# shanglianlm0525/CvPytorch

Hardware: AMD Instinct MI355X
Metric: images/sec/node train step, YOLOv5-s@640 (value: batch resident in HBM when the timed region starts; with_h2d.value: the same step fed from pinned host memory inside the region) & DeepLabv3+R50@1024x512 (config3_deeplabv3plus_r50.value) (higher is better)
Workload: dtype bf16; 1 GPU; coco_yolov5_s.yml YOLOv5-s 640x640 bf16 train step (fwd+loss+bwd+SGD-nesterov+EMA), per-GPU batch 64, synthetic COCO-shape tensors resident in HBM; global_batch=64, parallelism=dp1, launch=hipGraph replay of the whole step, world=1, transport=none (single process), grad_buckets=0, sync_bn=False, deterministic=True

## Files before the change

cvpytorch_amd/arena.py:

```python
import math
from copy import deepcopy

import torch

from . import comm as CM
from . import lib as L
from . import ops
from .train import build_param_groups

_PREP_PLAN = __import__("os").environ.get("CVHIP_PREP_PLAN", "1") != "0"
_ALIGN = 8


def _dense_view(flat, off, like):
    return flat[off:off + like.numel()].as_strided(like.shape, like.stride())


def paired_arena_order(items, follow):
    present = {id(t) for t in items}
    out, placed = [], set()
    for t in items:
        if id(t) in placed:
            continue
        out.append(t)
# ... 346 lines not shown
            if torch.cuda.is_current_stream_capturing():
                ops._OWNED_BACKWARD[0] = True
                try:
                    loss.backward()
                finally:
                    ops._OWNED_BACKWARD[0] = False
                ops.check_parked()
                return None
            seed = self._seeds[key] = torch.ones_like(loss)
        ops._OWNED_BACKWARD[0] = True
        try:
            loss.backward(gradient=seed)
        finally:
            ops._OWNED_BACKWARD[0] = False
        ops.check_parked()

    def scale_loss(self, loss):
        return loss * self.ls_state[0] if self.loss_scaling else loss

    def loss_scale(self):
        v = self.ls_state.tolist()
        return v[0], int(v[3])

    def pre_step(self):
        d = 0.0
        if self.ema_param is not None:
            self.ema_updates += 1
            d = self.ema_decay * (1 - math.exp(-self.ema_updates / 2000))
        slot = self._dyn_host[self.steps % self._dyn_host.shape[0]]
        slot[0], slot[1] = d, self.lr_scale
        self.dyn.copy_(slot, non_blocking=True)

    def step_kernels(self):
        self.finish_allreduce()
        ema_ptr = self.ema_param.data_ptr() if self.ema_param is not None else None
        st = ops._stream()
        if self.loss_scaling:
            g, b, iv = self.ls_hyper
            L.call("cvhip_loss_scale_check", self.grad.data_ptr(), self.total, self.ls_state.data_ptr(), st)
            L.call("cvhip_loss_scale_update", self.ls_state.data_ptr(), self.ls_dyn.data_ptr(), g, b, iv, st)
        if self.optimizer == "adamw":
            L.call("cvhip_adamw_ema", self.param.data_ptr(), self.grad.data_ptr(), self.mom.data_ptr(), self.mom2.data_ptr(), ema_ptr, self.total,
                   self.seg_bounds.data_ptr(), self.seg_lr.data_ptr(), self.seg_wd.data_ptr(), len(self.params), self.betas[0], self.betas[1],
                   self.adam_eps, self.adam_step.data_ptr(), 0.0, 1.0 / self.world, self.dyn.data_ptr(),
                   self.ls_dyn.data_ptr() if self.loss_scaling else None, st)
        elif self.loss_scaling:
            L.call("cvhip_sgd_nesterov_ema_scaled", self.param.data_ptr(), self.grad.data_ptr(), self.mom.data_ptr(), ema_ptr, self.total,
                   self.seg_bounds.data_ptr(), self.seg_lr.data_ptr(), self.seg_wd.data_ptr(), len(self.params), self.momentum,
                   int(self.nesterov), 0, 0.0, 1.0 / self.world, self.dyn.data_ptr(), self.ls_dyn.data_ptr(), st)
        else:
            L.call("cvhip_sgd_nesterov_ema", self.param.data_ptr(), self.grad.data_ptr(), self.mom.data_ptr(), ema_ptr, self.total,
                   self.seg_bounds.data_ptr(), self.seg_lr.data_ptr(), self.seg_wd.data_ptr(), len(self.params), self.momentum,
                   int(self.nesterov), 0, 0.0, 1.0 / self.world, self.dyn.data_ptr(), st)
        if self.ema_buf is not None and self.buf.numel():
            L.call("cvhip_ema_update", self.ema_buf.data_ptr(), self.buf.data_ptr(), self.buf.numel(), 0.0, self.dyn.data_ptr(), st)
        if self._nbt is not None and self.model.training:
            L.call("cvhip_i64_add", self._nbt.data_ptr(), self._nbt.numel(), 1, st)
        self.zero_grad()
        self.zero_stats()

    def prepare_weights(self):
        if not _PREP_PLAN:
            return
        plan = self.prep_plan
        if plan is None or not plan.valid():
            states = [s for s in ops.conv_states_of(self.model) if s.w_fprop is not None and s.rec is not None]
            if not states:
                return
            if torch.cuda.is_current_stream_capturing():
                return
            plan = self.prep_plan = ops.PrepPlan(states)
        plan.run()

    def post_step(self):
        self.steps += 1
        ops.bump_weights_epoch()
        self._reset_buckets()

    def step(self):
        self.pre_step()
        self.step_kernels()
        self.post_step()


class FlatTrainStep:

    def __init__(self, model, state, sync_buffers=False):
        self.model, self.state, self.sync_buffers = model, state, sync_buffers
        self.g1 = self.g2 = None
        self.static_losses = None
        self.eager_tail = False
        self.static_imgs = self.static_targets = None
        self.feats = self.g_feats = None

    @property
    def graph(self):
        return self.g1

    @graph.setter
    def graph(self, v):
        if v is None:
            self.g1 = self.g2 = None
            self.state.defer_allreduce = False
            self.eager_tail = False

    def _eager(self, imgs, targets):
        self.state.prepare_weights()
        losses = self.model(imgs, targets, "train")
        self.state.backward(losses["loss"])
# ... 83 lines not shown
```

cvpytorch_amd/csrc/f16_names.h:

```cpp
#pragma once
#define cvhip_adamw_ema cvhip_adamw_ema_f16
#define cvhip_add2d cvhip_add2d_f16
#define cvhip_add_act_fwd cvhip_add_act_fwd_f16
#define cvhip_bn_acc_shards cvhip_bn_acc_shards_f16
#define cvhip_bn_act_bwd_apply cvhip_bn_act_bwd_apply_f16
#define cvhip_bn_act_bwd_apply_acc cvhip_bn_act_bwd_apply_acc_f16
#define cvhip_bn_act_bwd_partial cvhip_bn_act_bwd_partial_f16
#define cvhip_bn_act_bwd_sums_acc cvhip_bn_act_bwd_sums_acc_f16
#define cvhip_bn_act_fwd cvhip_bn_act_fwd_f16
#define cvhip_bn_act_fwd_acc cvhip_bn_act_fwd_acc_f16
#define cvhip_bn_act_fwd_acc_lazyres cvhip_bn_act_fwd_acc_lazyres_f16
#define cvhip_bn_add_act_fwd cvhip_bn_add_act_fwd_f16
#define cvhip_bn_bwd_finalize cvhip_bn_bwd_finalize_f16
#define cvhip_bn_eval_scale_shift cvhip_bn_eval_scale_shift_f16
#define cvhip_bn_finalize cvhip_bn_finalize_f16
#define cvhip_bn_finalize_acc cvhip_bn_finalize_acc_f16
#define cvhip_bn_stats_partial cvhip_bn_stats_partial_f16
#define cvhip_bn_tail_bwd_sums_acc cvhip_bn_tail_bwd_sums_acc_f16
#define cvhip_box_iou cvhip_box_iou_f16
#define cvhip_channel_scale_bwd_ds cvhip_channel_scale_bwd_ds_f16
#define cvhip_colreduce_rows cvhip_colreduce_rows_f16
#define cvhip_colsum_finalize cvhip_colsum_finalize_f16
#define cvhip_colsum_partial cvhip_colsum_partial_f16
#define cvhip_conv1x1_bwd_fused cvhip_conv1x1_bwd_fused_f16
// ... 31 lines not shown
#define cvhip_dwconv2d_fprop cvhip_dwconv2d_fprop_f16
#define cvhip_dwconv2d_fprop_act cvhip_dwconv2d_fprop_act_f16
#define cvhip_dwconv2d_fprop_stats cvhip_dwconv2d_fprop_stats_f16
#define cvhip_dwconv2d_fprop_stats_rows cvhip_dwconv2d_fprop_stats_rows_f16
#define cvhip_dwconv2d_wgrad cvhip_dwconv2d_wgrad_f16
#define cvhip_ema_update cvhip_ema_update_f16
#define cvhip_f32_unpad_add cvhip_f32_unpad_add_f16
#define cvhip_focus_nchw_f32_to_nhwc_bf16 cvhip_focus_nchw_f32_to_nhwc_bf16_f16
#define cvhip_global_avgpool_bwd cvhip_global_avgpool_bwd_f16
#define cvhip_global_avgpool_fwd cvhip_global_avgpool_fwd_f16
#define cvhip_head_permute_bwd cvhip_head_permute_bwd_f16
#define cvhip_head_permute_fwd cvhip_head_permute_fwd_f16
#define cvhip_i64_add cvhip_i64_add_f16
#define cvhip_last_error cvhip_last_error_f16
#define cvhip_loss_scale_check cvhip_loss_scale_check_f16
#define cvhip_loss_scale_update cvhip_loss_scale_update_f16
#define cvhip_maxpool2d_bwd cvhip_maxpool2d_bwd_f16
#define cvhip_maxpool2d_fwd cvhip_maxpool2d_fwd_f16
#define cvhip_nchw_f32_to_nhwc_bf16 cvhip_nchw_f32_to_nhwc_bf16_f16
#define cvhip_nchw_f32_to_nhwc_bf16_ld cvhip_nchw_f32_to_nhwc_bf16_ld_f16
#define cvhip_nhwc_bf16_to_nchw_f32 cvhip_nhwc_bf16_to_nchw_f32_f16
#define cvhip_nms_sorted cvhip_nms_sorted_f16
#define cvhip_nms_workspace_bytes cvhip_nms_workspace_bytes_f16
#define cvhip_ohem_select cvhip_ohem_select_f16
#define cvhip_ohem_select_workspace_bytes cvhip_ohem_select_workspace_bytes_f16
#define cvhip_ota_assign cvhip_ota_assign_f16
#define cvhip_ota_read_overflow cvhip_ota_read_overflow_f16
#define cvhip_ota_workspace_bytes cvhip_ota_workspace_bytes_f16
#define cvhip_prep_plan_build cvhip_prep_plan_build_f16
#define cvhip_prep_plan_item_bytes cvhip_prep_plan_item_bytes_f16
#define cvhip_prep_plan_run cvhip_prep_plan_run_f16
#define cvhip_resize_bilinear_bwd cvhip_resize_bilinear_bwd_f16
#define cvhip_resize_bilinear_bwd_workspace_bytes cvhip_resize_bilinear_bwd_workspace_bytes_f16
#define cvhip_resize_bilinear_bwd_ws cvhip_resize_bilinear_bwd_ws_f16
#define cvhip_resize_bilinear_fwd cvhip_resize_bilinear_fwd_f16
#define cvhip_resize_nearest_bwd cvhip_resize_nearest_bwd_f16
#define cvhip_resize_nearest_fwd cvhip_resize_nearest_fwd_f16
#define cvhip_scale_nc cvhip_scale_nc_f16
#define cvhip_seg_ce_bilinear_bwd cvhip_seg_ce_bilinear_bwd_f16
#define cvhip_seg_ce_bilinear_bwd_ohem cvhip_seg_ce_bilinear_bwd_ohem_f16
#define cvhip_seg_ce_bilinear_bwd_px cvhip_seg_ce_bilinear_bwd_px_f16
#define cvhip_seg_ce_bilinear_fwd cvhip_seg_ce_bilinear_fwd_f16
#define cvhip_seg_ce_bilinear_fwd_px cvhip_seg_ce_bilinear_fwd_px_f16
#define cvhip_seg_ce_bilinear_ok cvhip_seg_ce_bilinear_ok_f16
#define cvhip_seg_ce_bwd cvhip_seg_ce_bwd_f16
#define cvhip_seg_ce_fwd cvhip_seg_ce_fwd_f16
#define cvhip_seg_ce_rows cvhip_seg_ce_rows_f16
#define cvhip_sgd_nesterov_ema cvhip_sgd_nesterov_ema_f16
#define cvhip_sgd_nesterov_ema_scaled cvhip_sgd_nesterov_ema_scaled_f16
#define cvhip_simota_loss_bwd cvhip_simota_loss_bwd_f16
#define cvhip_simota_loss_fwd cvhip_simota_loss_fwd_f16
#define cvhip_simota_read_assignment cvhip_simota_read_assignment_f16
#define cvhip_simota_workspace_bytes cvhip_simota_workspace_bytes_f16
#define cvhip_u8_nhwc_to_bf16_norm cvhip_u8_nhwc_to_bf16_norm_f16
#define cvhip_upsample2x_bwd cvhip_upsample2x_bwd_f16
#define cvhip_upsample2x_cat_fwd cvhip_upsample2x_cat_fwd_f16
#define cvhip_version cvhip_version_f16
#define cvhip_yolov5_decode cvhip_yolov5_decode_f16
#define cvhip_yolov5_loss_finalize cvhip_yolov5_loss_finalize_f16
#define cvhip_yolov5_loss_level_bwd cvhip_yolov5_loss_level_bwd_f16
#define cvhip_yolov5_loss_level_bwd_bias cvhip_yolov5_loss_level_bwd_bias_f16
#define cvhip_yolov5_loss_level_fwd cvhip_yolov5_loss_level_fwd_f16
#define cvhip_yolov5_loss_level_fwd_assigned cvhip_yolov5_loss_level_fwd_assigned_f16
#define cvhip_yolov5_loss_workspace_bytes cvhip_yolov5_loss_workspace_bytes_f16
#define cvhip_zero_fill cvhip_zero_fill_f16
```

cvpytorch_amd/csrc/pool_resize.hip:

```cpp
#include "common.h"
#include "bilinear_index.h"

namespace cvhip {

__device__ __forceinline__ bool aligned16(const void* p) { return (((uintptr_t)p) & 15) == 0; }

__device__ __forceinline__ f32x8 load8(const h16_t* p, int c, int C, bool vec) {
  if (vec) return unpack8(*reinterpret_cast<const uint4*>(p + c));
  f32x8 r;
#pragma unroll
  for (int j = 0; j < 8; ++j) r.v[j] = (c + j < C) ? (float)p[c + j] : 0.f;
  return r;
}
__device__ __forceinline__ void store8(h16_t* p, int c, int C, bool vec, const f32x8& v) {
  if (vec) {
    *reinterpret_cast<uint4*>(p + c) = pack8(v);
    return;
  }
#pragma unroll
  for (int j = 0; j < 8; ++j)
    if (c + j < C) p[c + j] = (h16_t)v.v[j];
}

struct PoolParams {
// ... 71 lines not shown
    int oh_lo = ih + p.pad - p.k + 1;
    oh_lo = oh_lo <= 0 ? 0 : (oh_lo + p.s - 1) / p.s;
    int oh_hi = (ih + p.pad) / p.s;
    if (oh_hi > p.OH - 1) oh_hi = p.OH - 1;
    int ow_lo = iw + p.pad - p.k + 1;
    ow_lo = ow_lo <= 0 ? 0 : (ow_lo + p.s - 1) / p.s;
    int ow_hi = (iw + p.pad) / p.s;
    if (ow_hi > p.OW - 1) ow_hi = p.OW - 1;
    for (int oh = oh_lo; oh <= oh_hi; ++oh) {
      const int kh = ih - (oh * p.s - p.pad);
      for (int ow = ow_lo; ow <= ow_hi; ++ow) {
        const int kw = iw - (ow * p.s - p.pad);
        const int off = kh * p.k + kw;
        const int64_t opix = ((int64_t)(n * p.OH + oh) * p.OW + ow);
        const f32x8 g = load8(p.dy + opix * p.ld_dy, c, p.C, vec);
        const uint8_t* ip = p.cidx + opix * p.C + c;
        if (vec) {
          const uint2 iv = *reinterpret_cast<const uint2*>(ip);
#pragma unroll
          for (int j = 0; j < 8; ++j) {
            const unsigned b = ((j < 4 ? iv.x : iv.y) >> (8 * (j & 3))) & 0xffu;
            if ((int)b == off) acc[j] += g.v[j];
          }
        } else {
#pragma unroll
          for (int j = 0; j < 8; ++j)
            if (c + j < p.C && ip[j] == off) acc[j] += g.v[j];
        }
      }
    }
    h16_t* dst = p.dx + ((int64_t)(n * p.H + ih) * p.W + iw) * p.ld_dx;
    f32x8 o;
    if (p.accumulate) {
      const f32x8 old = load8(dst, c, p.C, vec);
#pragma unroll
      for (int j = 0; j < 8; ++j) o.v[j] = old.v[j] + acc[j];
    } else {
#pragma unroll
      for (int j = 0; j < 8; ++j) o.v[j] = acc[j];
    }
    store8(dst, c, p.C, vec, o);
  }
}

constexpr int kPoolLdsCvbMax = 4;
constexpr int kPoolLdsMaxPix = 4096;
static inline int pool_lds_cvb(int HW, bool bwd) {
  for (int cvb = kPoolLdsCvbMax; cvb >= 1; cvb >>= 1)
    if (HW * cvb * (bwd ? 24 : 40) <= 160 * 1024) return cvb;
  return 0;
}

template <int K, int kPoolLdsCvb>
__global__ __launch_bounds__(256) void maxpool_s1_lds_fwd_kernel(const PoolParams p) {
  extern __shared__ __attribute__((aligned(16))) unsigned char pool_smem[];
  const int CV = p.C >> 3;
  const int groups = (CV + kPoolLdsCvb - 1) / kPoolLdsCvb;
  const int n = blockIdx.x / groups, cv0 = (blockIdx.x - n * groups) * kPoolLdsCvb;
  const int cvb = min(kPoolLdsCvb, CV - cv0);
  const int HW = p.H * p.W;
  const int items = HW * kPoolLdsCvb;
  uint4* const xs = reinterpret_cast<uint4*>(pool_smem);
  uint4* const rvs = xs + items;
  uint2* const rks = reinterpret_cast<uint2*>(rvs + items);
  const h16_t* const xn = p.x + (int64_t)n * HW * p.ld_x + cv0 * 8;
  for (int i = threadIdx.x; i < items; i += 256) {
    const int pix = i / kPoolLdsCvb, cv = i - pix * kPoolLdsCvb;
    if (cv < cvb) xs[i] = *reinterpret_cast<const uint4*>(xn + (int64_t)pix * p.ld_x + cv * 8);
  }
  __syncthreads();
  constexpr int PAD = K / 2;
  for (int i = threadIdx.x; i < items; i += 256) {
    const int pix = i / kPoolLdsCvb, cv = i - pix * kPoolLdsCvb;
    if (cv >= cvb) continue;
    const int h = pix / p.W, w = pix - h * p.W;
    f32x8 ov;
    int ok[8];
    bool first = true;
#pragma unroll
    for (int j = 0; j < 8; ++j) {
      ov.v[j] = -INFINITY;
      ok[j] = 0;
    }
#pragma unroll
    for (int kw = 0; kw < K; ++kw) {
      const int iw = w + kw - PAD;
      if ((unsigned)iw >= (unsigned)p.W) continue;
      const f32x8 v = unpack8(xs[(h * p.W + iw) * kPoolLdsCvb + cv]);
#pragma unroll
      for (int j = 0; j < 8; ++j) {
        if (first) ok[j] = kw;
        if (v.v[j] > ov.v[j] || v.v[j] != v.v[j]) {
          ov.v[j] = v.v[j];
          ok[j] = kw;
        }
      }
      first = false;
    }
    rvs[i] = pack8(ov);
    uint2 kk;
    kk.x = (unsigned)ok[0] | ((unsigned)ok[1] << 8) | ((unsigned)ok[2] << 16) | ((unsigned)ok[3] << 24);
    kk.y = (unsigned)ok[4] | ((unsigned)ok[5] << 8) | ((unsigned)ok[6] << 16) | ((unsigned)ok[7] << 24);
    rks[i] = kk;
  }
  __syncthreads();
  for (int i = threadIdx.x; i < items; i += 256) {
    const int pix = i / kPoolLdsCvb, cv = i - pix * kPoolLdsCvb;
    if (cv >= cvb) continue;
    const int h = pix / p.W, w = pix - h * p.W;
    float best[8];
    int bi[8];
    bool first = true;
#pragma unroll
    for (int j = 0; j < 8; ++j) {
      best[j] = -INFINITY;
      bi[j] = 0;
    }
#pragma unroll
    for (int kh = 0; kh < K; ++kh) {
      const int ih = h + kh - PAD;
      if ((unsigned)ih >= (unsigned)p.H) continue;
      const int o = (ih * p.W + w) * kPoolLdsCvb + cv;
      const f32x8 v = unpack8(rvs[o]);
      const uint2 kk = rks[o];
#pragma unroll
      for (int j = 0; j < 8; ++j) {
        const int off = kh * K + (int)(((j < 4 ? kk.x : kk.y) >> (8 * (j & 3))) & 0xffu);
        if (first) bi[j] = off;
        if (v.v[j] > best[j] || v.v[j] != v.v[j]) {
          best[j] = v.v[j];
          bi[j] = off;
        }
      }
      first = false;
    }
    {
      const int64_t opix = (int64_t)n * HW + h * p.W + w;
      f32x8 o;
#pragma unroll
      for (int j = 0; j < 8; ++j) o.v[j] = best[j];
      *reinterpret_cast<uint4*>(p.y + opix * p.ld_y + (cv0 + cv) * 8) = pack8(o);
      if (p.idx) {
        uint2 iv;
        iv.x = (unsigned)bi[0] | ((unsigned)bi[1] << 8) | ((unsigned)bi[2] << 16) | ((unsigned)bi[3] << 24);
        iv.y = (unsigned)bi[4] | ((unsigned)bi[5] << 8) | ((unsigned)bi[6] << 16) | ((unsigned)bi[7] << 24);
        *reinterpret_cast<uint2*>(p.idx + opix * p.C + (cv0 + cv) * 8) = iv;
      }
    }
  }
}

template <int K, int kPoolLdsCvb>
__global__ __launch_bounds__(256) void maxpool_s1_lds_bwd_kernel(const PoolParams p) {
  extern __shared__ __attribute__((aligned(16))) unsigned char pool_smem[];
  const int HW = p.H * p.W;
  uint4* const gs = reinterpret_cast<uint4*>(pool_smem);
  uint2* const is = reinterpret_cast<uint2*>(pool_smem + (size_t)HW * kPoolLdsCvb * 16);
  const int CV = p.C >> 3;
  const int groups = (CV + kPoolLdsCvb - 1) / kPoolLdsCvb;
  const int n = blockIdx.x / groups, cv0 = (blockIdx.x - n * groups) * kPoolLdsCvb;
  const int cvb = min(kPoolLdsCvb, CV - cv0);
  for (int i = threadIdx.x; i < HW * kPoolLdsCvb; i += 256) {
    const int pix = i / kPoolLdsCvb, cv = i - pix * kPoolLdsCvb;
    if (cv < cvb) {
      const int64_t opix = (int64_t)n * HW + pix;
      gs[i] = *reinterpret_cast<const uint4*>(p.dy + opix * p.ld_dy + (cv0 + cv) * 8);
      is[i] = *reinterpret_cast<const uint2*>(p.cidx + opix * p.C + (cv0 + cv) * 8);
    }
  }
  __syncthreads();
  constexpr int PAD = K / 2;
  for (int i = threadIdx.x; i < HW * kPoolLdsCvb; i += 256) {
    const int pix = i / kPoolLdsCvb, cv = i - pix * kPoolLdsCvb;
    if (cv >= cvb) continue;
    const int ih = pix / p.W, iw = pix - ih * p.W;
    float acc[8];
#pragma unroll
    for (int j = 0; j < 8; ++j) acc[j] = 0.f;
    const int oh_lo = max(0, ih - PAD), oh_hi = min(p.H - 1, ih + PAD);
    const int ow_lo = max(0, iw - PAD), ow_hi = min(p.W - 1, iw + PAD);
    for (int oh = oh_lo; oh <= oh_hi; ++oh) {
      const int kh = ih - oh + PAD;
      for (int ow = ow_lo; ow <= ow_hi; ++ow) {
        const unsigned off = (unsigned)(kh * K + (iw - ow + PAD));
        const int o = (oh * p.W + ow) * kPoolLdsCvb + cv;
        const f32x8 g = unpack8(gs[o]);
        const uint2 iv = is[o];
#pragma unroll
        for (int j = 0; j < 8; ++j) {
          const unsigned b = ((j < 4 ? iv.x : iv.y) >> (8 * (j & 3))) & 0xffu;
          if (b == off) acc[j] += g.v[j];
        }
      }
    }
    h16_t* const dst = p.dx + ((int64_t)n * HW + pix) * p.ld_dx + (cv0 + cv) * 8;
    f32x8 o;
    if (p.accumulate) {
      const f32x8 old = unpack8(*reinterpret_cast<const uint4*>(dst));
#pragma unroll
      for (int j = 0; j < 8; ++j) o.v[j] = old.v[j] + acc[j];
    } else {
#pragma unroll
      for (int j = 0; j < 8; ++j) o.v[j] = acc[j];
    }
    *reinterpret_cast<uint4*>(dst) = pack8(o);
  }
}

static bool pool_lds_ok(const PoolParams& p, bool bwd) {
  auto a16 = [](const void* q) { return (((uintptr_t)q) & 15) == 0; };
  static int on = -1;
  if (on < 0) {
    const char* e = getenv("CVHIP_POOL_LDS");
    on = (e && e[0] == '0') ? 0 : 1;
  }
  if (!on || p.s != 1 || !(p.k & 1) || p.pad != p.k / 2 || p.OH != p.H || p.OW != p.W || (p.k != 3 && p.k != 5 && p.k != 9 && p.k != 13)) return false;
  const int cvb = pool_lds_cvb(p.H * p.W, bwd);
  if ((p.C & 7) || p.H * p.W > kPoolLdsMaxPix || cvb == 0 || (int64_t)p.N * ((p.C / 8 + cvb - 1) / cvb) < 128) return false;
  if (bwd) return (p.ld_dy & 7) == 0 && (p.ld_dx & 7) == 0 && a16(p.dy) && a16(p.dx) && ((((uintptr_t)p.cidx) & 7) == 0);
  return (p.ld_x & 7) == 0 && (p.ld_y & 7) == 0 && a16(p.x) && a16(p.y) && (!p.idx || ((((uintptr_t)p.idx) & 7) == 0));
}

template <int K, int CVB>
static int launch_pool_lds(const PoolParams& p, bool bwd, hipStream_t s) {
  constexpr int kPoolLdsCvb = CVB;
  const int groups = (p.C / 8 + kPoolLdsCvb - 1) / kPoolLdsCvb;
  const int lds = p.H * p.W * kPoolLdsCvb * (bwd ? 24 : 40);
  auto kf = maxpool_s1_lds_fwd_kernel<K, CVB>;
  auto kb = maxpool_s1_lds_bwd_kernel<K, CVB>;
  static bool attr_done[2][64] = {};
  int devid = 0;
  (void)hipGetDevice(&devid);
  bool& done = attr_done[bwd ? 1 : 0][devid & 63];
  if (!done) {
    const int cap = 160 * 1024;
    hipError_t e = bwd ? hipFuncSetAttribute(reinterpret_cast<const void*>(kb), hipFuncAttributeMaxDynamicSharedMemorySize, cap)
                       : hipFuncSetAttribute(reinterpret_cast<const void*>(kf), hipFuncAttributeMaxDynamicSharedMemorySize, cap);
    if (e != hipSuccess) {
      set_last_error("hipFuncSetAttribute(maxpool_s1_lds)", e);
      return CVHIP_ERR_LAUNCH;
    }
    done = true;
  }
  if (bwd) hipLaunchKernelGGL(kb, dim3(p.N * groups), dim3(256), lds, s, p);
  else hipLaunchKernelGGL(kf, dim3(p.N * groups), dim3(256), lds, s, p);
  return check_launch(bwd ? "maxpool_s1_lds_bwd_kernel" : "maxpool_s1_lds_fwd_kernel");
}

static int try_pool_lds(const PoolParams& p, bool bwd, hipStream_t s) {
  if (!pool_lds_ok(p, bwd)) return -1;
  const int cvb = pool_lds_cvb(p.H * p.W, bwd);
#define CVHIP_POOL_K(KV)                                       \
  if (cvb == 4) return launch_pool_lds<KV, 4>(p, bwd, s);     \
  if (cvb == 2) return launch_pool_lds<KV, 2>(p, bwd, s);     \
  return launch_pool_lds<KV, 1>(p, bwd, s);
  switch (p.k) {
    case 3: CVHIP_POOL_K(3)
    case 5: CVHIP_POOL_K(5)
    case 9: CVHIP_POOL_K(9)
    default: CVHIP_POOL_K(13)
  }
#undef CVHIP_POOL_K
}

struct UpParams {
  const h16_t *a, *b;
  h16_t* out;
  int ld_a, ld_b, ld_out, Ca, Cb, N, Ha, Wa;
};

__global__ __launch_bounds__(256) void up2cat_fwd_kernel(const UpParams p) {
  const int Ct = p.Ca + p.Cb;
  const int CVa = (p.Ca + 7) >> 3, CVb = (p.Cb + 7) >> 3;
  const int CV = CVa + CVb;
  const int OH = p.Ha * 2, OW = p.Wa * 2;
  const bool vec = (p.Ca & 7) == 0 && (p.Cb & 7) == 0 && (p.ld_a & 7) == 0 && (p.ld_b & 7) == 0 &&
                   (p.ld_out & 7) == 0 && aligned16(p.a) && aligned16(p.b) && aligned16(p.out);
  (void)Ct;
  const int64_t total = (int64_t)p.N * OH * OW * CV;
  for (int64_t i = (int64_t)blockIdx.x * 256 + threadIdx.x; i < total; i += (int64_t)gridDim.x * 256) {
    int cv, ow, oh, n;
    split_index(i, CV, OW, OH, &cv, &ow, &oh, &n);
    h16_t* orow = p.out + ((int64_t)(n * OH + oh) * OW + ow) * p.ld_out;
    if (cv < CVa) {
      const f32x8 v = load8(p.a + ((int64_t)(n * p.Ha + (oh >> 1)) * p.Wa + (ow >> 1)) * p.ld_a, cv * 8, p.Ca, vec);
      store8(orow, cv * 8, p.Ca, vec, v);
    } else {
      const int cb = (cv - CVa) * 8;
      const f32x8 v = load8(p.b + ((int64_t)(n * OH + oh) * OW + ow) * p.ld_b, cb, p.Cb, vec);
      store8(orow + p.Ca, cb, p.Cb, vec, v);
    }
  }
}

__global__ __launch_bounds__(256) void up2_bwd_kernel(const UpParams p) {
  const int CV = (p.Ca + 7) >> 3;
  const int OW = p.Wa * 2, OH = p.Ha * 2;
  const bool vec = (p.Ca & 7) == 0 && (p.ld_a & 7) == 0 && (p.ld_out & 7) == 0 && aligned16(p.a) && aligned16(p.out);
  const int64_t total = (int64_t)p.N * p.Ha * p.Wa * CV;
  for (int64_t i = (int64_t)blockIdx.x * 256 + threadIdx.x; i < total; i += (int64_t)gridDim.x * 256) {
    int cv, w, h, n;
    split_index(i, CV, p.Wa, p.Ha, &cv, &w, &h, &n);
    f32x8 s;
#pragma unroll
    for (int j = 0; j < 8; ++j) s.v[j] = 0.f;
#pragma unroll
    for (int dy = 0; dy < 2; ++dy)
#pragma unroll
      for (int dx = 0; dx < 2; ++dx) {
        const f32x8 v = load8(p.out + ((int64_t)(n * OH + 2 * h + dy) * OW + 2 * w + dx) * p.ld_out, cv * 8, p.Ca, vec);
#pragma unroll
        for (int j = 0; j < 8; ++j) s.v[j] += v.v[j];
      }
    store8(const_cast<h16_t*>(p.a) + ((int64_t)(n * p.Ha + h) * p.Wa + w) * p.ld_a, cv * 8, p.Ca, vec, s);
  }
// ... 553 lines not shown
  if (k * k > 255 || pad * 2 > k) return CVHIP_ERR_UNSUPPORTED;
  PoolParams p{};
  p.x = (const h16_t*)x;
  p.y = (h16_t*)y;
  p.idx = argmax;
  p.ld_x = ld_x;
  p.ld_y = ld_y;
  p.N = N;
  p.C = C;
  p.H = H;
  p.W = W;
  p.k = k;
  p.s = stride;
  p.pad = pad;
  p.OH = (H + 2 * pad - k) / stride + 1;
  p.OW = (W + 2 * pad - k) / stride + 1;
  {
    const int rc = try_pool_lds(p, false, (hipStream_t)stream);
    if (rc >= 0 || rc < -1) return rc;
  }
  const int64_t total = (int64_t)N * p.OH * p.OW * ((C + 7) / 8);
  hipLaunchKernelGGL(maxpool_fwd_kernel, dim3(grid_for(total)), dim3(256), 0, (hipStream_t)stream, p);
  return check_launch("maxpool_fwd_kernel");
}

int cvhip_maxpool2d_bwd(const void* dy, int32_t ld_dy, const uint8_t* argmax, void* dx, int32_t ld_dx, int32_t N,
                        int32_t C, int32_t H, int32_t W, int32_t k, int32_t stride, int32_t pad, int accumulate,
                        void* stream) {
  if (!dy || !dx || !argmax || N <= 0 || C <= 0 || H <= 0 || W <= 0 || k <= 0 || stride <= 0 || pad < 0)
    return CVHIP_ERR_INVALID;
  PoolParams p{};
  p.dy = (const h16_t*)dy;
  p.cidx = argmax;
  p.dx = (h16_t*)dx;
  p.ld_dy = ld_dy;
  p.ld_dx = ld_dx;
  p.N = N;
  p.C = C;
  p.H = H;
  p.W = W;
  p.k = k;
  p.s = stride;
  p.pad = pad;
  p.OH = (H + 2 * pad - k) / stride + 1;
  p.OW = (W + 2 * pad - k) / stride + 1;
  p.accumulate = accumulate;
  {
    const int rc = try_pool_lds(p, true, (hipStream_t)stream);
    if (rc >= 0 || rc < -1) return rc;
  }
  const int64_t total = (int64_t)N * H * W * ((C + 7) / 8);
  hipLaunchKernelGGL(maxpool_bwd_kernel, dim3(grid_for(total)), dim3(256), 0, (hipStream_t)stream, p);
  return check_launch("maxpool_bwd_kernel");
}

int cvhip_upsample2x_cat_fwd(const void* a, int32_t ld_a, int32_t Ca, const void* b, int32_t ld_b, int32_t Cb,
                             void* out, int32_t ld_out, int32_t N, int32_t Ha, int32_t Wa, void* stream) {
  if (!a || !out || Ca <= 0 || Cb < 0 || (Cb > 0 && !b) || N <= 0 || Ha <= 0 || Wa <= 0) return CVHIP_ERR_INVALID;
  UpParams p{};
  p.a = (const h16_t*)a;
  p.b = (const h16_t*)b;
  p.out = (h16_t*)out;
  p.ld_a = ld_a;
  p.ld_b = ld_b;
  p.ld_out = ld_out;
  p.Ca = Ca;
  p.Cb = Cb;
  p.N = N;
  p.Ha = Ha;
  p.Wa = Wa;
  const int64_t total = (int64_t)N * Ha * 2 * Wa * 2 * ((Ca + 7) / 8 + (Cb + 7) / 8);
  hipLaunchKernelGGL(up2cat_fwd_kernel, dim3(grid_for(total)), dim3(256), 0, (hipStream_t)stream, p);
  return check_launch("up2cat_fwd_kernel");
}

int cvhip_upsample2x_bwd(const void* dout, int32_t ld_dout, void* da, int32_t ld_da, int32_t Ca, int32_t N, int32_t Ha,
                         int32_t Wa, void* stream) {
  if (!dout || !da || Ca <= 0 || N <= 0 || Ha <= 0 || Wa <= 0) return CVHIP_ERR_INVALID;
  UpParams p{};
  p.out = (h16_t*)const_cast<void*>(dout);
  p.a = (const h16_t*)da;
  p.ld_out = ld_dout;
  p.ld_a = ld_da;
  p.Ca = Ca;
  p.N = N;
  p.Ha = Ha;
  p.Wa = Wa;
  const int64_t total = (int64_t)N * Ha * Wa * ((Ca + 7) / 8);
  hipLaunchKernelGGL(up2_bwd_kernel, dim3(grid_for(total)), dim3(256), 0, (hipStream_t)stream, p);
  return check_launch("up2_bwd_kernel");
}

int cvhip_resize_nearest_fwd(const void* x, int32_t ld_x, void* y, int32_t ld_y, int32_t N, int32_t C, int32_t Hi, int32_t Wi,
                             int32_t Ho, int32_t Wo, void* stream) {
  if (!x || !y || N <= 0 || C <= 0 || Hi <= 0 || Wi <= 0 || Ho <= 0 || Wo <= 0) return CVHIP_ERR_INVALID;
  BilParams p{};
  p.src = (const h16_t*)x;
  p.dst = (h16_t*)y;
  p.ld_src = ld_x;
  p.ld_dst = ld_y;
  p.N = N;
  p.C = C;
  p.Hi = Hi;
  p.Wi = Wi;
  p.Ho = Ho;
  p.Wo = Wo;
// ... 186 lines not shown
```

cvpytorch_amd/csrc/weights_optim.hip:

```cpp
#include <string.h>

#include "common.h"
#include "conv_plan.h"

namespace cvhip {

__global__ __launch_bounds__(256) void cast_f32_bf16_kernel(const float* __restrict__ src, h16_t* __restrict__ dst, int64_t n) {
  const int64_t nv = n >> 3;
  const bool al = (((uintptr_t)src) & 15) == 0;
  for (int64_t i = (int64_t)blockIdx.x * 256 + threadIdx.x; i < nv; i += (int64_t)gridDim.x * 256) {
    float4 a, b;
    if (al) {
      a = reinterpret_cast<const float4*>(src)[2 * i];
      b = reinterpret_cast<const float4*>(src)[2 * i + 1];
    } else {
      const float* q = src + 8 * i;
      a = make_float4(q[0], q[1], q[2], q[3]);
      b = make_float4(q[4], q[5], q[6], q[7]);
    }
    uint4 u;
    u.x = pack2(a.x, a.y);
    u.y = pack2(a.z, a.w);
    u.z = pack2(b.x, b.y);
    u.w = pack2(b.z, b.w);
// ... 475 lines not shown
    it.K = d->K;
    it.R = d->R;
    it.S = d->S;
    it.C = d->C;
    it.Kv = d->k_valid > 0 ? d->k_valid : d->K;
    it.Cv = d->c_valid > 0 ? d->c_valid : d->C;
    const int64_t nel = (int64_t)d->K * d->R * d->S * d->C;
    it.blk_begin = blk;
    it.nblk_f = (int)cdiv64(nel, kPrepFpropPerBlock);
    it.nblk_d = 0;
    if (it.wd) {
      IgemmParams ip;
      const int ncls = plan_dgrad(d, &ip);
      if (ncls < 0) return ncls;
      it.ncls = ncls;
      int64_t end = 0;
      int tapn = 0;
      for (int q = 0; q < ncls; ++q) {
        const IgemmClass& c = ip.cls[q];
        PrepClass& pc = it.cls[q];
        pc.TR = c.TR; pc.TS = c.TS; pc.r0 = c.r0; pc.r_step = c.r_step; pc.s0 = c.s0; pc.s_step = c.s_step;
        pc.tap_begin = tapn;
        tapn += c.TR * c.TS;
        pc.w_off = c.w_off;
        pc.w_end = c.w_off + (int64_t)d->C * c.TR * c.TS * d->K;
        if (pc.w_off != end) return CVHIP_ERR_UNSUPPORTED;
        end = pc.w_end;
      }
      if (end != nel || tapn != d->R * d->S) return CVHIP_ERR_UNSUPPORTED;
      it.ktiles = cdiv(d->K, kPrepTile);
      it.ctiles = cdiv(d->C, kPrepTile);
      it.nblk_d = tapn * it.ktiles * it.ctiles;
    }
    it.nblk_bf = band_image_fprop(d) ? (int)cdiv64(nel / 8, 256) : 0;
    it.nblk_bd = (it.wd && band_image_dgrad(d)) ? (int)cdiv64(nel / 8, 256) : 0;
    blk += it.nblk_f + it.nblk_d + it.nblk_bf + it.nblk_bd;
  }
  *total_blocks = blk;
  return CVHIP_OK;
}

int cvhip_prep_plan_run(const void* table_device, int32_t n, int32_t total_blocks, void* stream) {
  if (!table_device || n <= 0 || total_blocks <= 0) return CVHIP_ERR_INVALID;
  hipLaunchKernelGGL(prep_all_kernel, dim3(total_blocks), dim3(256), 0, (hipStream_t)stream, (const PrepItem*)table_device, n);
  return check_launch("prep_all_kernel");
}

extern "C++" {
namespace cvhip {
__global__ void i64_add_kernel(long long* v, int64_t n, long long delta) {
  const int64_t i = (int64_t)blockIdx.x * blockDim.x + threadIdx.x;
  if (i < n) v[i] += delta;
}
}
}

int cvhip_i64_add(int64_t* v, int64_t n, int64_t delta, void* stream) {
  if (!v || n < 0) return CVHIP_ERR_INVALID;
  if (n == 0) return CVHIP_OK;
  hipLaunchKernelGGL(i64_add_kernel, dim3((unsigned)((n + 255) / 256)), dim3(256), 0, (hipStream_t)stream, (long long*)v, n, (long long)delta);
  return check_launch("i64_add_kernel");
}

int cvhip_ema_update(float* ema, const float* src, int64_t n, float decay, const float* dyn_decay, void* stream) {
  if (!ema || !src || n < 0) return CVHIP_ERR_INVALID;
  if (n == 0) return CVHIP_OK;
  hipLaunchKernelGGL(ema_kernel, dim3(grid1d(n)), dim3(256), 0, (hipStream_t)stream, ema, src, n, decay, dyn_decay);
  return check_launch("ema_kernel");
}

}
```

cvpytorch_amd/csrc/yolo_loss.hip:

```cpp
#pragma clang fp contract(off)
#include "common.h"
#include "dual4.h"

namespace cvhip {

constexpr int kLossMaxA = 8;
constexpr int kCandStride = 4;

struct YoloLossParams {
  const h16_t* raw;
  h16_t* draw;
  const float* targets;
  const int* assign;
  int ld, N, A, NO, H, W, T, nc, ncand;
  float anchor_t;
  float anchors[kLossMaxA * 2];
  int* winner;
  int* head;
  int* next;
  int* cell;
  float* cand;
  float* cgrad;
  int gstride;
  float* partial;
  float* dobj;
  float* sums;
  const float* gout;
  float k_box, k_cls, k_obj;
};

__device__ __forceinline__ D4 ciou_xywh(float x, float y, float w, float h, float tx, float ty, float tw, float th) {
  const float eps = 1e-7f;
  const D4 X = var(x, 0), Y = var(y, 1), Wd = var(w, 2), Hd = var(h, 3);
  const D4 b1x1 = X - scale(Wd, 0.5f), b1x2 = X + scale(Wd, 0.5f);
  const D4 b1y1 = Y - scale(Hd, 0.5f), b1y2 = Y + scale(Hd, 0.5f);
  const float b2x1 = tx - tw / 2, b2x2 = tx + tw / 2, b2y1 = ty - th / 2, b2y2 = ty + th / 2;
  const D4 iw = clamp0(dmin(b1x2, cst(b2x2)) - dmax(b1x1, cst(b2x1)));
  const D4 ih = clamp0(dmin(b1y2, cst(b2y2)) - dmax(b1y1, cst(b2y1)));
  const D4 inter = iw * ih;
  const D4 w1 = b1x2 - b1x1, h1 = (b1y2 - b1y1) + cst(eps);
  const float w2 = b2x2 - b2x1, h2 = b2y2 - b2y1 + eps;
  const D4 uni = (w1 * h1 + cst(w2 * h2)) - inter + cst(eps);
  const D4 iou = inter / uni;
  const D4 cw = dmax(b1x2, cst(b2x2)) - dmin(b1x1, cst(b2x1));
  const D4 ch = dmax(b1y2, cst(b2y2)) - dmin(b1y1, cst(b2y1));
  const D4 c2 = cw * cw + ch * ch + cst(eps);
  const D4 dx = cst(b2x1 + b2x2) - b1x1 - b1x2;
  const D4 dy = cst(b2y1 + b2y2) - b1y1 - b1y2;
  const D4 rho2 = scale(dx * dx + dy * dy, 0.25f);
  const D4 da = cst(atanf(w2 / h2)) - datan(w1 / h1);
  const D4 v = scale(da * da, 0.40528473456935108578f);
  const float alpha = v.v / (v.v - iou.v + (1.f + eps));
  return iou - (rho2 / c2 + scale(v, alpha));
}

__global__ __launch_bounds__(256) void yolo_cand_kernel(const YoloLossParams p) {
  const int lane = threadIdx.x & 63;
  const int c = blockIdx.x * 4 + (threadIdx.x >> 6);
  if (c >= p.ncand) return;
  const int T = p.T, A = p.A;
  const int off = c / (A * T);
  const int a = (c / T) % A;
  const int t = c % T;
  const float* tg = p.targets + (int64_t)t * 6;
  const float img = tg[0];
  const float nx = (float)p.W, ny = (float)p.H;
  const float gx = tg[2] * nx, gy = tg[3] * ny, gw = tg[4] * nx, gh = tg[5] * ny;
  const float aw = p.anchors[a * 2], ah = p.anchors[a * 2 + 1];
  const float rw = gw / aw, rh = gh / ah;
  const float rmax = fmaxf(fmaxf(rw, 1.f / rw), fmaxf(rh, 1.f / rh));
  bool sel = (img >= 0.f) && (rmax < p.anchor_t);
  const float gxi = nx - gx, gyi = ny - gy;
  const float g = 0.5f;
  if (off == 1) sel = sel && ((gx - floorf(gx)) < g) && (gx > 1.f);
  else if (off == 2) sel = sel && ((gy - floorf(gy)) < g) && (gy > 1.f);
  else if (off == 3) sel = sel && ((gxi - floorf(gxi)) < g) && (gxi > 1.f);
  else if (off == 4) sel = sel && ((gyi - floorf(gyi)) < g) && (gyi > 1.f);
  float* cs = p.cand + (int64_t)c * kCandStride;
  const float* tm = tg;
  if (p.assign) {
    const int m = p.assign[c];
    sel = m >= 0;
    if (sel) tm = p.targets + (int64_t)m * 6;
  }
  if (!sel) {
    if (lane == 0) {
      p.cell[c] = -1;
      cs[0] = 0.f;
      cs[1] = 0.f;
      cs[2] = 0.f;
    }
    return;
  }
  const float ox = (off == 1 ? 0.5f : (off == 3 ? -0.5f : 0.f)), oy = (off == 2 ? 0.5f : (off == 4 ? -0.5f : 0.f));
  int gi = (int)(gx - ox), gj = (int)(gy - oy);
  gi = min(max(gi, 0), p.W - 1);
  gj = min(max(gj, 0), p.H - 1);
  const int b = (int)img;
  const int cell = ((b * A + a) * p.H + gj) * p.W + gi;
  if (lane == 0) {
    p.cell[c] = cell;
    atomicMax(p.winner + cell, c + 1);
    p.next[c] = atomicExch(p.head + cell, c + 1);
  }
  const h16_t* px = p.raw + ((int64_t)(b * p.H + gj) * p.W + gi) * p.ld + a * p.NO;
  const float r0 = (float)px[0], r1 = (float)px[1], r2 = (float)px[2], r3 = (float)px[3];
  const float s0 = sigmoid_ref(r0), s1 = sigmoid_ref(r1), s2 = sigmoid_ref(r2), s3 = sigmoid_ref(r3);
  const float bx = s0 * 2.f - 0.5f, by = s1 * 2.f - 0.5f;
  const float bw = (s2 * 2.f) * (s2 * 2.f) * aw, bh = (s3 * 2.f) * (s3 * 2.f) * ah;
  const float mx = tm[2] * nx, my = tm[3] * ny, mw = tm[4] * nx, mh = tm[5] * ny;
  const D4 ci = ciou_xywh(bx, by, bw, bh, mx - (float)gi, my - (float)gj, mw, mh);
  float* gr = p.cgrad + (int64_t)c * p.gstride;
  if (lane == 0) {
    cs[0] = ci.v;
    cs[1] = 1.f - ci.v;
    gr[0] = -ci.d[0] * (2.f * s0 * (1.f - s0));
    gr[1] = -ci.d[1] * (2.f * s1 * (1.f - s1));
    gr[2] = -ci.d[2] * (8.f * s2 * s2 * (1.f - s2) * aw);
    gr[3] = -ci.d[3] * (8.f * s3 * s3 * (1.f - s3) * ah);
    gr[4] = 0.f;
  }
  int cls = (int)tm[1];
  cls = min(max(cls, 0), p.nc - 1);
  float lsum = 0.f;
  for (int k = lane; k < p.nc; k += 64) {
    const float x = (float)px[5 + k];
    const float tt = (k == cls) ? 1.f : 0.f;
    lsum += bce_logits(x, tt);
    gr[5 + k] = sigmoid_ref(x) - tt;
  }
#pragma unroll
  for (int o = 32; o > 0; o >>= 1) lsum += __shfl_xor(lsum, o, 64);
  if (lane == 0) cs[2] = p.nc > 1 ? lsum : 0.f;
}

__device__ __forceinline__ float block_sum_1024(float v, float* red) {
  const int t = threadIdx.x;
  red[t] = v;
  __syncthreads();
  for (int s = 512; s > 0; s >>= 1) {
    if (t < s) red[t] += red[t + s];
    __syncthreads();
  }
  const float r = red[0];
  __syncthreads();
  return r;
}

__device__ __forceinline__ void yolo_cand_reduce(const YoloLossParams& p, float* red) {
  float n = 0.f, lb = 0.f, lc = 0.f;
  for (int c0 = threadIdx.x; c0 < p.ncand; c0 += 8 * 1024) {
    int cl[8];
    float b8[8], c8[8];
#pragma unroll
    for (int u = 0; u < 8; ++u) {
      const int c = c0 + u * 1024;
      cl[u] = c < p.ncand ? p.cell[c] : -1;
    }
#pragma unroll
    for (int u = 0; u < 8; ++u) {
      const int64_t c = cl[u] >= 0 ? c0 + u * 1024 : 0;
      b8[u] = p.cand[c * kCandStride + 1];
      c8[u] = p.cand[c * kCandStride + 2];
    }
#pragma unroll
    for (int u = 0; u < 8; ++u) {
      if (cl[u] >= 0) {
        n += 1.f;
        lb += b8[u];
        lc += c8[u];
      }
    }
  }
  n = block_sum_1024(n, red);
  lb = block_sum_1024(lb, red);
  lc = block_sum_1024(lc, red);
  if (threadIdx.x == 0) {
    p.sums[0] = n;
    p.sums[1] = lb;
    p.sums[2] = lc;
  }
}

template <typename IT>
__global__ __launch_bounds__(256) void yolo_obj_bwd_fill_kernel(const YoloLossParams p) {
  const IT VP = (IT)(p.ld >> 3);
  const IT HW = (IT)p.H * (IT)p.W;
  const IT nvec = (IT)p.N * HW * VP;
  const float go = (p.gout ? p.gout[0] : 1.f) * p.k_obj;
  const IT step = (IT)gridDim.x * 256;
  const bool inv = (VP & (VP - 1)) == 0 && (step & (VP - 1)) == 0;
  const int vp_shift = inv ? __ffs((int)VP) - 1 : 0;
  auto anchors_of = [&](int c0) {
    unsigned m = 0;
    for (int a = 0; a < p.A; ++a) {
      const int oc = a * p.NO + 4;
      if (oc >= c0 && oc < c0 + 8) m |= 1u << a;
    }
    return m;
  };
  const unsigned my_mask = inv ? anchors_of((int)(((IT)blockIdx.x * 256 + threadIdx.x) & (VP - 1)) * 8) : 0u;
  for (IT i = (IT)blockIdx.x * 256 + threadIdx.x; i < nvec; i += step) {
    IT pix;
    int c0;
    unsigned mask;
    if (inv) {
      pix = i >> vp_shift;
      c0 = (int)(i & (VP - 1)) * 8;
      mask = my_mask;
    } else {
      pix = i / VP;
      c0 = (int)(i - pix * VP) * 8;
      mask = anchors_of(c0);
    }
    h16_t out[8];
#pragma unroll
    for (int j = 0; j < 8; ++j) out[j] = (h16_t)0.f;
    if (mask) {
      const IT n = pix / HW;
      const IT cell0 = pix + n * (IT)(p.A - 1) * HW;
      for (int a = 0; a < p.A; ++a) {
        if (!((mask >> a) & 1u)) continue;
        const int oc = a * p.NO + 4;
        const h16_t gq = (h16_t)(p.dobj[(int64_t)cell0 + (int64_t)a * (int64_t)HW] * go);
#pragma unroll
        for (int j = 0; j < 8; ++j)
          if (c0 + j == oc) out[j] = gq;
      }
    }
    *reinterpret_cast<uint4*>(p.draw + (int64_t)pix * p.ld + c0) = *reinterpret_cast<const uint4*>(out);
  }
}

template <bool BWD, typename IT>
__global__ __launch_bounds__(256) void yolo_obj_kernel(const YoloLossParams p) {
  __shared__ float red[256];
  const IT ncell = (IT)p.N * (IT)p.A * (IT)p.H * (IT)p.W;
  const float go = BWD ? (p.gout ? p.gout[0] : 1.f) * p.k_obj : 0.f;
  float acc = 0.f;
  for (IT i = (IT)blockIdx.x * 256 + threadIdx.x; i < ncell; i += (IT)gridDim.x * 256) {
    IT r = i / (IT)p.W;
    const int gi = (int)(i - r * (IT)p.W);
    const IT r2 = r / (IT)p.H;
    const int gj = (int)(r - r2 * (IT)p.H);
    const int n = (int)(r2 / (IT)p.A);
    const int a = (int)(r2 - (IT)n * (IT)p.A);
    const int64_t o = ((int64_t)(n * p.H + gj) * p.W + gi) * p.ld + a * p.NO + 4;
    const float x = (float)p.raw[o];
    const int w = p.winner[i];
    const float tt = w > 0 ? fmaxf(p.cand[(int64_t)(w - 1) * kCandStride], 0.f) : 0.f;
    if (BWD) p.draw[o] = (h16_t)((sigmoid_ref(x) - tt) * go);
    else {
      acc += bce_logits(x, tt);
      p.dobj[i] = sigmoid_ref(x) - tt;
    }
  }
  if (!BWD) {
    red[threadIdx.x] = acc;
    __syncthreads();
    for (int s = 128; s > 0; s >>= 1) {
      if (threadIdx.x < s) red[threadIdx.x] += red[threadIdx.x + s];
      __syncthreads();
    }
    if (threadIdx.x == 0) p.partial[blockIdx.x] = red[0];
  }
}

__global__ __launch_bounds__(1024) void yolo_obj_reduce_kernel(const YoloLossParams p, int nblocks) {
  __shared__ float red[1024];
  if (blockIdx.x == 1) {
    yolo_cand_reduce(p, red);
    return;
  }
  float v = 0.f;
  for (int i = threadIdx.x; i < nblocks; i += 1024) v += p.partial[i];
  v = block_sum_1024(v, red);
  if (threadIdx.x == 0) p.sums[3] = v;
}

__global__ __launch_bounds__(256) void yolo_cand_bwd_kernel(const YoloLossParams p) {
  const int lane = threadIdx.x & 63;
  const int c = blockIdx.x * 4 + (threadIdx.x >> 6);
  if (c >= p.ncand) return;
  const int cell = p.cell[c];
  if (cell < 0 || p.winner[cell] != c + 1) return;
  const float n = p.sums[0];
  const float g = p.gout ? p.gout[0] : 1.f;
  const float kb = g * p.k_box / n, kc = g * p.k_cls / n;
  int mine = 0x7fffffff;
  int cur = p.head[cell];
  int cnt = 0;
  float acc0 = 0.f, acc1 = 0.f;
  const int ch0 = lane, ch1 = lane + 64;
  while (cur != 0) {
    const int e = cur - 1;
    if (cnt < 64) {
      if (lane == cnt) mine = e;
    } else {
      const float* gr = p.cgrad + (int64_t)e * p.gstride;
      if (ch0 < p.NO) acc0 += gr[ch0];
      if (ch1 < p.NO) acc1 += gr[ch1];
    }
    ++cnt;
    cur = p.next[e];
  }
  const int k = cnt < 64 ? cnt : 64;
  int last = -1;
  for (int i = 0; i < k; ++i) {
    int cand_v = mine > last ? mine : 0x7fffffff;
#pragma unroll
    for (int o = 32; o > 0; o >>= 1) cand_v = min(cand_v, __shfl_xor(cand_v, o, 64));
    last = cand_v;
    const float* gr = p.cgrad + (int64_t)cand_v * p.gstride;
    if (ch0 < p.NO) acc0 += gr[ch0];
    if (ch1 < p.NO) acc1 += gr[ch1];
  }
  const int gi = cell % p.W;
  int r = cell / p.W;
  const int gj = r % p.H;
  r /= p.H;
  const int a = r % p.A;
  const int b = r / p.A;
  h16_t* dst = p.draw + ((int64_t)(b * p.H + gj) * p.W + gi) * p.ld + a * p.NO;
  if (ch0 < p.NO && ch0 != 4) dst[ch0] = (h16_t)(acc0 * (ch0 < 4 ? kb : kc));
  if (ch1 < p.NO) dst[ch1] = (h16_t)(acc1 * kc);
}

constexpr int kBiasRows = CVHIP_YOLO_BIAS_ROWS;
template <typename IT>
__global__ __launch_bounds__(256) void yolo_bias_partial_kernel(const YoloLossParams p, float* __restrict__ part) {
  __shared__ float wacc[4][kLossMaxA * 128];
  __shared__ float ored[kLossMaxA][256];
  const int K = p.A * p.NO;
  const int t = threadIdx.x, lane = t & 63, wave = t >> 6;
  for (int i = t; i < 4 * kLossMaxA * 128; i += 256) (&wacc[0][0])[i] = 0.f;
  __syncthreads();
  const int per_blk = (p.ncand + gridDim.x - 1) / gridDim.x;
  const int c_begin = blockIdx.x * per_blk, c_end = min(c_begin + per_blk, p.ncand);
  for (int g0 = c_begin + wave * 64; g0 < c_end; g0 += 256) {
    const int c = g0 + lane;
    unsigned long long m = __ballot(c < c_end && p.cell[c] >= 0);
    while (m) {
      int cc[8];
      float v0[8], v1[8];
      int nv = 0;
#pragma unroll
      for (int u = 0; u < 8; ++u) {
        cc[u] = -1;
        if (m) {
          cc[u] = g0 + __ffsll((long long)m) - 1;
          m &= m - 1;
          nv = u + 1;
        }
      }
#pragma unroll
      for (int u = 0; u < 8; ++u) {
        const float* gr = p.cgrad + (int64_t)(cc[u] >= 0 ? cc[u] : 0) * p.gstride;
        v0[u] = (cc[u] >= 0 && lane < p.NO && lane != 4) ? gr[lane] : 0.f;
        v1[u] = (cc[u] >= 0 && lane + 64 < p.NO) ? gr[lane + 64] : 0.f;
      }
#pragma unroll
      for (int u = 0; u < 8; ++u) {
        if (u < nv) {
          const int a = (cc[u] / p.T) % p.A;
          if (lane < p.NO && lane != 4) wacc[wave][a * p.NO + lane] += v0[u];
          if (lane + 64 < p.NO) wacc[wave][a * p.NO + lane + 64] += v1[u];
        }
      }
    }
  }
  float oa[kLossMaxA];
#pragma unroll
  for (int k = 0; k < kLossMaxA; ++k) oa[k] = 0.f;
  {
    const IT ncell = (IT)p.N * (IT)p.A * (IT)p.H * (IT)p.W, HW = (IT)p.H * (IT)p.W;
    const IT per = (ncell + gridDim.x - 1) / gridDim.x;
    const IT i_begin = (IT)blockIdx.x * per;
    IT i_end = i_begin + per;
    if (i_end > ncell) i_end = ncell;
    for (IT i0 = i_begin + t; i0 < i_end; i0 += 256 * 8) {
      float d[8];
      int a[8];
#pragma unroll
      for (int u = 0; u < 8; ++u) {
        const IT i = i0 + (IT)u * 256;
        const bool ok = i < i_end;
        d[u] = ok ? p.dobj[ok ? i : i_begin] : 0.f;
        a[u] = (int)(((ok ? i : i_begin) / HW) % (IT)p.A);
      }
#pragma unroll
      for (int u = 0; u < 8; ++u)
#pragma unroll
        for (int k = 0; k < kLossMaxA; ++k) oa[k] += k == a[u] ? d[u] : 0.f;
    }
  }
#pragma unroll
  for (int k = 0; k < kLossMaxA; ++k) ored[k][t] = oa[k];
  __syncthreads();
  for (int st = 128; st > 0; st >>= 1) {
    if (t < st) {
#pragma unroll
      for (int k = 0; k < kLossMaxA; ++k) ored[k][t] += ored[k][t + st];
    }
    __syncthreads();
  }
  const float n = p.sums[0];
  const float g = p.gout ? p.gout[0] : 1.f;
  const float kb = n > 0.f ? g * p.k_box / n : 0.f, kc = n > 0.f ? g * p.k_cls / n : 0.f, go = g * p.k_obj;
  float* const row = part + (int64_t)blockIdx.x * 2 * K;
  for (int ch = t; ch < K; ch += 256) {
    const int a = ch / p.NO, o = ch - a * p.NO;
    const float v = ((wacc[0][ch] + wacc[1][ch]) + wacc[2][ch]) + wacc[3][ch];
    row[ch] = o == 4 ? ored[a][0] * go : v * (o < 4 ? kb : kc);
  }
}

__global__ void yolo_finalize_kernel(const float* sums, int L, const float* ncell, const float* balance, float hyp_box,
                                     float hyp_obj, float hyp_cls, int nc, float bs, float* total, float* stats) {
  if (threadIdx.x != 0 || blockIdx.x != 0) return;
  float lbox = 0.f, lobj = 0.f, lcls = 0.f;
  for (int i = 0; i < L; ++i) {
    const float n = sums[i * 4];
    if (n > 0.f) {
      lbox += sums[i * 4 + 1] / n;
      lcls += sums[i * 4 + 2] / (n * (float)nc);
    }
    lobj += sums[i * 4 + 3] / ncell[i] * balance[i];
  }
  lbox *= hyp_box;
  lobj *= hyp_obj;
  lcls *= hyp_cls;
  total[0] = (lbox + lobj + lcls) * bs;
  stats[0] = lbox;
  stats[1] = lobj;
  stats[2] = lcls;
}

static int fill(YoloLossParams& p, const cvhip_yolo_loss_desc* d, const void* raw, const float* targets, void* ws, float* sums) {
  if (!d || !raw || !targets || !ws || !sums) return CVHIP_ERR_INVALID;
  if (d->N <= 0 || d->A <= 0 || d->A > kLossMaxA || d->NO < 6 || d->NO > 128 || d->H <= 0 || d->W <= 0 || d->T <= 0 || d->ld < d->A * d->NO)
    return CVHIP_ERR_INVALID;
  const int64_t ncell = (int64_t)d->N * d->A * d->H * d->W;
  const int64_t ncand = (int64_t)5 * d->A * d->T;
  if (ncell >= (1ll << 31) || ncand >= (1ll << 30)) return CVHIP_ERR_UNSUPPORTED;
  p.raw = (const h16_t*)raw;
  p.draw = nullptr;
  p.targets = targets;
  p.assign = nullptr;
  p.ld = d->ld;
  p.N = d->N;
  p.A = d->A;
  p.NO = d->NO;
  p.H = d->H;
  p.W = d->W;
  p.T = d->T;
  p.nc = d->NO - 5;
  p.ncand = (int)ncand;
  p.anchor_t = d->anchor_t;
  for (int i = 0; i < d->A * 2; ++i) p.anchors[i] = d->anchors[i];
  p.gstride = (d->NO + 3) / 4 * 4;
  unsigned char* w = (unsigned char*)ws;
  auto take = [&](int64_t bytes) {
    unsigned char* r = w;
    w += (bytes + 255) / 256 * 256;
    return r;
  };
  p.winner = (int*)take(ncell * 4);
  p.head = (int*)take(ncell * 4);
  p.next = (int*)take(ncand * 4);
  p.cell = (int*)take(ncand * 4);
  p.cand = (float*)take(ncand * kCandStride * 4);
  p.cgrad = (float*)take(ncand * p.gstride * 4);
  p.partial = (float*)take(1024 * 4);
  p.dobj = (float*)take(ncell * 4);
  p.sums = sums;
  p.gout = nullptr;
  p.k_box = p.k_cls = p.k_obj = 0.f;
  return CVHIP_OK;
}

}

using namespace cvhip;

extern "C" {

int64_t cvhip_yolov5_loss_workspace_bytes(const cvhip_yolo_loss_desc* d) {
  if (!d || d->N <= 0 || d->A <= 0 || d->NO <= 0 || d->H <= 0 || d->W <= 0 || d->T <= 0) return CVHIP_ERR_INVALID;
  const int64_t ncell = (int64_t)d->N * d->A * d->H * d->W;
  const int64_t ncand = (int64_t)5 * d->A * d->T;
  const int64_t gs = (d->NO + 3) / 4 * 4;
  auto r = [](int64_t b) { return (b + 255) / 256 * 256; };
  return r(ncell * 4) * 2 + r(ncand * 4) * 2 + r(ncand * kCandStride * 4) + r(ncand * gs * 4) + r(1024 * 4) + r(ncell * 4);
}

static int level_fwd(const cvhip_yolo_loss_desc* d, const void* raw, const float* targets, const int32_t* assign, void* ws, float* sums4,
                     void* stream);

int cvhip_yolov5_loss_level_fwd(const cvhip_yolo_loss_desc* d, const void* raw, const float* targets, void* ws, float* sums4,
                                void* stream) {
  return level_fwd(d, raw, targets, nullptr, ws, sums4, stream);
}

int cvhip_yolov5_loss_level_fwd_assigned(const cvhip_yolo_loss_desc* d, const void* raw, const float* targets, const int32_t* assign,
                                         void* ws, float* sums4, void* stream) {
  if (!assign) return CVHIP_ERR_INVALID;
  return level_fwd(d, raw, targets, assign, ws, sums4, stream);
}

static int level_fwd(const cvhip_yolo_loss_desc* d, const void* raw, const float* targets, const int32_t* assign, void* ws, float* sums4,
                     void* stream) {
  YoloLossParams p;
  int rc = fill(p, d, raw, targets, ws, sums4);
  if (rc != CVHIP_OK) return rc;
  p.assign = assign;
  hipStream_t st = (hipStream_t)stream;
  const int64_t ncell = (int64_t)p.N * p.A * p.H * p.W;
  rc = zero_fill(p.winner, (ncell * 4 + 255) / 256 * 256 * 2, st);
  if (rc != CVHIP_OK) return rc;
  hipLaunchKernelGGL(yolo_cand_kernel, dim3(cdiv(p.ncand, 4)), dim3(256), 0, st, p);
  const int nb = (int)(cdiv64(ncell, 256) < 1024 ? cdiv64(ncell, 256) : 1024);
// ... 9 lines not shown
  hipLaunchKernelGGL(yolo_finalize_kernel, dim3(1), dim3(64), 0, (hipStream_t)stream, sums, levels, ncell, balance, hyp_box, hyp_obj,
                     hyp_cls, nc, batch, total, stats3);
  return check_launch("yolov5_loss_finalize");
}

static int level_bwd(const cvhip_yolo_loss_desc* d, const void* raw, const float* targets, void* ws, const float* sums4, const float* gout,
                     float k_box, float k_cls, float k_obj, void* draw, float* bias_partial, void* stream);

int cvhip_yolov5_loss_level_bwd(const cvhip_yolo_loss_desc* d, const void* raw, const float* targets, void* ws, const float* sums4,
                                const float* gout, float k_box, float k_cls, float k_obj, void* draw, void* stream) {
  return level_bwd(d, raw, targets, ws, sums4, gout, k_box, k_cls, k_obj, draw, nullptr, stream);
}

int cvhip_yolov5_loss_level_bwd_bias(const cvhip_yolo_loss_desc* d, const void* raw, const float* targets, void* ws, const float* sums4,
                                     const float* gout, float k_box, float k_cls, float k_obj, void* draw, float* bias_partial,
                                     void* stream) {
  if (!bias_partial) return CVHIP_ERR_INVALID;
  return level_bwd(d, raw, targets, ws, sums4, gout, k_box, k_cls, k_obj, draw, bias_partial, stream);
}

static int level_bwd(const cvhip_yolo_loss_desc* d, const void* raw, const float* targets, void* ws, const float* sums4, const float* gout,
                     float k_box, float k_cls, float k_obj, void* draw, float* bias_partial, void* stream) {
  YoloLossParams p;
  int rc = fill(p, d, raw, targets, ws, const_cast<float*>(sums4));
  if (rc != CVHIP_OK) return rc;
  if (!draw) return CVHIP_ERR_INVALID;
  p.draw = (h16_t*)draw;
  p.gout = gout;
  p.k_box = k_box;
  p.k_cls = k_cls;
  p.k_obj = k_obj;
  hipStream_t st = (hipStream_t)stream;
  const int64_t ncell = (int64_t)p.N * p.A * p.H * p.W;
  if ((p.ld & 7) == 0 && (((uintptr_t)p.draw) & 15) == 0) {
    const int64_t nvec = (int64_t)p.N * p.H * p.W * (p.ld >> 3);
    const int nbf = (int)(cdiv64(nvec, 256 * 4) < 8192 ? cdiv64(nvec, 256 * 4) : 8192);
    if (nvec + (int64_t)nbf * 256 < (1ll << 32)) hipLaunchKernelGGL(yolo_obj_bwd_fill_kernel<unsigned>, dim3(nbf > 0 ? nbf : 1), dim3(256), 0, st, p);
    else hipLaunchKernelGGL(yolo_obj_bwd_fill_kernel<int64_t>, dim3(nbf > 0 ? nbf : 1), dim3(256), 0, st, p);
  } else {
    rc = zero_fill(p.draw, (int64_t)p.N * p.H * p.W * p.ld * 2, st);
    if (rc != CVHIP_OK) return rc;
    const int nb = (int)(cdiv64(ncell, 256) < 8192 ? cdiv64(ncell, 256) : 8192);
    if (ncell + (int64_t)nb * 256 < (1ll << 32)) hipLaunchKernelGGL((yolo_obj_kernel<true, unsigned>), dim3(nb), dim3(256), 0, st, p);
    else hipLaunchKernelGGL((yolo_obj_kernel<true, int64_t>), dim3(nb), dim3(256), 0, st, p);
  }
  hipLaunchKernelGGL(yolo_cand_bwd_kernel, dim3(cdiv(p.ncand, 4)), dim3(256), 0, st, p);
  if (bias_partial) {
    if (ncell < (1ll << 31)) hipLaunchKernelGGL(yolo_bias_partial_kernel<unsigned>, dim3(kBiasRows), dim3(256), 0, st, p, bias_partial);
    else hipLaunchKernelGGL(yolo_bias_partial_kernel<int64_t>, dim3(kBiasRows), dim3(256), 0, st, p, bias_partial);
  }
  return check_launch("yolov5_loss_level_bwd");
}

}
```

cvpytorch_amd/lib.py:

```python
import ctypes as C
import os

import torch

_HERE = os.path.dirname(os.path.abspath(__file__))
LIB_PATH = os.environ.get("CVHIP_LIB") or os.path.join(_HERE, "libcvhip.so")

OK, ERR_INVALID, ERR_UNSUPPORTED, ERR_LAUNCH = 0, -1, -2, -3
ACT_NONE, ACT_RELU, ACT_SILU, ACT_LEAKY, ACT_SIGMOID, ACT_HSWISH = 0, 1, 2, 3, 4, 5
DTYPE_F32, DTYPE_F64, DTYPE_I32, DTYPE_BF16, DTYPE_U8 = 0, 1, 2, 3, 4
RED_SUM, RED_MAX, RED_MIN = 0, 1, 2
DGRAD_CLASS_INTS = 12
REDUCE_SCRATCH_ROWS = 64
YOLO_BIAS_ROWS = 256
BN_ACC_SHARDS = 16


class CvhipError(RuntimeError):
    pass


class ConvDesc(C.Structure):
    _fields_ = [(n, C.c_int32) for n in (
        "N", "C", "H", "W", "K", "R", "S", "stride_h", "stride_w", "pad_h", "pad_w", "dil_h", "dil_w",
        "groups", "x_ld", "y_ld", "k_valid", "c_valid")]

    def key(self):
        return tuple(getattr(self, n) for n, _ in self._fields_)


class ConvFuse(C.Structure):
    _fields_ = [("bias", C.c_void_p), ("stats_partial", C.c_void_p), ("bn_acc", C.c_void_p), ("ep_scale", C.c_void_p),
                ("ep_shift", C.c_void_p), ("ep_act", C.c_int32), ("ep_act_param", C.c_float), ("pro_scale", C.c_void_p),
                ("pro_shift", C.c_void_p), ("pro_act", C.c_int32), ("pro_act_param", C.c_float), ("z_out", C.c_void_p),
                ("z_ld", C.c_int32), ("residual", C.c_void_p), ("residual_ld", C.c_int32), ("residual_pre", C.c_int32),
                ("x_image", C.c_void_p), ("x_image_planes", C.c_int32), ("pro_lo", C.c_int32), ("pro_hi", C.c_int32),
                ("y2", C.c_void_p), ("y2_ld", C.c_int32), ("y_split", C.c_int32)]


class LazyIn(C.Structure):
    _fields_ = [("scale", C.c_void_p), ("shift", C.c_void_p), ("act", C.c_int32), ("act_param", C.c_float), ("c_lo", C.c_int32),
                ("c_hi", C.c_int32)]


PATCH_CLASS_INTS = 30
BAND_PLAN_INTS = 13
WGRAD_BAND_PLAN_INTS = 8


class PrepEntry(C.Structure):
    _fields_ = [("desc", ConvDesc), ("master", C.c_void_p), ("w_fprop", C.c_void_p), ("w_dgrad", C.c_void_p)]


class YoloLossDesc(C.Structure):
    _fields_ = [(n, C.c_int32) for n in ("N", "A", "NO", "H", "W", "ld", "T")] + [("anchor_t", C.c_float), ("anchors", C.c_float * 16)]


class OtaDesc(C.Structure):
    _fields_ = [(n, C.c_int32) for n in ("L", "N", "A", "NO", "T", "G")] + [("H", C.c_int32 * 4), ("W", C.c_int32 * 4), ("ld", C.c_int32 * 4),
                                                                            ("stride", C.c_float * 4), ("anchors", (C.c_float * 16) * 4),
                                                                            ("anchor_t", C.c_float), ("img_size", C.c_float)]


class SimotaDesc(C.Structure):
    _fields_ = [(n, C.c_int32) for n in ("L", "B", "A", "G", "nc")] + [("H", C.c_int32 * 4), ("W", C.c_int32 * 4), ("ld", C.c_int32 * 4),
                                                                       ("stride", C.c_float * 4)]

# ... 22 lines not shown
    "cvhip_prep_plan_run": (_i32, [_p, _i32, _i32, _p]),
    "cvhip_conv2d_fprop": (_i32, [_dp, _p, _p, _p, _p, _p, _p]),
    "cvhip_conv2d_fprop_fused": (_i32, [_dp, _p, _p, _p, C.POINTER(ConvFuse), _p]),
    "cvhip_conv2d_wgrad_image": (_i32, [_dp, _p, _i32, _p, _p, _p]),
    "cvhip_conv2d_fprop_prologue_ok": (_i32, [_dp, _i32]),
    "cvhip_conv2d_patch_plan": (_i32, [_dp, _i32, C.POINTER(_i32), _i32]),
    "cvhip_conv2d_band_plan": (_i32, [_dp, _i32, C.POINTER(_i32)]),
    "cvhip_conv2d_wgrad_band_plan": (_i32, [_dp, C.POINTER(_i32)]),
    "cvhip_conv1x1_stream_prologue_ok": (_i32, [_dp, _i32]),
    "cvhip_conv2d_wgrad_stem_bn": (_i32, [_dp, _p, _p, _i32, _p, _p, _p, _p, _p, _p, _p, _i32, _p, _p, _i32, _i32, _f32, _p, _p]),
    "cvhip_bn_finalize_acc": (_i32, [_p, _i32, _i32, _i64, _p, _p, _p, _p, _f32, _f32, _p, _p, _p, _p, _p]),
    "cvhip_bn_act_fwd_acc_lazyres": (_i32, [_p, _i32, _p, _i32, _i64, _i32, _p, _i32, _i64, _p, _p, _p, _p, _f32, _f32, _p, _p, _p, _p, _i32, _f32,
                                     _p, _i32, _p, _p, _p]),
    "cvhip_conv1x1_bwd_fused_split": (_i32, [_dp, _p, _i32, _p, _i32, _i32, _p, _p, _i32, _p, _p, _p, _p, _p, _p, _p, _i32, _p, _p, _i32, _i32, _f32, _p,
                                      _i32, _p, _i32, _p, C.POINTER(LazyIn), _p]),
    "cvhip_conv1x1_bwd_fused_lazy": (_i32, [_dp, _p, _i32, _p, _i32, _i32, _p, _p, _p, _p, _p, _p, _p, _p, _i32, _p, _p, _i32, _i32, _f32, _p, _i32,
                                     _p, _i32, _p, C.POINTER(LazyIn), _p]),
    "cvhip_conv2d_dgrad": (_i32, [_dp, _p, _p, _p, _p]),
    "cvhip_conv2d_dgrad_add": (_i32, [_dp, _p, _p, _p, _i32, _p, _p]),
    "cvhip_conv2d_wgrad": (_i32, [_dp, _p, _p, _p, _i32, _p]),
    "cvhip_conv2d_wgrad_det_workspace_bytes": (_i64, [_dp]),
    "cvhip_conv2d_wgrad_det": (_i32, [_dp, _p, _p, _p, _i32, _p, _i64, _p]),
    "cvhip_conv1x1_bwd_fused_ok": (_i32, [_dp]),
    "cvhip_conv1x1_bwd_fused": (_i32, [_dp, _p, _i32, _p, _i32, _i32, _p, _p, _p, _p, _p, _p, _p, _p, _p, _i32, _f32, _p, _i32, _p, _i32,
                                _p, _p]),
    "cvhip_dwconv2d_fprop": (_i32, [_dp, _p, _p, _p, _p, _p]),
    "cvhip_dwconv2d_fprop_act": (_i32, [_dp, _p, _p, _p, _i32, _f32, _p, _p]),
    "cvhip_dwconv2d_fprop_stats_rows": (_i64, [_dp, _p, _p]),
    "cvhip_dwconv2d_fprop_stats": (_i32, [_dp, _p, _p, _p, _p, _p, _p]),
    "cvhip_dwconv2d_dgrad": (_i32, [_dp, _p, _p, _p, _p]),
    "cvhip_dwconv2d_wgrad": (_i32, [_dp, _p, _p, _p, _i32, _p]),
    "cvhip_colreduce_rows": (_i32, [_i64, _i32]),
    "cvhip_bn_stats_partial": (_i32, [_p, _i64, _i32, _i32, _p, _p]),
    "cvhip_bn_finalize": (_i32, [_p, _i32, _i32, _i64, _p, _p, _p, _p, _f32, _f32, _p, _p, _p, _p, _p]),
    "cvhip_bn_eval_scale_shift": (_i32, [_i32, _p, _p, _p, _p, _f32, _p, _p, _p]),
    "cvhip_bn_act_fwd": (_i32, [_p, _i32, _p, _i32, _i64, _i32, _p, _p, _i32, _f32, _p, _i32, _p]),
    "cvhip_bn_add_act_fwd": (_i32, [_p, _i32, _p, _i32, _i64, _i32, _p, _p, _i32, _f32, _p, _i32, _p]),
    "cvhip_bn_act_bwd_partial": (_i32, [_p, _i32, _p, _i32, _i64, _i32, _p, _p, _p, _p, _i32, _f32, _p, _p]),
    "cvhip_bn_bwd_finalize": (_i32, [_p, _i32, _i32, _p, _p, _p, _p, _p]),
    "cvhip_bn_act_bwd_apply": (_i32, [_p, _i32, _p, _i32, _p, _i32, _i64, _i32, _p, _p, _p, _p, _p, _p, _i32, _f32, _p]),
    "cvhip_bn_acc_shards": (_i32, []),
    "cvhip_conv2d_fprop_acc": (_i32, [_dp, _p, _p, _p, _p, _p]),
    "cvhip_bn_act_fwd_acc": (_i32, [_p, _i32, _p, _i32, _i64, _i32, _p, _i32, _i64, _p, _p, _p, _p, _f32, _f32, _p, _p, _p, _p, _i32, _f32, _p, _i32,
                             _i32, _p]),
    "cvhip_bn_act_bwd_sums_acc": (_i32, [_p, _i32, _p, _i32, _i64, _i32, _p, _p, _p, _p, _i32, _f32, _p, _i32, _p]),
    "cvhip_bn_tail_bwd_sums_acc": (_i32, [_p, _i32, _p, _i32, _p, _i32, _p, _i32, _i64, _i32, _p, _p, _i32, _f32, _p, _i32, _p]),
    "cvhip_bn_act_bwd_apply_acc": (_i32, [_p, _i32, _p, _i32, _p, _i32, _i64, _i32, _p, _p, _p, _p, _p, _i32, _p, _p, _i32, _i32, _f32, _p]),
    "cvhip_conv1x1_bwd_fused_acc": (_i32, [_dp, _p, _i32, _p, _i32, _i32, _p, _p, _p, _p, _p, _p, _p, _p, _i32, _p, _p, _i32, _i32, _f32, _p, _i32,
                                    _p, _i32, _p, _p]),
    "cvhip_colsum_partial": (_i32, [_p, _i64, _i32, _i32, _p, _p]),
    "cvhip_colsum_finalize": (_i32, [_p, _i32, _i32, _p, _i32, _p]),
    "cvhip_maxpool2d_fwd": (_i32, [_p, _i32, _p, _i32, _p, _i32, _i32, _i32, _i32, _i32, _i32, _i32, _p]),
    "cvhip_maxpool2d_bwd": (_i32, [_p, _i32, _p, _p, _i32, _i32, _i32, _i32, _i32, _i32, _i32, _i32, _i32, _p]),
    "cvhip_upsample2x_cat_fwd": (_i32, [_p, _i32, _i32, _p, _i32, _i32, _p, _i32, _i32, _i32, _i32, _p]),
    "cvhip_upsample2x_bwd": (_i32, [_p, _i32, _p, _i32, _i32, _i32, _i32, _i32, _p]),
    "cvhip_zero_fill": (_i32, [_p, _i64, _p]),
    "cvhip_f32_unpad_add": (_i32, [_p, _p, _i32, _i32, _i32, _i32, _p]),
    "cvhip_copy2d": (_i32, [_p, _i32, _p, _i32, _i64, _i32, _p]),
    "cvhip_add2d": (_i32, [_p, _i32, _p, _i32, _p, _i32, _i64, _i32, _p]),
    "cvhip_add_act_fwd": (_i32, [_p, _i32, _p, _i32, _p, _i32, _i64, _i32, _i32, _f32, _p]),
    "cvhip_channel_scale_bwd_ds": (_i32, [_p, _i32, _p, _i32, _p, _i32, _i32, _i32, _p]),
    "cvhip_scale_nc": (_i32, [_p, _i32, _p, _p, _i32, _i32, _i32, _i32, _p]),
    "cvhip_seg_ce_rows": (_i32, [_i64]),
    "cvhip_seg_ce_fwd": (_i32, [_p, _i32, _p, _i64, _i32, _i32, _p, _p, _p]),
    "cvhip_seg_ce_bwd": (_i32, [_p, _i32, _p, _i64, _i32, _i32, _p, _p, _p, _i32, _p]),
    "cvhip_seg_ce_bilinear_ok": (_i32, [_i32, _i32, _i32, _i32, _i32, _i32]),
    "cvhip_seg_ce_bilinear_fwd": (_i32, [_p, _i32, _p, _i32, _i32, _i32, _i32, _i32, _i32, _i32, _i32, _p, _p, _p]),
    "cvhip_seg_ce_bilinear_bwd": (_i32, [_p, _i32, _p, _i32, _i32, _i32, _i32, _i32, _i32, _i32, _i32, _p, _p, _p, _i32, _p]),
    "cvhip_seg_ce_bilinear_fwd_px": (_i32, [_p, _i32, _p, _i32, _i32, _i32, _i32, _i32, _i32, _i32, _i32, _p, _p]),
    "cvhip_seg_ce_bilinear_bwd_px": (_i32, [_p, _i32, _p, _i32, _i32, _i32, _i32, _i32, _i32, _i32, _i32, _p, _p, _p, _i32, _p]),
    "cvhip_detail_boundary_targets": (_i32, [_p, _i32, _i32, _i32, _f32, _p, _p]),
    "cvhip_ohem_select_workspace_bytes": (_i64, []),
    "cvhip_ohem_select": (_i32, [_p, _i64, _i32, _f32, _f32, _p, _p, _p]),
    "cvhip_seg_ce_bilinear_bwd_ohem": (_i32, [_p, _i32, _p, _i32, _i32, _i32, _i32, _i32, _i32, _i32, _i32, _p, _f32, _p, _p, _p, _i32, _p]),
    "cvhip_resize_nearest_fwd": (_i32, [_p, _i32, _p, _i32, _i32, _i32, _i32, _i32, _i32, _i32, _p]),
    "cvhip_resize_nearest_bwd": (_i32, [_p, _i32, _p, _i32, _i32, _i32, _i32, _i32, _i32, _i32, _p]),
    "cvhip_resize_bilinear_fwd": (_i32, [_p, _i32, _p, _i32, _i32, _i32, _i32, _i32, _i32, _i32, _i32, _p]),
    "cvhip_resize_bilinear_bwd": (_i32, [_p, _i32, _p, _i32, _i32, _i32, _i32, _i32, _i32, _i32, _i32, _p]),
    "cvhip_resize_bilinear_bwd_workspace_bytes": (_i64, [_i32, _i32, _i32, _i32, _i32, _i32]),
    "cvhip_resize_bilinear_bwd_ws": (_i32, [_p, _i32, _p, _i32, _i32, _i32, _i32, _i32, _i32, _i32, _i32, _p, _i64, _p]),
    "cvhip_global_avgpool_fwd": (_i32, [_p, _i32, _p, _i32, _i32, _i32, _p]),
    "cvhip_global_avgpool_bwd": (_i32, [_p, _p, _i32, _i32, _i32, _i32, _p]),
    "cvhip_nchw_f32_to_nhwc_bf16": (_i32, [_p, _p, _i32, _i32, _i32, _i32, _i32, _p]),
    "cvhip_focus_nchw_f32_to_nhwc_bf16": (_i32, [_p, _p, _i32, _i32, _i32, _i32, _i32, _p]),
    "cvhip_nhwc_bf16_to_nchw_f32": (_i32, [_p, _i32, _p, _i32, _i32, _i32, _i32, _p]),
    "cvhip_nchw_f32_to_nhwc_bf16_ld": (_i32, [_p, _p, _i32, _i32, _i32, _i32, _i32, _p]),
    "cvhip_head_permute_fwd": (_i32, [_p, _i32, _p, _i32, _i32, _i32, _i32, _i32, _p]),
    "cvhip_head_permute_bwd": (_i32, [_p, _p, _i32, _i32, _i32, _i32, _i32, _i32, _p]),
    "cvhip_yolov5_decode": (_i32, [_p, _i32, _p, _i32, _i32, _i32, _i32, _i32, _f32, _p, _i64, _i64, _p]),
    "cvhip_nms_workspace_bytes": (_i64, [_i32]),
    "cvhip_nms_sorted": (_i32, [_p, _i32, _f32, _p, _p, _p, _p]),
    "cvhip_detect_postprocess_workspace_bytes": (_i64, [_i32, _i32, _i32]),
    "cvhip_detect_postprocess": (_i32, [_p, _i32, _i32, _i32, _i32, _f32, _f32, _f32, _i32, _i32, _i32, _i32, _i32, _p, _p, _p, _p, _p]),
    "cvhip_sort_workspace_bytes": (_i64, [_i64]),
    "cvhip_argsort_desc_f32": (_i32, [_p, _i64, _p, _p, _p]),
    "cvhip_box_iou": (_i32, [_p, _i32, _p, _i32, _p, _p]),
    "cvhip_adamw_ema": (_i32, [_p, _p, _p, _p, _p, _i64, _p, _p, _p, _i32, _f32, _f32, _f32, _p, _f32, _f32, _p, _p, _p]),
    "cvhip_sgd_nesterov_ema": (_i32, [_p, _p, _p, _p, _i64, _p, _p, _p, _i32, _f32, _i32, _i32, _f32, _f32, _p, _p]),
    "cvhip_sgd_nesterov_ema_scaled": (_i32, [_p, _p, _p, _p, _i64, _p, _p, _p, _i32, _f32, _i32, _i32, _f32, _f32, _p, _p, _p]),
    "cvhip_loss_scale_check": (_i32, [_p, _i64, _p, _p]),
    "cvhip_loss_scale_update": (_i32, [_p, _p, _f32, _f32, _i32, _p]),
    "cvhip_i64_add": (_i32, [_p, _i64, _i64, _p]),
    "cvhip_ema_update": (_i32, [_p, _p, _i64, _f32, _p, _p]),
    "cvhip_u8_nhwc_to_bf16_norm": (_i32, [_p, _i64, _i32, _p, _i32, _p, _p, _p]),
    "cvhip_yolov5_loss_workspace_bytes": (_i64, [_ylp]),
    "cvhip_yolov5_loss_level_fwd": (_i32, [_ylp, _p, _p, _p, _p, _p]),
    "cvhip_yolov5_loss_finalize": (_i32, [_p, _i32, _p, _p, _f32, _f32, _f32, _i32, _f32, _p, _p, _p]),
    "cvhip_yolov5_loss_level_bwd": (_i32, [_ylp, _p, _p, _p, _p, _p, _f32, _f32, _f32, _p, _p]),
    "cvhip_yolov5_loss_level_bwd_bias": (_i32, [_ylp, _p, _p, _p, _p, _p, _f32, _f32, _f32, _p, _p, _p]),
    "cvhip_ota_workspace_bytes": (_i64, [_otp]),
    "cvhip_ota_assign": (_i32, [_otp, _pp, _p, _p, _p, _p]),
    "cvhip_ota_read_overflow": (_i32, [_otp, _p, _p, _p]),
    "cvhip_yolov5_loss_level_fwd_assigned": (_i32, [_ylp, _p, _p, _p, _p, _p, _p]),
    "cvhip_simota_workspace_bytes": (_i64, [_smp]),
    "cvhip_simota_loss_fwd": (_i32, [_smp, _pp, _p, _p, _p, _p]),
    "cvhip_simota_loss_bwd": (_i32, [_smp, _pp, _p, _p, _p, _pp, _p]),
    "cvhip_simota_read_assignment": (_i32, [_smp, _p, _p, _p, _p]),
    "cvhip_comm_available": (_i32, []),
    "cvhip_comm_rccl_version": (_i32, []),
    "cvhip_comm_unique_id_bytes": (_i32, []),
    "cvhip_comm_get_unique_id": (_i32, [_p]),
    "cvhip_comm_init_rank": (_i32, [_pp, _i32, _i32, _p]),
    "cvhip_comm_destroy": (_i32, [_p]),
    "cvhip_comm_world": (_i32, [_p]),
    "cvhip_comm_rank": (_i32, [_p]),
    "cvhip_allreduce_bucket": (_i32, [_p, _p, _i64, _p]),
    "cvhip_comm_allreduce": (_i32, [_p, _p, _i64, _i32, _i32, _p]),
    "cvhip_comm_broadcast": (_i32, [_p, _p, _i64, _i32, _p]),
    "cvhip_comm_reduce_scatter_f32": (_i32, [_p, _p, _i64, _p]),
    "cvhip_comm_all_gather_f32": (_i32, [_p, _p, _i64, _p]),
}

PROBE_SIGNATURES = {
    "cvhip_probe_grid_barrier": (_i32, [_i32, _i32, _i32, _p, _p, _p, _p]),
    "cvhip_probe_mfma_16x16x32": (_i32, [_p, _p, _p, _p]),
    "cvhip_probe_ds_read_tr16": (_i32, [_p, _p, _p]),
    "cvhip_probe_lds_read_bw": (_i32, [_i32, _i32, _i32, _p, _p]),
    "cvhip_probe_mfma_peak": (_i32, [_i32, _i32, _p, _p]),
    "cvhip_probe_lds_read2": (_i32, [_i32, _i32, _i32, _i32, _p, _p]),
    "cvhip_probe_mfma_peak2": (_i32, [_i32, _i32, _i32, _i32, _i32, _p, _p]),
    "cvhip_probe_load_path": (_i32, [_i32, _i32, _p, _i64, _i64, _i32, _i32, _i32, _p, _p]),
    "cvhip_probe_atomic_add": (_i32, [_i32, _p, _i32, _i32, _i32, _p]),
    "cvhip_probe_stage": (_i32, [_i32, _p, _i64, _p, _i32, _i32, _i32, _i32, _p, _p]),
    "cvhip_probe_gather": (_i32, [_i32, _p, _i64, _i32, _i32, _i32, _i32, _i32, _i32, _p, _p]),
}
PROBES_LIB_PATH = os.path.join(_HERE, "libcvhip_probes.so")

_lib = None
_probes = None
_F16 = set()
PRECISION = "bf16"


def set_precision(p):
    global PRECISION
    if p not in ("bf16", "fp16"):
        raise CvhipError("precision must be 'bf16' or 'fp16'")
    load()
    PRECISION = p


def load():
# ... 74 lines not shown
```

cvpytorch_amd/ops.py:

```python
import ctypes as C

import torch

from . import lib as L

ACT_DTYPE = torch.bfloat16
_weights_epoch = 0
_stats_epoch = [0]


def set_precision(p):
    global ACT_DTYPE
    L.set_precision(p)
    ACT_DTYPE = torch.float16 if p == "fp16" else torch.bfloat16
    bump_weights_epoch()
    _desc_cache.clear()


def precision():
    return L.PRECISION


def bump_weights_epoch():
    global _weights_epoch
# ... 1507 lines not shown
        st = _stream()
        dz, dz_ld = as_nhwc(dz)
        dy = empty_nhwc(N, K, P, Q, dev)
        dgamma = dbeta = None
        if train_bn:
            rows = _colreduce_rows(M, K)
            partial = torch.empty((rows + L.REDUCE_SCRATCH_ROWS, 2, K), dtype=torch.float32, device=dev)
            L.call("cvhip_bn_act_bwd_partial", dz.data_ptr(), dz_ld, y.data_ptr(), y_ld, M, K, stats[2].data_ptr(),
                   stats[3].data_ptr(), stats[0].data_ptr(), stats[1].data_ptr(), act, ap, partial.data_ptr(), st)
            dgamma = torch.empty((K,), dtype=torch.float32, device=dev)
            dbeta = torch.empty((K,), dtype=torch.float32, device=dev)
            L.call("cvhip_bn_bwd_finalize", partial.data_ptr(), rows, K, dgamma.data_ptr(), dbeta.data_ptr(), None, None, st)
            ag, ab = (dgamma, dbeta) if ctx.sync is None else _sync_bwd_sums(dgamma, dbeta, ctx.sync)
            L.call("cvhip_bn_act_bwd_apply", dz.data_ptr(), dz_ld, y.data_ptr(), y_ld, dy.data_ptr(), K, M, K,
                   stats[2].data_ptr(), stats[3].data_ptr(), stats[0].data_ptr(), stats[1].data_ptr(), ag.data_ptr(),
                   ab.data_ptr(), act, ap, st)
        else:
            sc = stats[2].data_ptr() if stats is not None else None
            sh = stats[3].data_ptr() if stats is not None else None
            L.call("cvhip_bn_act_bwd_apply", dz.data_ptr(), dz_ld, y.data_ptr(), y_ld, dy.data_ptr(), K, M, K, sc, sh, None, None,
                   None, None, act, ap, st)
        return (dy, dgamma if ctx.needs_input_grad[1] else None, dbeta if ctx.needs_input_grad[2] else None, None, None,
                dz if has_res else None, None, None, None, None, None, None, None, None)


def bn_act(y, gamma=None, beta=None, running_mean=None, running_var=None, residual=None, has_bn=True, training=True,
           momentum=0.1, eps=1e-5, act=L.ACT_NONE, act_param=0.0, track=True, sync=None):
    return BnAct.apply(y, gamma, beta, running_mean, running_var, residual, has_bn, training, momentum, eps, act, act_param, track, sync)


class MaxPool2d(torch.autograd.Function):
    @staticmethod
    def forward(ctx, x, k, stride, pad):
        x, ld = as_nhwc(x)
        N, Cc, H, W = x.shape
        OH, OW = (H + 2 * pad - k) // stride + 1, (W + 2 * pad - k) // stride + 1
        y = empty_nhwc(N, Cc, OH, OW, x.device)
        idx = torch.empty((N, OH, OW, Cc), dtype=torch.uint8, device=x.device)
        L.call("cvhip_maxpool2d_fwd", x.data_ptr(), ld, y.data_ptr(), Cc, idx.data_ptr(), N, Cc, H, W, k, stride, pad, _stream())
        ctx.meta = (N, Cc, H, W, k, stride, pad)
        ctx.save_for_backward(idx)
        return y

    @staticmethod
    def backward(ctx, dy):
        (idx,) = ctx.saved_tensors
        N, Cc, H, W, k, stride, pad = ctx.meta
        dy, ld = as_nhwc(dy)
        dx = empty_nhwc(N, Cc, H, W, dy.device)
        L.call("cvhip_maxpool2d_bwd", dy.data_ptr(), ld, idx.data_ptr(), dx.data_ptr(), Cc, N, Cc, H, W, k, stride, pad, 0, _stream())
        return dx, None, None, None


class SppfChain(torch.autograd.Function):

    @staticmethod
    def forward(ctx, x0, k):
        x0v, ld = as_nhwc(x0)
        N, c, H, W = x0v.shape
        if ld != 4 * c:
            raise L.CvhipError("SppfChain: x0 must be the first channel slice of an (N, 4c, H, W) NHWC buffer")
        pad = k // 2
        st = _stream()
        idx = torch.empty((3, N, H, W, c), dtype=torch.uint8, device=x0v.device)
        esz = x0v.element_size()
        for j in range(3):
            L.call("cvhip_maxpool2d_fwd", x0v.data_ptr() + j * c * esz, ld, x0v.data_ptr() + (j + 1) * c * esz, ld, idx[j].data_ptr(),
                   N, c, H, W, k, 1, pad, st)
        ctx.meta = (N, c, H, W, k, pad)
        ctx.save_for_backward(idx)
        return x0v.as_strided((N, 4 * c, H, W), (H * W * 4 * c, 1, W * 4 * c, 4 * c))

    @staticmethod
    def backward(ctx, d):
        (idx,) = ctx.saved_tensors
        N, c, H, W, k, pad = ctx.meta
        d, ld = as_nhwc(d)
        if ld != 4 * c or not d.is_contiguous(memory_format=torch.channels_last):
            d = d.contiguous(memory_format=torch.channels_last).clone()
            d, ld = as_nhwc(d)
        elif not _OWNED_BACKWARD[0]:
            d = d.clone(memory_format=torch.channels_last)
            d, ld = as_nhwc(d)
        st = _stream()
        esz = d.element_size()
        for j in (2, 1, 0):
            L.call("cvhip_maxpool2d_bwd", d.data_ptr() + (j + 1) * c * esz, ld, idx[j].data_ptr(), d.data_ptr() + j * c * esz, ld,
                   N, c, H, W, k, 1, pad, 1, st)
        return d[:, :c], None


def sppf_chain(x0, k):
    return SppfChain.apply(x0, int(k))


class SppParallel(torch.autograd.Function):

    @staticmethod
    def forward(ctx, x0, ks):
        x0v, ld = as_nhwc(x0)
        N, c, H, W = x0v.shape
        nk = len(ks)
        if ld != (1 + nk) * c:
            raise L.CvhipError("SppParallel: x0 must be the first channel slice of an (N, (1 + len(ks)) * c, H, W) NHWC buffer")
        st = _stream()
        idx = torch.empty((nk, N, H, W, c), dtype=torch.uint8, device=x0v.device)
        esz = x0v.element_size()
        for j, k in enumerate(ks):
            L.call("cvhip_maxpool2d_fwd", x0v.data_ptr(), ld, x0v.data_ptr() + (j + 1) * c * esz, ld, idx[j].data_ptr(), N, c, H, W, int(k), 1, int(k) // 2, st)
        ctx.meta = (N, c, H, W, tuple(int(k) for k in ks))
        ctx.save_for_backward(idx)
        return x0v.as_strided((N, (1 + nk) * c, H, W), (H * W * (1 + nk) * c, 1, W * (1 + nk) * c, (1 + nk) * c))

    @staticmethod
    def backward(ctx, d):
        (idx,) = ctx.saved_tensors
        N, c, H, W, ks = ctx.meta
        nk = len(ks)
        d, ld = as_nhwc(d)
        if ld != (1 + nk) * c or not d.is_contiguous(memory_format=torch.channels_last):
            d = d.contiguous(memory_format=torch.channels_last).clone()
            d, ld = as_nhwc(d)
        elif not _OWNED_BACKWARD[0]:
            d = d.clone(memory_format=torch.channels_last)
            d, ld = as_nhwc(d)
        st = _stream()
        esz = d.element_size()
        for j, k in enumerate(ks):
            L.call("cvhip_maxpool2d_bwd", d.data_ptr() + (j + 1) * c * esz, ld, idx[j].data_ptr(), d.data_ptr(), ld, N, c, H, W, k, 1, k // 2, 1, st)
        return d[:, :c], None


def spp_parallel(x0, ks):
    return SppParallel.apply(x0, tuple(ks))


def max_pool2d(x, k, stride=None, pad=0):
    return MaxPool2d.apply(x, int(k), int(stride if stride is not None else k), int(pad))


class Upsample2xCat(torch.autograd.Function):
# ... 592 lines not shown
        L.call("cvhip_head_permute_fwd", x.data_ptr(), ld, y.data_ptr(), N, A, NO, H, W, _stream())
        ctx.meta = (N, A, NO, H, W)
        return y

    @staticmethod
    def backward(ctx, dy):
        N, A, NO, H, W = ctx.meta
        dy = dy.float().contiguous()
        Cp = _round8(A * NO)
        buf = torch.empty((N, H, W, Cp), dtype=ACT_DTYPE, device=dy.device)
        L.call("cvhip_head_permute_bwd", dy.data_ptr(), buf.data_ptr(), Cp, N, A, NO, H, W, _stream())
        return buf.permute(0, 3, 1, 2)[:, :A * NO], None, None


def head_permute(x, A, NO):
    return HeadPermute.apply(x, A, NO)


class YoloV5LossFused(torch.autograd.Function):

    @staticmethod
    def forward(ctx, targets, cfg, *raws):
        dev = raws[0].device
        st = _stream()
        tg = targets.detach()
        if tg.dtype != torch.float32 or not tg.is_contiguous():
            tg = tg.float().contiguous()
        T = tg.shape[0]
        A, NO = cfg.num_anchors, cfg.num_classes + 5
        nl = len(raws)
        sums = torch.empty((nl, 4), dtype=torch.float32, device=dev)
        descs, wss, maps, ncells = [], [], [], []
        raws = [as_nhwc(r) for r in raws]
        assign = None
        ota = getattr(cfg, "ota", None)
        if ota is not None:
            N = raws[0][0].shape[0]
            od = L.OtaDesc()
            od.L, od.N, od.A, od.NO, od.T, od.G = nl, N, A, NO, T, int(ota["G"])
            od.anchor_t, od.img_size = float(cfg.anchor_t), float(ota["img_size"])
            for i, (r, ld) in enumerate(raws):
                od.H[i], od.W[i], od.ld[i], od.stride[i] = r.shape[2], r.shape[3], ld, float(ota["stride"][i])
                for j, v in enumerate([float(x) for pair in cfg.anchors[i] for x in pair]):
                    od.anchors[i][j] = v
            nb = L.load().cvhip_ota_workspace_bytes(C.byref(od))
            if nb < 0:
                L.check(int(nb), "cvhip_ota_workspace_bytes")
            ota_ws = torch.empty((int(nb),), dtype=torch.uint8, device=dev)
            assign = torch.empty((nl, 5 * A * T), dtype=torch.int32, device=dev)
            ptrs = (C.c_void_p * nl)(*[r.data_ptr() for r, _ in raws])
            L.call("cvhip_ota_assign", C.byref(od), ptrs, tg.data_ptr(), ota_ws.data_ptr(), assign.data_ptr(), st)
            ctx.ota_keep = (ota_ws, od)
            cfg.last_assign = assign
        for i, (r, ld) in enumerate(raws):
            N, Cc, H, W = r.shape
            if Cc != A * NO:
                raise L.CvhipError("yolov5 loss: head map has %d channels, expected %d" % (Cc, A * NO))
            d = L.YoloLossDesc(N, A, NO, H, W, ld, T, float(cfg.anchor_t))
            for j, v in enumerate([float(x) for pair in cfg.anchors[i] for x in pair]):
                d.anchors[j] = v
            nbytes = L.load().cvhip_yolov5_loss_workspace_bytes(C.byref(d))
            if nbytes < 0:
                L.check(int(nbytes), "cvhip_yolov5_loss_workspace_bytes")
            ws = torch.empty((int(nbytes),), dtype=torch.uint8, device=dev)
            if assign is not None:
                L.call("cvhip_yolov5_loss_level_fwd_assigned", C.byref(d), r.data_ptr(), tg.data_ptr(), assign[i].data_ptr(), ws.data_ptr(),
                       sums[i].data_ptr(), st)
            else:
                L.call("cvhip_yolov5_loss_level_fwd", C.byref(d), r.data_ptr(), tg.data_ptr(), ws.data_ptr(), sums[i].data_ptr(), st)
            descs.append(d)
            wss.append(ws)
            maps.append(r)
            ncells.append(float(N * A * H * W))
        key = (tuple(ncells), tuple(cfg.balance[:nl]), str(dev))
        consts = cfg._const_cache.get(key)
        if consts is None:
            consts = (torch.tensor(ncells, dtype=torch.float32, device=dev), torch.tensor(list(cfg.balance[:nl]), dtype=torch.float32, device=dev))
            cfg._const_cache[key] = consts
        total = torch.empty((1,), dtype=torch.float32, device=dev)
        stats = torch.empty((3,), dtype=torch.float32, device=dev)
        bs = float(maps[0].shape[0])
        L.call("cvhip_yolov5_loss_finalize", sums.data_ptr(), nl, consts[0].data_ptr(), consts[1].data_ptr(), float(cfg.hyp_box),
               float(cfg.hyp_obj), float(cfg.hyp_cls), cfg.num_classes, bs, total.data_ptr(), stats.data_ptr(), st)
        ctx.cfg, ctx.descs, ctx.wss, ctx.ncells, ctx.bs = cfg, descs, wss, ncells, bs
        ctx.save_for_backward(tg, sums, *maps)
        ctx.mark_non_differentiable(stats)
        ctx.set_materialize_grads(False)
        return total, stats

    @staticmethod
    def backward(ctx, g_total, g_stats):
        tg, sums, *maps = ctx.saved_tensors
        cfg = ctx.cfg
        st = _stream()
        g = g_total.detach()
        if g.dtype != torch.float32 or not g.is_contiguous():
            g = g.float().contiguous()
        outs = []
        nc = cfg.num_classes
        clear_colsums()
        for i, r in enumerate(maps):
            d = ctx.descs[i]
            draw = torch.empty((d.N, d.H, d.W, d.ld), dtype=ACT_DTYPE, device=r.device)
            K = d.A * d.NO
            bp = torch.empty((L.YOLO_BIAS_ROWS + L.REDUCE_SCRATCH_ROWS, 2, K), dtype=torch.float32, device=r.device)
            L.call("cvhip_yolov5_loss_level_bwd_bias", C.byref(d), r.data_ptr(), tg.data_ptr(), ctx.wss[i].data_ptr(), sums[i].data_ptr(),
                   g.data_ptr(), float(cfg.hyp_box) * ctx.bs, (float(cfg.hyp_cls) * ctx.bs / nc) if nc > 1 else 0.0,
                   float(cfg.hyp_obj) * float(cfg.balance[i]) * ctx.bs / ctx.ncells[i], draw.data_ptr(), bp.data_ptr(), st)
            offer_colsum(draw, bp, L.YOLO_BIAS_ROWS, K)
            outs.append(draw.permute(0, 3, 1, 2)[:, :K])
        return (None, None, *outs)


def yolov5_loss_fused(raws, targets, cfg):
    return YoloV5LossFused.apply(targets, cfg, *raws)


class SimotaLossFused(torch.autograd.Function):

    @staticmethod
    def forward(ctx, targets, cfg, *raws):
        dev = raws[0].device
        st = _stream()
        tg = targets.detach()
        if tg.dtype != torch.float32 or not tg.is_contiguous():
            tg = tg.float().contiguous()
        B, G = int(tg.shape[0]), int(tg.shape[1])
        nc = cfg.num_classes
        maps = []
        d = L.SimotaDesc()
        d.L, d.B, d.G, d.nc = len(raws), B, G, nc
        A = 0
        for i, r in enumerate(raws):
            r, ld = as_nhwc(r)
            N, Cc, H, W = r.shape
            if Cc != nc + 5 or N != B:
                raise L.CvhipError("simota loss: head map %d has shape %s, expected (%d, %d, H, W)" % (i, tuple(r.shape), B, nc + 5))
            d.H[i], d.W[i], d.ld[i], d.stride[i] = H, W, ld, float(cfg.strides[i])
            A += H * W
            maps.append(r)
        d.A = A
        nbytes = L.load().cvhip_simota_workspace_bytes(C.byref(d))
        if nbytes < 0:
            L.check(int(nbytes), "cvhip_simota_workspace_bytes")
        ws = torch.empty((int(nbytes),), dtype=torch.uint8, device=dev)
        ptrs = (C.c_void_p * len(maps))(*[m.data_ptr() for m in maps])
        out5 = torch.empty((5,), dtype=torch.float32, device=dev)
        L.call("cvhip_simota_loss_fwd", C.byref(d), ptrs, tg.data_ptr(), ws.data_ptr(), out5.data_ptr(), st)
        ctx.desc, ctx.ws = d, ws
        ctx.save_for_backward(tg, *maps)
        return out5

    @staticmethod
    def backward(ctx, g5):
        tg, *maps = ctx.saved_tensors
        d = ctx.desc
        g = g5.detach().float()[0:1].contiguous()
        draws = [torch.empty((d.B, d.H[i], d.W[i], d.ld[i]), dtype=ACT_DTYPE, device=maps[i].device) for i in range(d.L)]
        ptrs = (C.c_void_p * d.L)(*[m.data_ptr() for m in maps])
        dptrs = (C.c_void_p * d.L)(*[t.data_ptr() for t in draws])
        L.call("cvhip_simota_loss_bwd", C.byref(d), ptrs, tg.data_ptr(), ctx.ws.data_ptr(), g.data_ptr(), dptrs, _stream())
# ... 54 lines not shown
```

include/cvhip.h:

```cpp
#if !defined(CVHIP_H_) || defined(CVHIP_REDECLARE_F16)
#ifndef CVHIP_H_
#define CVHIP_H_
#endif

#include <stddef.h>
#include <stdint.h>

#ifdef __cplusplus
extern "C" {
#endif

#define CVHIP_VERSION 100

#define CVHIP_OK 0
#define CVHIP_ERR_INVALID (-1)
#define CVHIP_ERR_UNSUPPORTED (-2)
#define CVHIP_ERR_LAUNCH (-3)

#define CVHIP_ACT_NONE 0
#define CVHIP_ACT_RELU 1
#define CVHIP_ACT_SILU 2
#define CVHIP_ACT_LEAKY 3
#define CVHIP_ACT_SIGMOID 4
#define CVHIP_ACT_HSWISH 5
// ... 73 lines not shown

int cvhip_dwconv2d_dgrad(const cvhip_conv_desc* d, const void* dy_bf16, const float* w_crs,
                         void* dx_bf16, void* stream);
int cvhip_dwconv2d_wgrad(const cvhip_conv_desc* d, const void* x_bf16, const void* dy_bf16,
                         float* dw_crs, int accumulate, void* stream);

#define CVHIP_REDUCE_SCRATCH_ROWS 64
#define CVHIP_BN_ACC_SHARDS 16
int cvhip_colreduce_rows(int64_t M, int32_t C);

int cvhip_bn_stats_partial(const void* x_bf16, int64_t M, int32_t C, int32_t ld,
                           float* partial, void* stream);

int cvhip_bn_finalize(const float* partial, int32_t rows, int32_t C, int64_t count,
                      const float* gamma, const float* beta, float* running_mean,
                      float* running_var, float momentum, float eps, float* mean, float* invstd,
                      float* scale, float* shift, void* stream);

int cvhip_bn_eval_scale_shift(int32_t C, const float* gamma, const float* beta,
                              const float* running_mean, const float* running_var, float eps,
                              float* scale, float* shift, void* stream);

int cvhip_bn_act_fwd(const void* y_bf16, int32_t ld_y, void* z_bf16, int32_t ld_z, int64_t M,
                     int32_t C, const float* scale, const float* shift, int32_t act,
                     float act_param, const void* residual_bf16, int32_t ld_res, void* stream);

int cvhip_bn_add_act_fwd(const void* y_bf16, int32_t ld_y, void* z_bf16, int32_t ld_z, int64_t M,
                         int32_t C, const float* scale, const float* shift, int32_t act,
                         float act_param, const void* residual_bf16, int32_t ld_res, void* stream);

int cvhip_bn_act_bwd_partial(const void* dz_bf16, int32_t ld_dz, const void* y_bf16, int32_t ld_y,
                             int64_t M, int32_t C, const float* scale, const float* shift,
                             const float* mean, const float* invstd, int32_t act,
                             float act_param, float* partial, void* stream);
int cvhip_bn_bwd_finalize(const float* partial, int32_t rows, int32_t C, float* dgamma,
                          float* dbeta, float* acc_dgamma, float* acc_dbeta, void* stream);
int cvhip_bn_act_bwd_apply(const void* dz_bf16, int32_t ld_dz, const void* y_bf16, int32_t ld_y,
                           void* dy_bf16, int32_t ld_dy, int64_t M, int32_t C, const float* scale,
                           const float* shift, const float* mean, const float* invstd,
                           const float* dgamma, const float* dbeta, int32_t act, float act_param,
                           void* stream);

int cvhip_colsum_partial(const void* x_bf16, int64_t M, int32_t C, int32_t ld, float* partial,
                         void* stream);
int cvhip_colsum_finalize(const float* partial, int32_t rows, int32_t C, float* out, int accumulate,
                          void* stream);

int cvhip_maxpool2d_fwd(const void* x_bf16, int32_t ld_x, void* y_bf16, int32_t ld_y,
                        uint8_t* argmax, int32_t N, int32_t C, int32_t H, int32_t W, int32_t k,
                        int32_t stride, int32_t pad, void* stream);
int cvhip_maxpool2d_bwd(const void* dy_bf16, int32_t ld_dy, const uint8_t* argmax, void* dx_bf16,
                        int32_t ld_dx, int32_t N, int32_t C, int32_t H, int32_t W, int32_t k,
                        int32_t stride, int32_t pad, int accumulate, void* stream);

int cvhip_upsample2x_cat_fwd(const void* a_bf16, int32_t ld_a, int32_t Ca, const void* b_bf16,
                             int32_t ld_b, int32_t Cb, void* out_bf16, int32_t ld_out, int32_t N,
                             int32_t Ha, int32_t Wa, void* stream);
int cvhip_upsample2x_bwd(const void* dout_bf16, int32_t ld_dout, void* da_bf16, int32_t ld_da,
                         int32_t Ca, int32_t N, int32_t Ha, int32_t Wa, void* stream);

int cvhip_zero_fill(void* ptr, int64_t bytes, void* stream);
int cvhip_f32_unpad_add(const float* src, float* dst, int32_t K_valid, int32_t T, int32_t C,
                        int32_t C_valid, void* stream);

int cvhip_copy2d(const void* src_bf16, int32_t ld_src, void* dst_bf16, int32_t ld_dst, int64_t M,
                 int32_t C, void* stream);
int cvhip_add2d(const void* a_bf16, int32_t ld_a, const void* b_bf16, int32_t ld_b, void* dst_bf16,
                int32_t ld_dst, int64_t M, int32_t C, void* stream);

int cvhip_add_act_fwd(const void* a_bf16, int32_t ld_a, const void* b_bf16, int32_t ld_b,
                      void* out_bf16, int32_t ld_out, int64_t M, int32_t C, int32_t act,
                      float act_param, void* stream);

int cvhip_scale_nc(const void* x_bf16, int32_t ld_x, const float* scale_nc, void* y_bf16,
                   int32_t ld_y, int32_t N, int32_t C, int32_t HW, void* stream);

int cvhip_seg_ce_rows(int64_t M);
int cvhip_seg_ce_fwd(const void* logits_bf16, int32_t ld, const int64_t* target, int64_t M,
                     int32_t C, int32_t ignore_index, float* partial, float* out2, void* stream);
int cvhip_seg_ce_bwd(const void* logits_bf16, int32_t ld, const int64_t* target, int64_t M,
                     int32_t C, int32_t ignore_index, const float* out2, const float* grad_scale,
                     void* dlogits_bf16, int32_t ld_d, void* stream);

int cvhip_seg_ce_bilinear_ok(int32_t C, int32_t Hi, int32_t Wi, int32_t Ho, int32_t Wo, int32_t align_corners);
int cvhip_seg_ce_bilinear_fwd(const void* x_bf16, int32_t ld_x, const int64_t* target, int32_t N, int32_t C, int32_t Hi, int32_t Wi,
                              int32_t Ho, int32_t Wo, int32_t align_corners, int32_t ignore_index, float* partial, float* out2,
                              void* stream);
int cvhip_seg_ce_bilinear_bwd(const void* x_bf16, int32_t ld_x, const int64_t* target, int32_t N, int32_t C, int32_t Hi, int32_t Wi,
                              int32_t Ho, int32_t Wo, int32_t align_corners, int32_t ignore_index, const float* out2,
                              const float* grad_scale, void* dx_bf16, int32_t ld_dx, void* stream);

int cvhip_seg_ce_bilinear_fwd_px(const void* x_bf16, int32_t ld_x, const int64_t* target, int32_t N, int32_t C, int32_t Hi, int32_t Wi,
                                 int32_t Ho, int32_t Wo, int32_t align_corners, int32_t ignore_index, float* loss_px, void* stream);
int cvhip_seg_ce_bilinear_bwd_px(const void* x_bf16, int32_t ld_x, const int64_t* target, int32_t N, int32_t C, int32_t Hi, int32_t Wi,
                                 int32_t Ho, int32_t Wo, int32_t align_corners, int32_t ignore_index, const float* w_px,
                                 const float* grad_scale, void* dx_bf16, int32_t ld_dx, void* stream);

int64_t cvhip_ohem_select_workspace_bytes(void);
int cvhip_ohem_select(const float* loss_px, int64_t M, int32_t min_kept, float thresh_nlog, float loss_weight, void* workspace,
                      float* sel8, void* stream);
int cvhip_seg_ce_bilinear_bwd_ohem(const void* x_bf16, int32_t ld_x, const int64_t* target, int32_t N, int32_t C, int32_t Hi, int32_t Wi,
                                   int32_t Ho, int32_t Wo, int32_t align_corners, int32_t ignore_index, const float* loss_px,
                                   float loss_weight, const float* sel8, const float* grad_scale, void* dx_bf16, int32_t ld_dx,
                                   void* stream);

int cvhip_detail_boundary_targets(const int64_t* labels, int32_t N, int32_t H, int32_t W, float threshold, float* out, void* stream);
// ... 23 lines not shown
int cvhip_u8_nhwc_to_bf16_norm(const void* x_u8, int64_t npix, int32_t C, void* y_bf16, int32_t ld, const float* scale,
                               const float* shift, void* stream);
int cvhip_nchw_f32_to_nhwc_bf16(const float* x, void* y_bf16, int32_t N, int32_t C, int32_t H,
                                int32_t W, int32_t Cpad, void* stream);
int cvhip_focus_nchw_f32_to_nhwc_bf16(const float* x, void* y_bf16, int32_t N, int32_t C,
                                      int32_t H, int32_t W, int32_t Cpad, void* stream);
int cvhip_nhwc_bf16_to_nchw_f32(const void* x_bf16, int32_t ld, float* y, int32_t N, int32_t C,
                                int32_t H, int32_t W, void* stream);
int cvhip_nchw_f32_to_nhwc_bf16_ld(const float* x, void* y_bf16, int32_t ld, int32_t N, int32_t C,
                                   int32_t H, int32_t W, void* stream);

int cvhip_head_permute_fwd(const void* x_bf16, int32_t ld, float* y, int32_t N, int32_t A,
                           int32_t NO, int32_t H, int32_t W, void* stream);
int cvhip_head_permute_bwd(const float* dy, void* dx_bf16, int32_t ld, int32_t N, int32_t A,
                           int32_t NO, int32_t H, int32_t W, void* stream);

int cvhip_yolov5_decode(const void* p_bf16, int32_t ld, float* out, int32_t N, int32_t A,
                        int32_t NO, int32_t H, int32_t W, float stride, const float* anchors_px,
                        int64_t out_image_stride, int64_t out_level_offset, void* stream);

int64_t cvhip_nms_workspace_bytes(int32_t n);
int cvhip_nms_sorted(const float* boxes_xyxy, int32_t n, float iou_thr, void* workspace,
                     int32_t* keep_idx, int32_t* keep_count, void* stream);

int64_t cvhip_detect_postprocess_workspace_bytes(int32_t B, int32_t cand_cap, int32_t cap);
int cvhip_detect_postprocess(const float* pred, int32_t B, int32_t n, int32_t no, int32_t nc, float conf_thres, float iou_thres,
                             float class_offset, int32_t mode, int32_t multi_label, int32_t cand_cap, int32_t cap, int32_t max_det,
                             void* workspace, float* dets, int32_t* counts, int32_t* overflow, void* stream);
int64_t cvhip_sort_workspace_bytes(int64_t n);
int cvhip_argsort_desc_f32(const float* scores, int64_t n, void* workspace, int64_t* order, void* stream);

int cvhip_box_iou(const float* a_xyxy, int32_t n, const float* b_xyxy, int32_t m, float* out,
                  void* stream);

int cvhip_adamw_ema(float* param, const float* grad, float* exp_avg, float* exp_avg_sq, float* ema, int64_t n, const int64_t* seg_bounds,
                    const float* seg_lr, const float* seg_wd, int32_t nseg, float beta1, float beta2, float eps, float* step_state,
                    float ema_decay, float grad_scale, const float* dyn_decay_lrscale, const float* scaler2, void* stream);
int cvhip_sgd_nesterov_ema(float* param, const float* grad, float* momentum_buf, float* ema,
                           int64_t n, const int64_t* seg_bounds, const float* seg_lr,
                           const float* seg_wd, int32_t nseg, float momentum, int32_t nesterov,
                           int32_t first_step, float ema_decay, float grad_scale,
                           const float* dyn_decay_lrscale, void* stream);

int cvhip_loss_scale_check(const float* grad_arena, int64_t n, float* state4, void* stream);
int cvhip_loss_scale_update(float* state4, float* scaler2, float growth_factor, float backoff_factor, int32_t growth_interval,
                            void* stream);
int cvhip_sgd_nesterov_ema_scaled(float* param, const float* grad, float* momentum_buf, float* ema, int64_t n,
                                  const int64_t* seg_bounds, const float* seg_lr, const float* seg_wd, int32_t nseg,
                                  float momentum, int32_t nesterov, int32_t first_step, float ema_decay, float grad_scale,
                                  const float* dyn_decay_lrscale, const float* scaler2, void* stream);
int cvhip_i64_add(int64_t* v, int64_t n, int64_t delta, void* stream);
int cvhip_ema_update(float* ema, const float* src, int64_t n, float decay, const float* dyn_decay,
                     void* stream);

#ifndef CVHIP_REDECLARE_F16
typedef struct cvhip_yolo_loss_desc {
  int32_t N, A, NO, H, W, ld, T;
  float anchor_t;
  float anchors[16];
} cvhip_yolo_loss_desc;
#endif
int64_t cvhip_yolov5_loss_workspace_bytes(const cvhip_yolo_loss_desc* d);
int cvhip_yolov5_loss_level_fwd(const cvhip_yolo_loss_desc* d, const void* raw_bf16, const float* targets, void* ws,
                                float* sums4, void* stream);
int cvhip_yolov5_loss_finalize(const float* sums, int32_t levels, const float* ncell, const float* balance, float hyp_box,
                               float hyp_obj, float hyp_cls, int32_t nc, float batch, float* total, float* stats3,
                               void* stream);
int cvhip_yolov5_loss_level_bwd(const cvhip_yolo_loss_desc* d, const void* raw_bf16, const float* targets, void* ws,
                                const float* sums4, const float* gout, float k_box, float k_cls, float k_obj,
                                void* draw_bf16, void* stream);
#define CVHIP_YOLO_BIAS_ROWS 256
int cvhip_yolov5_loss_level_bwd_bias(const cvhip_yolo_loss_desc* d, const void* raw_bf16, const float* targets, void* ws,
                                     const float* sums4, const float* gout, float k_box, float k_cls, float k_obj,
                                     void* draw_bf16, float* bias_partial, void* stream);

#ifndef CVHIP_REDECLARE_F16
typedef struct cvhip_ota_desc {
  int32_t L, N, A, NO, T, G;
  int32_t H[4], W[4], ld[4];
  float stride[4];
  float anchors[4][16];
  float anchor_t;
  float img_size;
} cvhip_ota_desc;
#endif
int64_t cvhip_ota_workspace_bytes(const cvhip_ota_desc* d);
int cvhip_ota_assign(const cvhip_ota_desc* d, const void* const* raws, const float* targets, void* ws, int32_t* assign, void* stream);
int cvhip_ota_read_overflow(const cvhip_ota_desc* d, const void* ws, int32_t* out_device, void* stream);
int cvhip_yolov5_loss_level_fwd_assigned(const cvhip_yolo_loss_desc* d, const void* raw_bf16, const float* targets, const int32_t* assign,
                                         void* ws, float* sums4, void* stream);

#ifndef CVHIP_REDECLARE_F16
typedef struct cvhip_simota_desc {
  int32_t L, B, A, G, nc;
  int32_t H[4], W[4], ld[4];
  float stride[4];
} cvhip_simota_desc;
#endif
int64_t cvhip_simota_workspace_bytes(const cvhip_simota_desc* d);
int cvhip_simota_loss_fwd(const cvhip_simota_desc* d, const void* const* raws, const float* targets, void* ws, float* out5,
                          void* stream);
int cvhip_simota_loss_bwd(const cvhip_simota_desc* d, const void* const* raws, const float* targets, void* ws,
                          const float* gout, void* const* draws, void* stream);
int cvhip_simota_read_assignment(const cvhip_simota_desc* d, void* ws, int32_t* matched_out, float* miou_out, void* stream);

#define CVHIP_DTYPE_F32 0
#define CVHIP_DTYPE_F64 1
#define CVHIP_DTYPE_I32 2
#define CVHIP_DTYPE_BF16 3
#define CVHIP_DTYPE_U8 4
#define CVHIP_RED_SUM 0
#define CVHIP_RED_MAX 1
#define CVHIP_RED_MIN 2
int cvhip_comm_available(void);
int cvhip_comm_rccl_version(void);
int cvhip_comm_unique_id_bytes(void);
int cvhip_comm_get_unique_id(void* id_out);
int cvhip_comm_init_rank(void** comm_out, int32_t world, int32_t rank, const void* unique_id);
int cvhip_comm_destroy(void* comm);
int cvhip_comm_world(void* comm);
int cvhip_comm_rank(void* comm);
int cvhip_allreduce_bucket(void* comm, void* buf_f32, int64_t count, void* stream);
int cvhip_comm_allreduce(void* comm, void* buf, int64_t count, int32_t dtype, int32_t op, void* stream);
int cvhip_comm_broadcast(void* comm, void* buf, int64_t bytes, int32_t root, void* stream);
int cvhip_comm_reduce_scatter_f32(void* comm, void* buf_f32, int64_t count, void* stream);
int cvhip_comm_all_gather_f32(void* comm, void* buf_f32, int64_t count, void* stream);

// ... 96 lines not shown
```

include/cvhip_f16.h:

```cpp
#ifndef CVHIP_F16_H_
#define CVHIP_F16_H_
#include "cvhip.h"
#define cvhip_adamw_ema cvhip_adamw_ema_f16
#define cvhip_add2d cvhip_add2d_f16
#define cvhip_add_act_fwd cvhip_add_act_fwd_f16
#define cvhip_bn_acc_shards cvhip_bn_acc_shards_f16
#define cvhip_bn_act_bwd_apply cvhip_bn_act_bwd_apply_f16
#define cvhip_bn_act_bwd_apply_acc cvhip_bn_act_bwd_apply_acc_f16
#define cvhip_bn_act_bwd_partial cvhip_bn_act_bwd_partial_f16
#define cvhip_bn_act_bwd_sums_acc cvhip_bn_act_bwd_sums_acc_f16
#define cvhip_bn_act_fwd cvhip_bn_act_fwd_f16
#define cvhip_bn_act_fwd_acc cvhip_bn_act_fwd_acc_f16
#define cvhip_bn_act_fwd_acc_lazyres cvhip_bn_act_fwd_acc_lazyres_f16
#define cvhip_bn_add_act_fwd cvhip_bn_add_act_fwd_f16
#define cvhip_bn_bwd_finalize cvhip_bn_bwd_finalize_f16
#define cvhip_bn_eval_scale_shift cvhip_bn_eval_scale_shift_f16
#define cvhip_bn_finalize cvhip_bn_finalize_f16
#define cvhip_bn_finalize_acc cvhip_bn_finalize_acc_f16
#define cvhip_bn_stats_partial cvhip_bn_stats_partial_f16
#define cvhip_bn_tail_bwd_sums_acc cvhip_bn_tail_bwd_sums_acc_f16
#define cvhip_box_iou cvhip_box_iou_f16
#define cvhip_channel_scale_bwd_ds cvhip_channel_scale_bwd_ds_f16
#define cvhip_colreduce_rows cvhip_colreduce_rows_f16
#define cvhip_colsum_finalize cvhip_colsum_finalize_f16
// ... 33 lines not shown
#define cvhip_dwconv2d_fprop cvhip_dwconv2d_fprop_f16
#define cvhip_dwconv2d_fprop_act cvhip_dwconv2d_fprop_act_f16
#define cvhip_dwconv2d_fprop_stats cvhip_dwconv2d_fprop_stats_f16
#define cvhip_dwconv2d_fprop_stats_rows cvhip_dwconv2d_fprop_stats_rows_f16
#define cvhip_dwconv2d_wgrad cvhip_dwconv2d_wgrad_f16
#define cvhip_ema_update cvhip_ema_update_f16
#define cvhip_f32_unpad_add cvhip_f32_unpad_add_f16
#define cvhip_focus_nchw_f32_to_nhwc_bf16 cvhip_focus_nchw_f32_to_nhwc_bf16_f16
#define cvhip_global_avgpool_bwd cvhip_global_avgpool_bwd_f16
#define cvhip_global_avgpool_fwd cvhip_global_avgpool_fwd_f16
#define cvhip_head_permute_bwd cvhip_head_permute_bwd_f16
#define cvhip_head_permute_fwd cvhip_head_permute_fwd_f16
#define cvhip_i64_add cvhip_i64_add_f16
#define cvhip_last_error cvhip_last_error_f16
#define cvhip_loss_scale_check cvhip_loss_scale_check_f16
#define cvhip_loss_scale_update cvhip_loss_scale_update_f16
#define cvhip_maxpool2d_bwd cvhip_maxpool2d_bwd_f16
#define cvhip_maxpool2d_fwd cvhip_maxpool2d_fwd_f16
#define cvhip_nchw_f32_to_nhwc_bf16 cvhip_nchw_f32_to_nhwc_bf16_f16
#define cvhip_nchw_f32_to_nhwc_bf16_ld cvhip_nchw_f32_to_nhwc_bf16_ld_f16
#define cvhip_nhwc_bf16_to_nchw_f32 cvhip_nhwc_bf16_to_nchw_f32_f16
#define cvhip_nms_sorted cvhip_nms_sorted_f16
#define cvhip_nms_workspace_bytes cvhip_nms_workspace_bytes_f16
#define cvhip_ohem_select cvhip_ohem_select_f16
#define cvhip_ohem_select_workspace_bytes cvhip_ohem_select_workspace_bytes_f16
#define cvhip_ota_assign cvhip_ota_assign_f16
#define cvhip_ota_read_overflow cvhip_ota_read_overflow_f16
#define cvhip_ota_workspace_bytes cvhip_ota_workspace_bytes_f16
#define cvhip_prep_plan_build cvhip_prep_plan_build_f16
#define cvhip_prep_plan_item_bytes cvhip_prep_plan_item_bytes_f16
#define cvhip_prep_plan_run cvhip_prep_plan_run_f16
#define cvhip_resize_bilinear_bwd cvhip_resize_bilinear_bwd_f16
#define cvhip_resize_bilinear_bwd_workspace_bytes cvhip_resize_bilinear_bwd_workspace_bytes_f16
#define cvhip_resize_bilinear_bwd_ws cvhip_resize_bilinear_bwd_ws_f16
#define cvhip_resize_bilinear_fwd cvhip_resize_bilinear_fwd_f16
#define cvhip_resize_nearest_bwd cvhip_resize_nearest_bwd_f16
#define cvhip_resize_nearest_fwd cvhip_resize_nearest_fwd_f16
#define cvhip_scale_nc cvhip_scale_nc_f16
#define cvhip_seg_ce_bilinear_bwd cvhip_seg_ce_bilinear_bwd_f16
#define cvhip_seg_ce_bilinear_bwd_ohem cvhip_seg_ce_bilinear_bwd_ohem_f16
#define cvhip_seg_ce_bilinear_bwd_px cvhip_seg_ce_bilinear_bwd_px_f16
#define cvhip_seg_ce_bilinear_fwd cvhip_seg_ce_bilinear_fwd_f16
#define cvhip_seg_ce_bilinear_fwd_px cvhip_seg_ce_bilinear_fwd_px_f16
#define cvhip_seg_ce_bilinear_ok cvhip_seg_ce_bilinear_ok_f16
#define cvhip_seg_ce_bwd cvhip_seg_ce_bwd_f16
#define cvhip_seg_ce_fwd cvhip_seg_ce_fwd_f16
#define cvhip_seg_ce_rows cvhip_seg_ce_rows_f16
#define cvhip_sgd_nesterov_ema cvhip_sgd_nesterov_ema_f16
#define cvhip_sgd_nesterov_ema_scaled cvhip_sgd_nesterov_ema_scaled_f16
#define cvhip_simota_loss_bwd cvhip_simota_loss_bwd_f16
#define cvhip_simota_loss_fwd cvhip_simota_loss_fwd_f16
#define cvhip_simota_read_assignment cvhip_simota_read_assignment_f16
#define cvhip_simota_workspace_bytes cvhip_simota_workspace_bytes_f16
#define cvhip_u8_nhwc_to_bf16_norm cvhip_u8_nhwc_to_bf16_norm_f16
#define cvhip_upsample2x_bwd cvhip_upsample2x_bwd_f16
#define cvhip_upsample2x_cat_fwd cvhip_upsample2x_cat_fwd_f16
#define cvhip_version cvhip_version_f16
#define cvhip_yolov5_decode cvhip_yolov5_decode_f16
#define cvhip_yolov5_loss_finalize cvhip_yolov5_loss_finalize_f16
#define cvhip_yolov5_loss_level_bwd cvhip_yolov5_loss_level_bwd_f16
#define cvhip_yolov5_loss_level_bwd_bias cvhip_yolov5_loss_level_bwd_bias_f16
#define cvhip_yolov5_loss_level_fwd cvhip_yolov5_loss_level_fwd_f16
#define cvhip_yolov5_loss_level_fwd_assigned cvhip_yolov5_loss_level_fwd_assigned_f16
#define cvhip_yolov5_loss_workspace_bytes cvhip_yolov5_loss_workspace_bytes_f16
#define cvhip_zero_fill cvhip_zero_fill_f16
#define CVHIP_REDECLARE_F16
#include "cvhip.h"
#undef CVHIP_REDECLARE_F16
#undef cvhip_adamw_ema
#undef cvhip_add2d
#undef cvhip_add_act_fwd
#undef cvhip_bn_acc_shards
#undef cvhip_bn_act_bwd_apply
#undef cvhip_bn_act_bwd_apply_acc
#undef cvhip_bn_act_bwd_partial
#undef cvhip_bn_act_bwd_sums_acc
#undef cvhip_bn_act_fwd
#undef cvhip_bn_act_fwd_acc
#undef cvhip_bn_act_fwd_acc_lazyres
#undef cvhip_bn_add_act_fwd
#undef cvhip_bn_bwd_finalize
#undef cvhip_bn_eval_scale_shift
#undef cvhip_bn_finalize
#undef cvhip_bn_finalize_acc
#undef cvhip_bn_stats_partial
#undef cvhip_bn_tail_bwd_sums_acc
#undef cvhip_box_iou
#undef cvhip_channel_scale_bwd_ds
#undef cvhip_colreduce_rows
#undef cvhip_colsum_finalize
#undef cvhip_colsum_partial
#undef cvhip_conv1x1_bwd_fused
#undef cvhip_conv1x1_bwd_fused_acc
#undef cvhip_conv1x1_bwd_fused_lazy
#undef cvhip_conv1x1_bwd_fused_ok
#undef cvhip_conv1x1_bwd_fused_split
#undef cvhip_conv1x1_stream_blocks
#undef cvhip_conv1x1_stream_prologue_ok
#undef cvhip_conv2d_band_plan
#undef cvhip_conv2d_dgrad
#undef cvhip_conv2d_dgrad_add
#undef cvhip_conv2d_dgrad_plan
#undef cvhip_conv2d_dgrad_weight_elems
#undef cvhip_conv2d_fprop
#undef cvhip_conv2d_fprop_acc
#undef cvhip_conv2d_fprop_fused
#undef cvhip_conv2d_fprop_prologue_ok
#undef cvhip_conv2d_fprop_stats_rows
#undef cvhip_conv2d_out_hw
#undef cvhip_conv2d_patch_plan
#undef cvhip_conv2d_prep_weights
#undef cvhip_conv2d_weight_image_elems
#undef cvhip_conv2d_wgrad
#undef cvhip_conv2d_wgrad_band_plan
#undef cvhip_conv2d_wgrad_det
#undef cvhip_conv2d_wgrad_det_workspace_bytes
#undef cvhip_conv2d_wgrad_image
// ... 6 lines not shown
#undef cvhip_dwconv2d_fprop
#undef cvhip_dwconv2d_fprop_act
#undef cvhip_dwconv2d_fprop_stats
#undef cvhip_dwconv2d_fprop_stats_rows
#undef cvhip_dwconv2d_wgrad
#undef cvhip_ema_update
#undef cvhip_f32_unpad_add
#undef cvhip_focus_nchw_f32_to_nhwc_bf16
#undef cvhip_global_avgpool_bwd
#undef cvhip_global_avgpool_fwd
#undef cvhip_head_permute_bwd
#undef cvhip_head_permute_fwd
#undef cvhip_i64_add
#undef cvhip_last_error
#undef cvhip_loss_scale_check
#undef cvhip_loss_scale_update
#undef cvhip_maxpool2d_bwd
#undef cvhip_maxpool2d_fwd
#undef cvhip_nchw_f32_to_nhwc_bf16
#undef cvhip_nchw_f32_to_nhwc_bf16_ld
#undef cvhip_nhwc_bf16_to_nchw_f32
#undef cvhip_nms_sorted
#undef cvhip_nms_workspace_bytes
#undef cvhip_ohem_select
#undef cvhip_ohem_select_workspace_bytes
#undef cvhip_ota_assign
#undef cvhip_ota_read_overflow
#undef cvhip_ota_workspace_bytes
#undef cvhip_prep_plan_build
#undef cvhip_prep_plan_item_bytes
#undef cvhip_prep_plan_run
#undef cvhip_resize_bilinear_bwd
#undef cvhip_resize_bilinear_bwd_workspace_bytes
#undef cvhip_resize_bilinear_bwd_ws
#undef cvhip_resize_bilinear_fwd
#undef cvhip_resize_nearest_bwd
#undef cvhip_resize_nearest_fwd
#undef cvhip_scale_nc
#undef cvhip_seg_ce_bilinear_bwd
#undef cvhip_seg_ce_bilinear_bwd_ohem
#undef cvhip_seg_ce_bilinear_bwd_px
#undef cvhip_seg_ce_bilinear_fwd
#undef cvhip_seg_ce_bilinear_fwd_px
#undef cvhip_seg_ce_bilinear_ok
#undef cvhip_seg_ce_bwd
#undef cvhip_seg_ce_fwd
#undef cvhip_seg_ce_rows
#undef cvhip_sgd_nesterov_ema
#undef cvhip_sgd_nesterov_ema_scaled
#undef cvhip_simota_loss_bwd
#undef cvhip_simota_loss_fwd
#undef cvhip_simota_read_assignment
#undef cvhip_simota_workspace_bytes
#undef cvhip_u8_nhwc_to_bf16_norm
#undef cvhip_upsample2x_bwd
#undef cvhip_upsample2x_cat_fwd
#undef cvhip_version
#undef cvhip_yolov5_decode
#undef cvhip_yolov5_loss_finalize
#undef cvhip_yolov5_loss_level_bwd
#undef cvhip_yolov5_loss_level_bwd_bias
#undef cvhip_yolov5_loss_level_fwd
#undef cvhip_yolov5_loss_level_fwd_assigned
#undef cvhip_yolov5_loss_workspace_bytes
#undef cvhip_zero_fill
#endif
```

Measured before the change: 4978 images/sec.

## Fuse SPPF maxpool chain, batch YOLO loss levels, merge train-step tail kernels

Adds a single LDS-resident kernel that runs the three chained SPPF maxpools (forward and backward) without round-tripping through HBM between pools. It also adds multi-level YOLOv5 loss forward/backward entry points that handle all detection levels in one launch each. A fused train-step tail kernel does the EMA update, counter increment and grad/stat zeroing in one launch. The aim is fewer kernel launches and less global memory traffic, at the cost of new code paths whose correctness depends on the shared-memory sizing and argmax indexing.

```diff
diff --git a/cvpytorch_amd/arena.py b/cvpytorch_amd/arena.py
--- a/cvpytorch_amd/arena.py
+++ b/cvpytorch_amd/arena.py
@@ -422,9 +422,18 @@
             L.call("cvhip_sgd_nesterov_ema", self.param.data_ptr(), self.grad.data_ptr(), self.mom.data_ptr(), ema_ptr, self.total,
                    self.seg_bounds.data_ptr(), self.seg_lr.data_ptr(), self.seg_wd.data_ptr(), len(self.params), self.momentum,
                    int(self.nesterov), 0, 0.0, 1.0 / self.world, self.dyn.data_ptr(), st)
-        if self.ema_buf is not None and self.buf.numel():
+        n_ema = self.buf.numel() if self.ema_buf is not None else 0
+        n_nbt = self._nbt.numel() if (self._nbt is not None and self.model.training) else 0
+        if hasattr(L.load(), "cvhip_train_step_tail"):
+            L.call("cvhip_train_step_tail", self.ema_buf.data_ptr() if n_ema else None, self.buf.data_ptr() if n_ema else None, n_ema, 0.0,
+                   self.dyn.data_ptr(), self._nbt.data_ptr() if n_nbt else None, n_nbt, 1, self.grad.data_ptr(),
+                   self.grad.numel() * self.grad.element_size(), self.stat_acc.data_ptr() if self.stat_acc.numel() else None,
+                   self.stat_acc.numel() * self.stat_acc.element_size(), st)
+            self._acc_epoch[0] += 1
+            return
+        if n_ema:
             L.call("cvhip_ema_update", self.ema_buf.data_ptr(), self.buf.data_ptr(), self.buf.numel(), 0.0, self.dyn.data_ptr(), st)
-        if self._nbt is not None and self.model.training:
+        if n_nbt:
             L.call("cvhip_i64_add", self._nbt.data_ptr(), self._nbt.numel(), 1, st)
         self.zero_grad()
         self.zero_stats()
diff --git a/cvpytorch_amd/csrc/f16_names.h b/cvpytorch_amd/csrc/f16_names.h
--- a/cvpytorch_amd/csrc/f16_names.h
+++ b/cvpytorch_amd/csrc/f16_names.h
@@ -107,15 +107,21 @@
 #define cvhip_simota_loss_fwd cvhip_simota_loss_fwd_f16
 #define cvhip_simota_read_assignment cvhip_simota_read_assignment_f16
 #define cvhip_simota_workspace_bytes cvhip_simota_workspace_bytes_f16
+#define cvhip_sppf_chain_bwd cvhip_sppf_chain_bwd_f16
+#define cvhip_sppf_chain_fwd cvhip_sppf_chain_fwd_f16
+#define cvhip_train_step_tail cvhip_train_step_tail_f16
 #define cvhip_u8_nhwc_to_bf16_norm cvhip_u8_nhwc_to_bf16_norm_f16
 #define cvhip_upsample2x_bwd cvhip_upsample2x_bwd_f16
 #define cvhip_upsample2x_cat_fwd cvhip_upsample2x_cat_fwd_f16
 #define cvhip_version cvhip_version_f16
 #define cvhip_yolov5_decode cvhip_yolov5_decode_f16
+#define cvhip_yolov5_loss_bwd_levels cvhip_yolov5_loss_bwd_levels_f16
 #define cvhip_yolov5_loss_finalize cvhip_yolov5_loss_finalize_f16
+#define cvhip_yolov5_loss_fwd_levels cvhip_yolov5_loss_fwd_levels_f16
 #define cvhip_yolov5_loss_level_bwd cvhip_yolov5_loss_level_bwd_f16
 #define cvhip_yolov5_loss_level_bwd_bias cvhip_yolov5_loss_level_bwd_bias_f16
 #define cvhip_yolov5_loss_level_fwd cvhip_yolov5_loss_level_fwd_f16
 #define cvhip_yolov5_loss_level_fwd_assigned cvhip_yolov5_loss_level_fwd_assigned_f16
 #define cvhip_yolov5_loss_workspace_bytes cvhip_yolov5_loss_workspace_bytes_f16
+#define cvhip_yolov5_loss_workspace_bytes_levels cvhip_yolov5_loss_workspace_bytes_levels_f16
 #define cvhip_zero_fill cvhip_zero_fill_f16
diff --git a/cvpytorch_amd/csrc/pool_resize.hip b/cvpytorch_amd/csrc/pool_resize.hip
--- a/cvpytorch_amd/csrc/pool_resize.hip
+++ b/cvpytorch_amd/csrc/pool_resize.hip
@@ -147,6 +147,103 @@
 }
 
 template <int K, int kPoolLdsCvb>
+__device__ __forceinline__ void pool_lds_row_pass(const uint4* xs, uint4* rvs, uint2* rks, const int items, const int cvb, const int W) {
+  constexpr int PAD = K / 2;
+  for (int i = threadIdx.x; i < items; i += 256) {
+    const int pix = i / kPoolLdsCvb, cv = i - pix * kPoolLdsCvb;
+    if (cv >= cvb) continue;
+    const int h = pix / W, w = pix - h * W;
+    f32x8 ov;
+    int ok[8];
+    bool first = true;
+#pragma unroll
+    for (int j = 0; j < 8; ++j) {
+      ov.v[j] = -INFINITY;
+      ok[j] = 0;
+    }
+#pragma unroll
+    for (int kw = 0; kw < K; ++kw) {
+      const int iw = w + kw - PAD;
+      if ((unsigned)iw >= (unsigned)W) continue;
+      const f32x8 v = unpack8(xs[(h * W + iw) * kPoolLdsCvb + cv]);
+#pragma unroll
+      for (int j = 0; j < 8; ++j) {
+        if (first) ok[j] = kw;
+        if (v.v[j] > ov.v[j] || v.v[j] != v.v[j]) {
+          ov.v[j] = v.v[j];
+          ok[j] = kw;
+        }
+      }
+      first = false;
+    }
+    rvs[i] = pack8(ov);
+    uint2 kk;
+    kk.x = (unsigned)ok[0] | ((unsigned)ok[1] << 8) | ((unsigned)ok[2] << 16) | ((unsigned)ok[3] << 24);
+    kk.y = (unsigned)ok[4] | ((unsigned)ok[5] << 8) | ((unsigned)ok[6] << 16) | ((unsigned)ok[7] << 24);
+    rks[i] = kk;
+  }
+}
+
+template <int K, int kPoolLdsCvb, bool KEEP>
+__device__ __forceinline__ void pool_lds_col_pass(const uint4* rvs, const uint2* rks, uint4* xs, const int items, const int cvb, const int H,
+                                                  const int W, h16_t* yn, const int ld_y, uint8_t* idxn, const int C) {
+  constexpr int PAD = K / 2;
+  for (int i = threadIdx.x; i < items; i += 256) {
+    const int pix = i / kPoolLdsCvb, cv = i - pix * kPoolLdsCvb;
+    if (cv >= cvb) continue;
+    const int h = pix / W, w = pix - h * W;
+    float best[8];
+    int bi[8];
+    bool first = true;
+#pragma unroll
+    for (int j = 0; j < 8; ++j) {
+      best[j] = -INFINITY;
+      bi[j] = 0;
+    }
+#pragma unroll
+    for (int kh = 0; kh < K; ++kh) {
+      const int ih = h + kh - PAD;
+      if ((unsigned)ih >= (unsigned)H) continue;
+      const int o = (ih * W + w) * kPoolLdsCvb + cv;
+      const f32x8 v = unpack8(rvs[o]);
+      const uint2 kk = rks[o];
+#pragma unroll
+      for (int j = 0; j < 8; ++j) {
+        const int off = kh * K + (int)(((j < 4 ? kk.x : kk.y) >> (8 * (j & 3))) & 0xffu);
+        if (first) bi[j] = off;
+        if (v.v[j] > best[j] || v.v[j] != v.v[j]) {
+          best[j] = v.v[j];
+          bi[j] = off;
+        }
+      }
+      first = false;
+    }
+    {
+      f32x8 o;
+#pragma unroll
+      for (int j = 0; j < 8; ++j) o.v[j] = best[j];
+      const uint4 packed = pack8(o);
+      *reinterpret_cast<uint4*>(yn + (int64_t)pix * ld_y + cv * 8) = packed;
+      if (KEEP) xs[i] = packed;
+      if (idxn) {
+        uint2 iv;
+        iv.x = (unsigned)bi[0] | ((unsigned)bi[1] << 8) | ((unsigned)bi[2] << 16) | ((unsigned)bi[3] << 24);
+        iv.y = (unsigned)bi[4] | ((unsigned)bi[5] << 8) | ((unsigned)bi[6] << 16) | ((unsigned)bi[7] << 24);
+        *reinterpret_cast<uint2*>(idxn + (int64_t)pix * C + cv * 8) = iv;
+      }
+    }
+  }
+}
+
+template <int kPoolLdsCvb>
+__device__ __forceinline__ void pool_lds_stage(uint4* xs, const h16_t* xn, const int ld_x, const int items, const int cvb) {
+  for (int i = threadIdx.x; i < items; i += 256) {
+    const int pix = i / kPoolLdsCvb, cv = i - pix * kPoolLdsCvb;
+    if (cv < cvb) xs[i] = *reinterpret_cast<const uint4*>(xn + (int64_t)pix * ld_x + cv * 8);
+  }
+}
+
+template <int K, int kPoolLdsCvb>
 __global__ __launch_bounds__(256) void maxpool_s1_lds_fwd_kernel(const PoolParams p) {
   extern __shared__ __attribute__((aligned(16))) unsigned char pool_smem[];
   const int CV = p.C >> 3;
@@ -158,91 +255,64 @@
   uint4* const xs = reinterpret_cast<uint4*>(pool_smem);
   uint4* const rvs = xs + items;
   uint2* const rks = reinterpret_cast<uint2*>(rvs + items);
-  const h16_t* const xn = p.x + (int64_t)n * HW * p.ld_x + cv0 * 8;
-  for (int i = threadIdx.x; i < items; i += 256) {
-    const int pix = i / kPoolLdsCvb, cv = i - pix * kPoolLdsCvb;
-    if (cv < cvb) xs[i] = *reinterpret_cast<const uint4*>(xn + (int64_t)pix * p.ld_x + cv * 8);
-  }
+  pool_lds_stage<kPoolLdsCvb>(xs, p.x + (int64_t)n * HW * p.ld_x + cv0 * 8, p.ld_x, items, cvb);
   __syncthreads();
+  pool_lds_row_pass<K, kPoolLdsCvb>(xs, rvs, rks, items, cvb, p.W);
+  __syncthreads();
+  pool_lds_col_pass<K, kPoolLdsCvb, false>(rvs, rks, xs, items, cvb, p.H, p.W, p.y + (int64_t)n * HW * p.ld_y + cv0 * 8, p.ld_y,
+                                           p.idx ? p.idx + (int64_t)n * HW * p.C + cv0 * 8 : nullptr, p.C);
+}
+
+template <int K, int kPoolLdsCvb>
+__global__ __launch_bounds__(256) void sppf_chain_fwd_kernel(h16_t* __restrict__ buf, const int ld, uint8_t* __restrict__ idx, const int N,
+                                                             const int c, const int H, const int W) {
+  extern __shared__ __attribute__((aligned(16))) unsigned char pool_smem[];
+  const int CV = c >> 3;
+  const int groups = (CV + kPoolLdsCvb - 1) / kPoolLdsCvb;
+  const int n = blockIdx.x / groups, cv0 = (blockIdx.x - n * groups) * kPoolLdsCvb;
+  const int cvb = min(kPoolLdsCvb, CV - cv0);
+  const int HW = H * W;
+  const int items = HW * kPoolLdsCvb;
+  uint4* const xs = reinterpret_cast<uint4*>(pool_smem);
+  uint4* const rvs = xs + items;
+  uint2* const rks = reinterpret_cast<uint2*>(rvs + items);
+  h16_t* const bn = buf + (int64_t)n * HW * ld + cv0 * 8;
+  uint8_t* const in = idx + (int64_t)n * HW * c + cv0 * 8;
+  pool_lds_stage<kPoolLdsCvb>(xs, bn, ld, items, cvb);
+  __syncthreads();
+#pragma unroll 1
+  for (int j = 0; j < 3; ++j) {
+    pool_lds_row_pass<K, kPoolLdsCvb>(xs, rvs, rks, items, cvb, W);
+    __syncthreads();
+    pool_lds_col_pass<K, kPoolLdsCvb, true>(rvs, rks, xs, items, cvb, H, W, bn + (j + 1) * c, ld, in + (int64_t)j * N * HW * c, c);
+    __syncthreads();
+  }
+}
+
+template <int K, int kPoolLdsCvb>
+__device__ __forceinline__ f32x8 pool_lds_bwd_item(const uint4* gs, const uint2* is, const int ih, const int iw, const int cv, const int H,
+                                                   const int W) {
   constexpr int PAD = K / 2;
-  for (int i = threadIdx.x; i < items; i += 256) {
-    const int pix = i / kPoolLdsCvb, cv = i - pix * kPoolLdsCvb;
-    if (cv >= cvb) continue;
-    const int h = pix / p.W, w = pix - h * p.W;
-    f32x8 ov;
-    int ok[8];
-    bool first = true;
-#pragma unroll
-    for (int j = 0; j < 8; ++j) {
-      ov.v[j] = -INFINITY;
-      ok[j] = 0;
-    }
-#pragma unroll
-    for (int kw = 0; kw < K; ++kw) {
-      const int iw = w + kw - PAD;
-      if ((unsigned)iw >= (unsigned)p.W) continue;
-      const f32x8 v = unpack8(xs[(h * p.W + iw) * kPoolLdsCvb + cv]);
+  f32x8 acc;
+#pragma unroll
+  for (int j = 0; j < 8; ++j) acc.v[j] = 0.f;
+  const int oh_lo = max(0, ih - PAD), oh_hi = min(H - 1, ih + PAD);
+  const int ow_lo = max(0, iw - PAD), ow_hi = min(W - 1, iw + PAD);
+  for (int oh = oh_lo; oh <= oh_hi; ++oh) {
+    const int kh = ih - oh + PAD;
+    for (int ow = ow_lo; ow <= ow_hi; ++ow) {
+      const unsigned off = (unsigned)(kh * K + (iw - ow + PAD));
+      const int o = (oh * W + ow) * kPoolLdsCvb + cv;
+      const f32x8 g = unpack8(gs[o]);
+      const uint2 iv = is[o];
 #pragma unroll
       for (int j = 0; j < 8; ++j) {
-        if (first) ok[j] = kw;
-        if (v.v[j] > ov.v[j] || v.v[j] != v.v[j]) {
-          ov.v[j] = v.v[j];
-          ok[j] = kw;
-        }
-      }
-      first = false;
-    }
-    rvs[i] = pack8(ov);
-    uint2 kk;
-    kk.x = (unsigned)ok[0] | ((unsigned)ok[1] << 8) | ((unsigned)ok[2] << 16) | ((unsigned)ok[3] << 24);
-    kk.y = (unsigned)ok[4] | ((unsigned)ok[5] << 8) | ((unsigned)ok[6] << 16) | ((unsigned)ok[7] << 24);
-    rks[i] = kk;
-  }
-  __syncthreads();
-  for (int i = threadIdx.x; i < items; i += 256) {
-    const int pix = i / kPoolLdsCvb, cv = i - pix * kPoolLdsCvb;
-    if (cv >= cvb) continue;
-    const int h = pix / p.W, w = pix - h * p.W;
-    float best[8];
-    int bi[8];
-    bool first = true;
-#pragma unroll
-    for (int j = 0; j < 8; ++j) {
-      best[j] = -INFINITY;
-      bi[j] = 0;
-    }
-#pragma unroll
-    for (int kh = 0; kh < K; ++kh) {
-      const int ih = h + kh - PAD;
-      if ((unsigned)ih >= (unsigned)p.H) continue;
-      const int o = (ih * p.W + w) * kPoolLdsCvb + cv;
-      const f32x8 v = unpack8(rvs[o]);
-      const uint2 kk = rks[o];
-#pragma unroll
-      for (int j = 0; j < 8; ++j) {
-        const int off = kh * K + (int)(((j < 4 ? kk.x : kk.y) >> (8 * (j & 3))) & 0xffu);
-        if (first) bi[j] = off;
-        if (v.v[j] > best[j] || v.v[j] != v.v[j]) {
-          best[j] = v.v[j];
-          bi[j] = off;
-        }
-      }
-      first = false;
-    }
-    {
-      const int64_t opix = (int64_t)n * HW + h * p.W + w;
-      f32x8 o;
-#pragma unroll
-      for (int j = 0; j < 8; ++j) o.v[j] = best[j];
-      *reinterpret_cast<uint4*>(p.y + opix * p.ld_y + (cv0 + cv) * 8) = pack8(o);
-      if (p.idx) {
-        uint2 iv;
-        iv.x = (unsigned)bi[0] | ((unsigned)bi[1] << 8) | ((unsigned)bi[2] << 16) | ((unsigned)bi[3] << 24);
-        iv.y = (unsigned)bi[4] | ((unsigned)bi[5] << 8) | ((unsigned)bi[6] << 16) | ((unsigned)bi[7] << 24);
-        *reinterpret_cast<uint2*>(p.idx + opix * p.C + (cv0 + cv) * 8) = iv;
-      }
-    }
-  }
+        const unsigned b = ((j < 4 ? iv.x : iv.y) >> (8 * (j & 3))) & 0xffu;
+        if (b == off) acc.v[j] += g.v[j];
+      }
+    }
+  }
+  return acc;
 }
 
 template <int K, int kPoolLdsCvb>
@@ -264,52 +334,81 @@
     }
   }
   __syncthreads();
-  constexpr int PAD = K / 2;
   for (int i = threadIdx.x; i < HW * kPoolLdsCvb; i += 256) {
     const int pix = i / kPoolLdsCvb, cv = i - pix * kPoolLdsCvb;
     if (cv >= cvb) continue;
     const int ih = pix / p.W, iw = pix - ih * p.W;
-    float acc[8];
-#pragma unroll
-    for (int j = 0; j < 8; ++j) acc[j] = 0.f;
-    const int oh_lo = max(0, ih - PAD), oh_hi = min(p.H - 1, ih + PAD);
-    const int ow_lo = max(0, iw - PAD), ow_hi = min(p.W - 1, iw + PAD);
-    for (int oh = oh_lo; oh <= oh_hi; ++oh) {
-      const int kh = ih - oh + PAD;
-      for (int ow = ow_lo; ow <= ow_hi; ++ow) {
-        const unsigned off = (unsigned)(kh * K + (iw - ow + PAD));
-        const int o = (oh * p.W + ow) * kPoolLdsCvb + cv;
-        const f32x8 g = unpack8(gs[o]);
-        const uint2 iv = is[o];
-#pragma unroll
-        for (int j = 0; j < 8; ++j) {
-          const unsigned b = ((j < 4 ? iv.x : iv.y) >> (8 * (j & 3))) & 0xffu;
-          if (b == off) acc[j] += g.v[j];
-        }
-      }
-    }
+    const f32x8 acc = pool_lds_bwd_item<K, kPoolLdsCvb>(gs, is, ih, iw, cv, p.H, p.W);
     h16_t* const dst = p.dx + ((int64_t)n * HW + pix) * p.ld_dx + (cv0 + cv) * 8;
     f32x8 o;
     if (p.accumulate) {
       const f32x8 old = unpack8(*reinterpret_cast<const uint4*>(dst));
 #pragma unroll
-      for (int j = 0; j < 8; ++j) o.v[j] = old.v[j] + acc[j];
+      for (int j = 0; j < 8; ++j) o.v[j] = old.v[j] + acc.v[j];
     } else {
 #pragma unroll
-      for (int j = 0; j < 8; ++j) o.v[j] = acc[j];
+      for (int j = 0; j < 8; ++j) o.v[j] = acc.v[j];
     }
     *reinterpret_cast<uint4*>(dst) = pack8(o);
   }
 }
 
-static bool pool_lds_ok(const PoolParams& p, bool bwd) {
-  auto a16 = [](const void* q) { return (((uintptr_t)q) & 15) == 0; };
+template <int K, int kPoolLdsCvb>
+__global__ __launch_bounds__(256) void sppf_chain_bwd_kernel(h16_t* __restrict__ d, const int ld, const uint8_t* __restrict__ idx, const int N,
+                                                             const int c, const int H, const int W) {
+  extern __shared__ __attribute__((aligned(16))) unsigned char pool_smem[];
+  const int CV = c >> 3;
+  const int groups = (CV + kPoolLdsCvb - 1) / kPoolLdsCvb;
+  const int n = blockIdx.x / groups, cv0 = (blockIdx.x - n * groups) * kPoolLdsCvb;
+  const int cvb = min(kPoolLdsCvb, CV - cv0);
+  const int HW = H * W;
+  const int items = HW * kPoolLdsCvb;
+  uint4* ga = reinterpret_cast<uint4*>(pool_smem);
+  uint4* gb = ga + items;
+  uint2* const is = reinterpret_cast<uint2*>(gb + items);
+  h16_t* const dn = d + (int64_t)n * HW * ld + cv0 * 8;
+  const uint8_t* const in = idx + (int64_t)n * HW * c + cv0 * 8;
+  pool_lds_stage<kPoolLdsCvb>(ga, dn + 3 * c, ld, items, cvb);
+#pragma unroll 1
+  for (int j = 2; j >= 0; --j) {
+    const uint8_t* const ij = in + (int64_t)j * N * HW * c;
+    for (int i = threadIdx.x; i < items; i += 256) {
+      const int pix = i / kPoolLdsCvb, cv = i - pix * kPoolLdsCvb;
+      if (cv < cvb) is[i] = *reinterpret_cast<const uint2*>(ij + (int64_t)pix * c + cv * 8);
+    }
+    __syncthreads();
+    for (int i = threadIdx.x; i < items; i += 256) {
+      const int pix = i / kPoolLdsCvb, cv = i - pix * kPoolLdsCvb;
+      if (cv >= cvb) continue;
+      h16_t* const dst = dn + (int64_t)pix * ld + j * c + cv * 8;
+      const f32x8 old = unpack8(*reinterpret_cast<const uint4*>(dst));
+      const int ih = pix / W, iw = pix - ih * W;
+      const f32x8 acc = pool_lds_bwd_item<K, kPoolLdsCvb>(ga, is, ih, iw, cv, H, W);
+      f32x8 o;
+#pragma unroll
+      for (int q = 0; q < 8; ++q) o.v[q] = old.v[q] + acc.v[q];
+      if (j == 0) *reinterpret_cast<uint4*>(dst) = pack8(o);
+      else gb[i] = pack8(o);
+    }
+    __syncthreads();
+    uint4* const t = ga;
+    ga = gb;
+    gb = t;
+  }
+}
+
+static bool pool_lds_enabled() {
   static int on = -1;
   if (on < 0) {
     const char* e = getenv("CVHIP_POOL_LDS");
     on = (e && e[0] == '0') ? 0 : 1;
   }
-  if (!on || p.s != 1 || !(p.k & 1) || p.pad != p.k / 2 || p.OH != p.H || p.OW != p.W || (p.k != 3 && p.k != 5 && p.k != 9 && p.k != 13)) return false;
+  return on != 0;
+}
+
+static bool pool_lds_ok(const PoolParams& p, bool bwd) {
+  auto a16 = [](const void* q) { return (((uintptr_t)q) & 15) == 0; };
+  if (!pool_lds_enabled() || p.s != 1 || !(p.k & 1) || p.pad != p.k / 2 || p.OH != p.H || p.OW != p.W || (p.k != 3 && p.k != 5 && p.k != 9 && p.k != 13)) return false;
   const int cvb = pool_lds_cvb(p.H * p.W, bwd);
   if ((p.C & 7) || p.H * p.W > kPoolLdsMaxPix || cvb == 0 || (int64_t)p.N * ((p.C / 8 + cvb - 1) / cvb) < 128) return false;
   if (bwd) return (p.ld_dy & 7) == 0 && (p.ld_dx & 7) == 0 && a16(p.dy) && a16(p.dx) && ((((uintptr_t)p.cidx) & 7) == 0);
@@ -356,6 +455,46 @@
     default: CVHIP_POOL_K(13)
   }
 #undef CVHIP_POOL_K
+}
+
+static int sppf_chain_cvb(const void* buf, int ld, const void* idx, int c, int H, int W, int k) {
+  if (!pool_lds_enabled() || k != 5 || (c & 7) || (ld & 7) || ld < 4 * c || (((uintptr_t)buf) & 15) || (((uintptr_t)idx) & 7)) return 0;
+  const int64_t HW = (int64_t)H * W;
+  if (HW > kPoolLdsMaxPix) return 0;
+  for (int cap = 80 * 1024; cap <= 160 * 1024; cap *= 2)
+    for (int cvb = kPoolLdsCvbMax; cvb >= 1; cvb >>= 1)
+      if (HW * cvb * 40 <= cap) return cvb;
+  return 0;
+}
+
+template <int CVB>
+static int launch_sppf_chain(bool bwd, void* buf, int ld, uint8_t* idx, int N, int c, int H, int W, hipStream_t s) {
+  const int groups = (c / 8 + CVB - 1) / CVB;
+  const int lds = H * W * CVB * 40;
+  auto kf = sppf_chain_fwd_kernel<5, CVB>;
+  auto kb = sppf_chain_bwd_kernel<5, CVB>;
+  static bool attr_done[2][64] = {};
+  int devid = 0;
+  (void)hipGetDevice(&devid);
+  bool& done = attr_done[bwd ? 1 : 0][devid & 63];
+  if (!done) {
+    hipError_t e = hipFuncSetAttribute(bwd ? reinterpret_cast<const void*>(kb) : reinterpret_cast<const void*>(kf),
+                                       hipFuncAttributeMaxDynamicSharedMemorySize, 160 * 1024);
+    if (e != hipSuccess) {
+      set_last_error("hipFuncSetAttribute(sppf_chain)", e);
+      return CVHIP_ERR_LAUNCH;
+    }
+    done = true;
+  }
+  if (bwd) hipLaunchKernelGGL(kb, dim3(N * groups), dim3(256), lds, s, (h16_t*)buf, ld, (const uint8_t*)idx, N, c, H, W);
+  else hipLaunchKernelGGL(kf, dim3(N * groups), dim3(256), lds, s, (h16_t*)buf, ld, idx, N, c, H, W);
+  return check_launch(bwd ? "sppf_chain_bwd_kernel" : "sppf_chain_fwd_kernel");
+}
+
+static int sppf_chain_args_ok(const void* buf, int32_t ld, const void* idx, int32_t N, int32_t c, int32_t H, int32_t W, int32_t k) {
+  if (!buf || !idx || N <= 0 || c <= 0 || H <= 0 || W <= 0 || k <= 0 || !(k & 1) || ld < 4 * c) return CVHIP_ERR_INVALID;
+  if (k * k > 255 || (int64_t)N * H * W * c >= (1ll << 31)) return CVHIP_ERR_UNSUPPORTED;
+  return CVHIP_OK;
 }
 
 struct UpParams {
@@ -1015,6 +1154,35 @@
   const int64_t total = (int64_t)N * H * W * ((C + 7) / 8);
   hipLaunchKernelGGL(maxpool_bwd_kernel, dim3(grid_for(total)), dim3(256), 0, (hipStream_t)stream, p);
   return check_launch("maxpool_bwd_kernel");
+}
+
+int cvhip_sppf_chain_fwd(void* buf, int32_t ld, uint8_t* argmax3, int32_t N, int32_t c, int32_t H, int32_t W, int32_t k, void* stream) {
+  int rc = sppf_chain_args_ok(buf, ld, argmax3, N, c, H, W, k);
+  if (rc != CVHIP_OK) return rc;
+  const int cvb = sppf_chain_cvb(buf, ld, argmax3, c, H, W, k);
+  if (cvb == 4) return launch_sppf_chain<4>(false, buf, ld, argmax3, N, c, H, W, (hipStream_t)stream);
+  if (cvb == 2) return launch_sppf_chain<2>(false, buf, ld, argmax3, N, c, H, W, (hipStream_t)stream);
+  if (cvb == 1) return launch_sppf_chain<1>(false, buf, ld, argmax3, N, c, H, W, (hipStream_t)stream);
+  h16_t* const b = (h16_t*)buf;
+  const int64_t plane = (int64_t)N * H * W * c;
+  for (int j = 0; j < 3 && rc == CVHIP_OK; ++j)
+    rc = cvhip_maxpool2d_fwd(b + j * c, ld, b + (j + 1) * c, ld, argmax3 + j * plane, N, c, H, W, k, 1, k / 2, stream);
+  return rc;
+}
+
+int cvhip_sppf_chain_bwd(void* d, int32_t ld, const uint8_t* argmax3, int32_t N, int32_t c, int32_t H, int32_t W, int32_t k, void* stream) {
+  int rc = sppf_chain_args_ok(d, ld, argmax3, N, c, H, W, k);
+  if (rc != CVHIP_OK) return rc;
+  const int cvb = sppf_chain_cvb(d, ld, argmax3, c, H, W, k);
+  uint8_t* const ix = const_cast<uint8_t*>(argmax3);
+  if (cvb == 4) return launch_sppf_chain<4>(true, d, ld, ix, N, c, H, W, (hipStream_t)stream);
+  if (cvb == 2) return launch_sppf_chain<2>(true, d, ld, ix, N, c, H, W, (hipStream_t)stream);
+  if (cvb == 1) return launch_sppf_chain<1>(true, d, ld, ix, N, c, H, W, (hipStream_t)stream);
+  h16_t* const b = (h16_t*)d;
+  const int64_t plane = (int64_t)N * H * W * c;
+  for (int j = 2; j >= 0 && rc == CVHIP_OK; --j)
+    rc = cvhip_maxpool2d_bwd(b + (j + 1) * c, ld, argmax3 + j * plane, b + j * c, ld, N, c, H, W, k, 1, k / 2, 1, stream);
+  return rc;
 }
 
 int cvhip_upsample2x_cat_fwd(const void* a, int32_t ld_a, int32_t Ca, const void* b, int32_t ld_b, int32_t Cb,
diff --git a/cvpytorch_amd/csrc/weights_optim.hip b/cvpytorch_amd/csrc/weights_optim.hip
--- a/cvpytorch_amd/csrc/weights_optim.hip
+++ b/cvpytorch_amd/csrc/weights_optim.hip
@@ -551,7 +551,64 @@
   const int64_t i = (int64_t)blockIdx.x * blockDim.x + threadIdx.x;
   if (i < n) v[i] += delta;
 }
-}
+struct StepTailParams {
+  float* ema;
+  const float* src;
+  int64_t n_ema;
+  const float* dyn;
+  float decay;
+  long long* cnt;
+  int64_t n_cnt;
+  long long delta;
+  void *za, *zb;
+  int64_t na, nb;
+  int vec, fill_blocks;
+};
+__global__ __launch_bounds__(256) void step_tail_kernel(const StepTailParams p) {
+  if ((int)blockIdx.x < p.fill_blocks) {
+    const int64_t n = p.na + p.nb;
+    for (int64_t i = (int64_t)blockIdx.x * 256 + threadIdx.x; i < n; i += (int64_t)p.fill_blocks * 256) {
+      if (p.vec) *(i < p.na ? (uint4*)p.za + i : (uint4*)p.zb + (i - p.na)) = make_uint4(0u, 0u, 0u, 0u);
+      else *(i < p.na ? (uint32_t*)p.za + i : (uint32_t*)p.zb + (i - p.na)) = 0u;
+    }
+    return;
+  }
+  const int64_t b = (int64_t)blockIdx.x - p.fill_blocks, nb = (int64_t)gridDim.x - p.fill_blocks;
+  const float decay = p.dyn ? p.dyn[0] : p.decay;
+  for (int64_t i = b * 256 + threadIdx.x; i < p.n_ema + p.n_cnt; i += nb * 256) {
+    if (i < p.n_ema) p.ema[i] = decay * p.ema[i] + (1.f - decay) * p.src[i];
+    else p.cnt[i - p.n_ema] += p.delta;
+  }
+}
+}
+}
+
+int cvhip_train_step_tail(float* ema, const float* src, int64_t n_ema, float decay, const float* dyn_decay, int64_t* counters,
+                          int64_t n_counters, int64_t delta, void* zero_a, int64_t bytes_a, void* zero_b, int64_t bytes_b, void* stream) {
+  if (n_ema < 0 || n_counters < 0 || bytes_a < 0 || bytes_b < 0 || (n_ema > 0 && (!ema || !src)) || (n_counters > 0 && !counters) ||
+      (bytes_a > 0 && !zero_a) || (bytes_b > 0 && !zero_b))
+    return CVHIP_ERR_INVALID;
+  if (((((uintptr_t)zero_a) | ((uintptr_t)zero_b) | (uintptr_t)bytes_a | (uintptr_t)bytes_b) & 3) != 0) return CVHIP_ERR_INVALID;
+  StepTailParams p;
+  p.ema = ema;
+  p.src = src;
+  p.n_ema = n_ema;
+  p.dyn = dyn_decay;
+  p.decay = decay;
+  p.cnt = (long long*)counters;
+  p.n_cnt = n_counters;
+  p.delta = (long long)delta;
+  p.za = zero_a;
+  p.zb = zero_b;
+  p.vec = ((((uintptr_t)zero_a) | ((uintptr_t)zero_b) | (uintptr_t)bytes_a | (uintptr_t)bytes_b) & 15) == 0;
+  p.na = bytes_a / (p.vec ? 16 : 4);
+  p.nb = bytes_b / (p.vec ? 16 : 4);
+  const int64_t fb = cdiv64(p.na + p.nb, 256);
+  p.fill_blocks = (int)(fb < 4096 ? fb : 4096);
+  const int rest = (n_ema + n_counters) > 0 ? grid1d(n_ema + n_counters) : 0;
+  if (p.fill_blocks + rest == 0) return CVHIP_OK;
+  hipLaunchKernelGGL(step_tail_kernel, dim3(p.fill_blocks + rest), dim3(256), 0, (hipStream_t)stream, p);
+  return check_launch("step_tail_kernel");
 }
 
 int cvhip_i64_add(int64_t* v, int64_t n, int64_t delta, void* stream) {
diff --git a/cvpytorch_amd/csrc/yolo_loss.hip b/cvpytorch_amd/csrc/yolo_loss.hip
--- a/cvpytorch_amd/csrc/yolo_loss.hip
+++ b/cvpytorch_amd/csrc/yolo_loss.hip
@@ -54,9 +54,9 @@
   return iou - (rho2 / c2 + scale(v, alpha));
 }
 
-__global__ __launch_bounds__(256) void yolo_cand_kernel(const YoloLossParams p) {
+__device__ __forceinline__ void yolo_cand_body(const YoloLossParams& p, const int bid) {
   const int lane = threadIdx.x & 63;
-  const int c = blockIdx.x * 4 + (threadIdx.x >> 6);
+  const int c = bid * 4 + (threadIdx.x >> 6);
   if (c >= p.ncand) return;
   const int T = p.T, A = p.A;
   const int off = c / (A * T);
@@ -134,6 +134,8 @@
   if (lane == 0) cs[2] = p.nc > 1 ? lsum : 0.f;
 }
 
+__global__ __launch_bounds__(256) void yolo_cand_kernel(const YoloLossParams p) { yolo_cand_body(p, (int)blockIdx.x); }
+
 __device__ __forceinline__ float block_sum_1024(float v, float* red) {
   const int t = threadIdx.x;
   red[t] = v;
@@ -183,12 +185,12 @@
 }
 
 template <typename IT>
-__global__ __launch_bounds__(256) void yolo_obj_bwd_fill_kernel(const YoloLossParams p) {
+__device__ __forceinline__ void yolo_obj_bwd_fill_body(const YoloLossParams& p, const int bid, const int nblk) {
   const IT VP = (IT)(p.ld >> 3);
   const IT HW = (IT)p.H * (IT)p.W;
   const IT nvec = (IT)p.N * HW * VP;
   const float go = (p.gout ? p.gout[0] : 1.f) * p.k_obj;
-  const IT step = (IT)gridDim.x * 256;
+  const IT step = (IT)nblk * 256;
   const bool inv = (VP & (VP - 1)) == 0 && (step & (VP - 1)) == 0;
   const int vp_shift = inv ? __ffs((int)VP) - 1 : 0;
   auto anchors_of = [&](int c0) {
@@ -199,8 +201,8 @@
     }
     return m;
   };
-  const unsigned my_mask = inv ? anchors_of((int)(((IT)blockIdx.x * 256 + threadIdx.x) & (VP - 1)) * 8) : 0u;
-  for (IT i = (IT)blockIdx.x * 256 + threadIdx.x; i < nvec; i += step) {
+  const unsigned my_mask = inv ? anchors_of((int)(((IT)bid * 256 + threadIdx.x) & (VP - 1)) * 8) : 0u;
+  for (IT i = (IT)bid * 256 + threadIdx.x; i < nvec; i += step) {
     IT pix;
     int c0;
     unsigned mask;
@@ -232,13 +234,17 @@
   }
 }
 
+template <typename IT>
+__global__ __launch_bounds__(256) void yolo_obj_bwd_fill_kernel(const YoloLossParams p) {
+  yolo_obj_bwd_fill_body<IT>(p, (int)blockIdx.x, (int)gridDim.x);
+}
+
 template <bool BWD, typename IT>
-__global__ __launch_bounds__(256) void yolo_obj_kernel(const YoloLossParams p) {
-  __shared__ float red[256];
+__device__ __forceinline__ void yolo_obj_body(const YoloLossParams& p, const int bid, const int nblk, float* red) {
   const IT ncell = (IT)p.N * (IT)p.A * (IT)p.H * (IT)p.W;
   const float go = BWD ? (p.gout ? p.gout[0] : 1.f) * p.k_obj : 0.f;
   float acc = 0.f;
-  for (IT i = (IT)blockIdx.x * 256 + threadIdx.x; i < ncell; i += (IT)gridDim.x * 256) {
+  for (IT i = (IT)bid * 256 + threadIdx.x; i < ncell; i += (IT)nblk * 256) {
     IT r = i / (IT)p.W;
     const int gi = (int)(i - r * (IT)p.W);
     const IT r2 = r / (IT)p.H;
@@ -262,13 +268,18 @@
       if (threadIdx.x < s) red[threadIdx.x] += red[threadIdx.x + s];
       __syncthreads();
     }
-    if (threadIdx.x == 0) p.partial[blockIdx.x] = red[0];
-  }
-}
-
-__global__ __launch_bounds__(1024) void yolo_obj_reduce_kernel(const YoloLossParams p, int nblocks) {
-  __shared__ float red[1024];
-  if (blockIdx.x == 1) {
+    if (threadIdx.x == 0) p.partial[bid] = red[0];
+  }
+}
+
+template <bool BWD, typename IT>
+__global__ __launch_bounds__(256) void yolo_obj_kernel(const YoloLossParams p) {
+  __shared__ float red[256];
+  yolo_obj_body<BWD, IT>(p, (int)blockIdx.x, (int)gridDim.x, red);
+}
+
+__device__ __forceinline__ void yolo_obj_reduce_body(const YoloLossParams& p, const int nblocks, const int bid, float* red) {
+  if (bid == 1) {
     yolo_cand_reduce(p, red);
     return;
   }
@@ -278,9 +289,14 @@
   if (threadIdx.x == 0) p.sums[3] = v;
 }
 
-__global__ __launch_bounds__(256) void yolo_cand_bwd_kernel(const YoloLossParams p) {
+__global__ __launch_bounds__(1024) void yolo_obj_reduce_kernel(const YoloLossParams p, int nblocks) {
+  __shared__ float red[1024];
+  yolo_obj_reduce_body(p, nblocks, (int)blockIdx.x, red);
+}
+
+__device__ __forceinline__ void yolo_cand_bwd_body(const YoloLossParams& p, const int bid) {
   const int lane = threadIdx.x & 63;
-  const int c = blockIdx.x * 4 + (threadIdx.x >> 6);
+  const int c = bid * 4 + (threadIdx.x >> 6);
   if (c >= p.ncand) return;
   const int cell = p.cell[c];
   if (cell < 0 || p.winner[cell] != c + 1) return;
@@ -326,17 +342,18 @@
   if (ch1 < p.NO) dst[ch1] = (h16_t)(acc1 * kc);
 }
 
+__global__ __launch_bounds__(256) void yolo_cand_bwd_kernel(const YoloLossParams p) { yolo_cand_bwd_body(p, (int)blockIdx.x); }
+
 constexpr int kBiasRows = CVHIP_YOLO_BIAS_ROWS;
 template <typename IT>
-__global__ __launch_bounds__(256) void yolo_bias_partial_kernel(const YoloLossParams p, float* __restrict__ part) {
-  __shared__ float wacc[4][kLossMaxA * 128];
-  __shared__ float ored[kLossMaxA][256];
+__device__ __forceinline__ void yolo_bias_partial_body(const YoloLossParams& p, float* __restrict__ part, const int bid, const int nblk,
+                                                       float (*wacc)[kLossMaxA * 128], float (*ored)[256]) {
   const int K = p.A * p.NO;
   const int t = threadIdx.x, lane = t & 63, wave = t >> 6;
   for (int i = t; i < 4 * kLossMaxA * 128; i += 256) (&wacc[0][0])[i] = 0.f;
   __syncthreads();
-  const int per_blk = (p.ncand + gridDim.x - 1) / gridDim.x;
-  const int c_begin = blockIdx.x * per_blk, c_end = min(c_begin + per_blk, p.ncand);
+  const int per_blk = (p.ncand + nblk - 1) / nblk;
+  const int c_begin = bid * per_blk, c_end = min(c_begin + per_blk, p.ncand);
   for (int g0 = c_begin + wave * 64; g0 < c_end; g0 += 256) {
     const int c = g0 + lane;
     unsigned long long m = __ballot(c < c_end && p.cell[c] >= 0);
@@ -374,8 +391,8 @@
   for (int k = 0; k < kLossMaxA; ++k) oa[k] = 0.f;
   {
     const IT ncell = (IT)p.N * (IT)p.A * (IT)p.H * (IT)p.W, HW = (IT)p.H * (IT)p.W;
-    const IT per = (ncell + gridDim.x - 1) / gridDim.x;
-    const IT i_begin = (IT)blockIdx.x * per;
+    const IT per = (ncell + (unsigned)nblk - 1) / (unsigned)nblk;
+    const IT i_begin = (IT)bid * per;
     IT i_end = i_begin + per;
     if (i_end > ncell) i_end = ncell;
     for (IT i0 = i_begin + t; i0 < i_end; i0 += 256 * 8) {
@@ -407,12 +424,19 @@
   const float n = p.sums[0];
   const float g = p.gout ? p.gout[0] : 1.f;
   const float kb = n > 0.f ? g * p.k_box / n : 0.f, kc = n > 0.f ? g * p.k_cls / n : 0.f, go = g * p.k_obj;
-  float* const row = part + (int64_t)blockIdx.x * 2 * K;
+  float* const row = part + (int64_t)bid * 2 * K;
   for (int ch = t; ch < K; ch += 256) {
     const int a = ch / p.NO, o = ch - a * p.NO;
     const float v = ((wacc[0][ch] + wacc[1][ch]) + wacc[2][ch]) + wacc[3][ch];
     row[ch] = o == 4 ? ored[a][0] * go : v * (o < 4 ? kb : kc);
   }
+}
+
+template <typename IT>
+__global__ __launch_bounds__(256) void yolo_bias_partial_kernel(const YoloLossParams p, float* __restrict__ part) {
+  __shared__ float wacc[4][kLossMaxA * 128];
+  __shared__ float ored[kLossMaxA][256];
+  yolo_bias_partial_body<IT>(p, part, (int)blockIdx.x, (int)gridDim.x, wacc, ored);
 }
 
 __global__ void yolo_finalize_kernel(const float* sums, int L, const float* ncell, const float* balance, float hyp_box,
@@ -436,7 +460,63 @@
   stats[2] = lcls;
 }
 
-static int fill(YoloLossParams& p, const cvhip_yolo_loss_desc* d, const void* raw, const float* targets, void* ws, float* sums) {
+constexpr int kLossMaxLevels = CVHIP_YOLO_MAX_LEVELS;
+struct YoloLevelsParams {
+  YoloLossParams lv[kLossMaxLevels];
+  int first[kLossMaxLevels + 1];
+  int nb_obj[kLossMaxLevels];
+  float* part[kLossMaxLevels];
+  int L;
+};
+
+__device__ __forceinline__ int level_of_block(const YoloLevelsParams& P, const int b) {
+  int l = 0;
+  while (l + 1 < P.L && b >= P.first[l + 1]) ++l;
+  return l;
+}
+
+__global__ __launch_bounds__(256) void yolo_cand_levels_kernel(const YoloLevelsParams P) {
+  const int l = level_of_block(P, (int)blockIdx.x);
+  yolo_cand_body(P.lv[l], (int)blockIdx.x - P.first[l]);
+}
+
+__global__ __launch_bounds__(256) void yolo_obj_levels_kernel(const YoloLevelsParams P) {
+  __shared__ float red[256];
+  const int l = level_of_block(P, (int)blockIdx.x);
+  yolo_obj_body<false, unsigned>(P.lv[l], (int)blockIdx.x - P.first[l], P.first[l + 1] - P.first[l], red);
+}
+
+__global__ __launch_bounds__(1024) void yolo_obj_reduce_levels_kernel(const YoloLevelsParams P) {
+  __shared__ float red[1024];
+  const int l = (int)blockIdx.x >> 1;
+  yolo_obj_reduce_body(P.lv[l], P.nb_obj[l], (int)blockIdx.x & 1, red);
+}
+
+__global__ __launch_bounds__(256) void yolo_obj_bwd_fill_levels_kernel(const YoloLevelsParams P) {
+  const int l = level_of_block(P, (int)blockIdx.x);
+  yolo_obj_bwd_fill_body<unsigned>(P.lv[l], (int)blockIdx.x - P.first[l], P.first[l + 1] - P.first[l]);
+}
+
+__global__ __launch_bounds__(256) void yolo_cand_bwd_levels_kernel(const YoloLevelsParams P) {
+  const int l = level_of_block(P, (int)blockIdx.x);
+  yolo_cand_bwd_body(P.lv[l], (int)blockIdx.x - P.first[l]);
+}
+
+__global__ __launch_bounds__(256) void yolo_bias_partial_levels_kernel(const YoloLevelsParams P) {
+  __shared__ float wacc[4][kLossMaxA * 128];
+  __shared__ float ored[kLossMaxA][256];
+  const int l = (int)blockIdx.x / kBiasRows;
+  yolo_bias_partial_body<unsigned>(P.lv[l], P.part[l], (int)blockIdx.x - l * kBiasRows, kBiasRows, wacc, ored);
+}
+
+static int64_t ws_front_bytes(int64_t ncell) { return (ncell * 4 + 255) / 256 * 256 * 2; }
+static int64_t ws_rest_bytes(int64_t ncell, int64_t ncand, int64_t gs) {
+  auto r = [](int64_t b) { return (b + 255) / 256 * 256; };
+  return r(ncand * 4) * 2 + r(ncand * kCandStride * 4) + r(ncand * gs * 4) + r(1024 * 4) + r(ncell * 4);
+}
+
+static int fill(YoloLossParams& p, const cvhip_yolo_loss_desc* d, const void* raw, const float* targets, void* ws, float* sums,
+                void* ws_rest = nullptr) {
   if (!d || !raw || !targets || !ws || !sums) return CVHIP_ERR_INVALID;
   if (d->N <= 0 || d->A <= 0 || d->A > kLossMaxA || d->NO < 6 || d->NO > 128 || d->H <= 0 || d->W <= 0 || d->T <= 0 || d->ld < d->A * d->NO)
     return CVHIP_ERR_INVALID;
@@ -467,6 +547,7 @@
   };
   p.winner = (int*)take(ncell * 4);
   p.head = (int*)take(ncell * 4);
+  if (ws_rest) w = (unsigned char*)ws_rest;
   p.next = (int*)take(ncand * 4);
   p.cell = (int*)take(ncand * 4);
   p.cand = (float*)take(ncand * kCandStride * 4);
@@ -582,4 +663,117 @@
   return check_launch("yolov5_loss_level_bwd");
 }
 
-}
+int64_t cvhip_yolov5_loss_workspace_bytes_levels(const cvhip_yolo_loss_desc* d, int32_t levels) {
+  if (!d || levels <= 0 || levels > kLossMaxLevels) return CVHIP_ERR_INVALID;
+  int64_t total = 0;
+  for (int l = 0; l < levels; ++l) {
+    const int64_t b = cvhip_yolov5_loss_workspace_bytes(d + l);
+    if (b < 0) return b;
+    total += b;
+  }
+  return total;
+}
+
+static int levels_fill(YoloLevelsParams& P, const cvhip_yolo_loss_desc* d, int levels, const void* const* raws, const float* targets, void* ws,
+                       float* sums, int64_t* front_bytes) {
+  if (!d || !raws || !ws || !sums || levels <= 0 || levels > kLossMaxLevels) return CVHIP_ERR_INVALID;
+  int64_t front = 0;
+  for (int l = 0; l < levels; ++l) front += ws_front_bytes((int64_t)d[l].N * d[l].A * d[l].H * d[l].W);
+  unsigned char* f = (unsigned char*)ws;
+  unsigned char* r = f + front;
+  for (int l = 0; l < levels; ++l) {
+    const int rc = fill(P.lv[l], d + l, raws[l], targets, f, sums + l * 4, r);
+    if (rc != CVHIP_OK) return rc;
+    const int64_t ncell = (int64_t)d[l].N * d[l].A * d[l].H * d[l].W;
+    f += ws_front_bytes(ncell);
+    r += ws_rest_bytes(ncell, P.lv[l].ncand, P.lv[l].gstride);
+  }
+  for (int l = levels; l < kLossMaxLevels; ++l) P.lv[l] = P.lv[0];
+  for (int l = 0; l < kLossMaxLevels; ++l) {
+    P.nb_obj[l] = 0;
+    P.part[l] = nullptr;
+  }
+  P.L = levels;
+  *front_bytes = front;
+  return CVHIP_OK;
+}
+
+int cvhip_yolov5_loss_fwd_levels(const cvhip_yolo_loss_desc* d, int32_t levels, const void* const* raws, const float* targets, void* ws,
+                                 float* sums, void* stream) {
+  YoloLevelsParams P;
+  int64_t front = 0;
+  int rc = levels_fill(P, d, levels, raws, targets, ws, sums, &front);
+  if (rc != CVHIP_OK) return rc;
+  hipStream_t st = (hipStream_t)stream;
+  int nb[kLossMaxLevels];
+  for (int l = 0; l < levels; ++l) {
+    const YoloLossParams& p = P.lv[l];
+    const int64_t ncell = (int64_t)p.N * p.A * p.H * p.W;
+    nb[l] = (int)(cdiv64(ncell, 256) < 1024 ? cdiv64(ncell, 256) : 1024);
+    if (ncell + (int64_t)nb[l] * 256 >= (1ll << 32)) return CVHIP_ERR_UNSUPPORTED;
+  }
+  rc = zero_fill(ws, front, st);
+  if (rc != CVHIP_OK) return rc;
+  P.first[0] = 0;
+  for (int l = 0; l < kLossMaxLevels; ++l) P.first[l + 1] = P.first[l] + (l < levels ? cdiv(P.lv[l].ncand, 4) : 0);
+  hipLaunchKernelGGL(yolo_cand_levels_kernel, dim3(P.first[levels]), dim3(256), 0, st, P);
+  for (int l = 0; l < kLossMaxLevels; ++l) P.first[l + 1] = P.first[l] + (l < levels ? nb[l] : 0);
+  hipLaunchKernelGGL(yolo_obj_levels_kernel, dim3(P.first[levels]), dim3(256), 0, st, P);
+  for (int l = 0; l < levels; ++l) P.nb_obj[l] = nb[l];
+  hipLaunchKernelGGL(yolo_obj_reduce_levels_kernel, dim3(2 * levels), dim3(1024), 0, st, P);
+  return check_launch("yolov5_loss_fwd_levels");
+}
+
+int cvhip_yolov5_loss_bwd_levels(const cvhip_yolo_loss_desc* d, int32_t levels, const void* const* raws, const float* targets, void* ws,
+                                 const float* sums, const float* gout, float k_box, float k_cls, const float* k_obj, void* const* draws,
+                                 float* const* bias_partials, void* stream) {
+  YoloLevelsParams P;
+  int64_t front = 0;
+  int rc = levels_fill(P, d, levels, raws, targets, ws, const_cast<float*>(sums), &front);
+  if (rc != CVHIP_OK) return rc;
+  if (!k_obj || !draws) return CVHIP_ERR_INVALID;
+  hipStream_t st = (hipStream_t)stream;
+  for (int l = 0; l < levels; ++l) {
+    if (!draws[l] || (bias_partials && !bias_partials[l])) return CVHIP_ERR_INVALID;
+    YoloLossParams& p = P.lv[l];
+    p.draw = (h16_t*)draws[l];
+    p.gout = gout;
+    p.k_box = k_box;
+    p.k_cls = k_cls;
+    p.k_obj = k_obj[l];
+    if (bias_partials) P.part[l] = bias_partials[l];
+  }
+  YoloLevelsParams F = P;
+  int nf = 0;
+  F.first[0] = 0;
+  for (int l = 0; l < levels; ++l) {
+    const YoloLossParams& p = P.lv[l];
+    if ((p.ld & 7) == 0 && (((uintptr_t)p.draw) & 15) == 0) {
+      const int64_t nvec = (int64_t)p.N * p.H * p.W * (p.ld >> 3);
+      const int nbf = (int)(cdiv64(nvec, 256 * 4) < 8192 ? cdiv64(nvec, 256 * 4) : 8192);
+      if (nvec + (int64_t)nbf * 256 >= (1ll << 32)) return CVHIP_ERR_UNSUPPORTED;
+      F.lv[nf] = p;
+      F.first[nf + 1] = F.first[nf] + (nbf > 0 ? nbf : 1);
+      ++nf;
+    } else {
+      const int64_t ncell = (int64_t)p.N * p.A * p.H * p.W;
+      rc = zero_fill(p.draw, (int64_t)p.N * p.H * p.W * p.ld * 2, st);
+      if (rc != CVHIP_OK) return rc;
+      const int nbo = (int)(cdiv64(ncell, 256) < 8192 ? cdiv64(ncell, 256) : 8192);
+      if (ncell + (int64_t)nbo * 256 < (1ll << 32)) hipLaunchKernelGGL((yolo_obj_kernel<true, unsigned>), dim3(nbo), dim3(256), 0, st, p);
+      else hipLaunchKernelGGL((yolo_obj_kernel<true, int64_t>), dim3(nbo), dim3(256), 0, st, p);
+    }
+  }
+  if (nf > 0) {
+    for (int l = nf; l < kLossMaxLevels; ++l) F.first[l + 1] = F.first[l];
+    F.L = nf;
+    hipLaunchKernelGGL(yolo_obj_bwd_fill_levels_kernel, dim3(F.first[nf]), dim3(256), 0, st, F);
+  }
+  P.first[0] = 0;
+  for (int l = 0; l < kLossMaxLevels; ++l) P.first[l + 1] = P.first[l] + (l < levels ? cdiv(P.lv[l].ncand, 4) : 0);
+  hipLaunchKernelGGL(yolo_cand_bwd_levels_kernel, dim3(P.first[levels]), dim3(256), 0, st, P);
+  if (bias_partials) hipLaunchKernelGGL(yolo_bias_partial_levels_kernel, dim3(kBiasRows * levels), dim3(256), 0, st, P);
+  return check_launch("yolov5_loss_bwd_levels");
+}
+
+}
diff --git a/cvpytorch_amd/lib.py b/cvpytorch_amd/lib.py
--- a/cvpytorch_amd/lib.py
+++ b/cvpytorch_amd/lib.py
@@ -13,6 +13,7 @@
 DGRAD_CLASS_INTS = 12
 REDUCE_SCRATCH_ROWS = 64
 YOLO_BIAS_ROWS = 256
+YOLO_MAX_LEVELS = 4
 BN_ACC_SHARDS = 16
 
 
@@ -141,6 +142,8 @@
     "cvhip_colsum_finalize": (_i32, [_p, _i32, _i32, _p, _i32, _p]),
     "cvhip_maxpool2d_fwd": (_i32, [_p, _i32, _p, _i32, _p, _i32, _i32, _i32, _i32, _i32, _i32, _i32, _p]),
     "cvhip_maxpool2d_bwd": (_i32, [_p, _i32, _p, _p, _i32, _i32, _i32, _i32, _i32, _i32, _i32, _i32, _i32, _p]),
+    "cvhip_sppf_chain_fwd": (_i32, [_p, _i32, _p, _i32, _i32, _i32, _i32, _i32, _p]),
+    "cvhip_sppf_chain_bwd": (_i32, [_p, _i32, _p, _i32, _i32, _i32, _i32, _i32, _p]),
     "cvhip_upsample2x_cat_fwd": (_i32, [_p, _i32, _i32, _p, _i32, _i32, _p, _i32, _i32, _i32, _i32, _p]),
     "cvhip_upsample2x_bwd": (_i32, [_p, _i32, _p, _i32, _i32, _i32, _i32, _i32, _p]),
     "cvhip_zero_fill": (_i32, [_p, _i64, _p]),
@@ -191,12 +194,16 @@
     "cvhip_loss_scale_update": (_i32, [_p, _p, _f32, _f32, _i32, _p]),
     "cvhip_i64_add": (_i32, [_p, _i64, _i64, _p]),
     "cvhip_ema_update": (_i32, [_p, _p, _i64, _f32, _p, _p]),
+    "cvhip_train_step_tail": (_i32, [_p, _p, _i64, _f32, _p, _p, _i64, _i64, _p, _i64, _p, _i64, _p]),
     "cvhip_u8_nhwc_to_bf16_norm": (_i32, [_p, _i64, _i32, _p, _i32, _p, _p, _p]),
     "cvhip_yolov5_loss_workspace_bytes": (_i64, [_ylp]),
     "cvhip_yolov5_loss_level_fwd": (_i32, [_ylp, _p, _p, _p, _p, _p]),
     "cvhip_yolov5_loss_finalize": (_i32, [_p, _i32, _p, _p, _f32, _f32, _f32, _i32, _f32, _p, _p, _p]),
     "cvhip_yolov5_loss_level_bwd": (_i32, [_ylp, _p, _p, _p, _p, _p, _f32, _f32, _f32, _p, _p]),
     "cvhip_yolov5_loss_level_bwd_bias": (_i32, [_ylp, _p, _p, _p, _p, _p, _f32, _f32, _f32, _p, _p, _p]),
+    "cvhip_yolov5_loss_workspace_bytes_levels": (_i64, [_ylp, _i32]),
+    "cvhip_yolov5_loss_fwd_levels": (_i32, [_ylp, _i32, _pp, _p, _p, _p, _p]),
+    "cvhip_yolov5_loss_bwd_levels": (_i32, [_ylp, _i32, _pp, _p, _p, _p, _p, _f32, _f32, C.POINTER(_f32), _pp, _pp, _p]),
     "cvhip_ota_workspace_bytes": (_i64, [_otp]),
     "cvhip_ota_assign": (_i32, [_otp, _pp, _p, _p, _p, _p]),
     "cvhip_ota_read_overflow": (_i32, [_otp, _p, _p, _p]),
diff --git a/cvpytorch_amd/ops.py b/cvpytorch_amd/ops.py
--- a/cvpytorch_amd/ops.py
+++ b/cvpytorch_amd/ops.py
@@ -1583,6 +1583,10 @@
         return dx, None, None, None
 
 
+def _has_sppf_chain():
+    return hasattr(L.load(), "cvhip_sppf_chain_fwd")
+
+
 class SppfChain(torch.autograd.Function):
 
     @staticmethod
@@ -1594,10 +1598,13 @@
         pad = k // 2
         st = _stream()
         idx = torch.empty((3, N, H, W, c), dtype=torch.uint8, device=x0v.device)
-        esz = x0v.element_size()
-        for j in range(3):
-            L.call("cvhip_maxpool2d_fwd", x0v.data_ptr() + j * c * esz, ld, x0v.data_ptr() + (j + 1) * c * esz, ld, idx[j].data_ptr(),
-                   N, c, H, W, k, 1, pad, st)
+        if _has_sppf_chain():
+            L.call("cvhip_sppf_chain_fwd", x0v.data_ptr(), ld, idx.data_ptr(), N, c, H, W, k, st)
+        else:
+            esz = x0v.element_size()
+            for j in range(3):
+                L.call("cvhip_maxpool2d_fwd", x0v.data_ptr() + j * c * esz, ld, x0v.data_ptr() + (j + 1) * c * esz, ld, idx[j].data_ptr(),
+                       N, c, H, W, k, 1, pad, st)
         ctx.meta = (N, c, H, W, k, pad)
         ctx.save_for_backward(idx)
         return x0v.as_strided((N, 4 * c, H, W), (H * W * 4 * c, 1, W * 4 * c, 4 * c))
@@ -1614,10 +1621,13 @@
             d = d.clone(memory_format=torch.channels_last)
             d, ld = as_nhwc(d)
         st = _stream()
-        esz = d.element_size()
-        for j in (2, 1, 0):
-            L.call("cvhip_maxpool2d_bwd", d.data_ptr() + (j + 1) * c * esz, ld, idx[j].data_ptr(), d.data_ptr() + j * c * esz, ld,
-                   N, c, H, W, k, 1, pad, 1, st)
+        if _has_sppf_chain():
+            L.call("cvhip_sppf_chain_bwd", d.data_ptr(), ld, idx.data_ptr(), N, c, H, W, k, st)
+        else:
+            esz = d.element_size()
+            for j in (2, 1, 0):
+                L.call("cvhip_maxpool2d_bwd", d.data_ptr() + (j + 1) * c * esz, ld, idx[j].data_ptr(), d.data_ptr() + j * c * esz, ld,
+                       N, c, H, W, k, 1, pad, 1, st)
         return d[:, :c], None
 
 
@@ -2316,13 +2326,21 @@
             L.call("cvhip_ota_assign", C.byref(od), ptrs, tg.data_ptr(), ota_ws.data_ptr(), assign.data_ptr(), st)
             ctx.ota_keep = (ota_ws, od)
             cfg.last_assign = assign
+        multi = assign is None and nl <= L.YOLO_MAX_LEVELS and hasattr(L.load(), "cvhip_yolov5_loss_fwd_levels")
+        darr = (L.YoloLossDesc * nl)()
         for i, (r, ld) in enumerate(raws):
             N, Cc, H, W = r.shape
             if Cc != A * NO:
                 raise L.CvhipError("yolov5 loss: head map has %d channels, expected %d" % (Cc, A * NO))
-            d = L.YoloLossDesc(N, A, NO, H, W, ld, T, float(cfg.anchor_t))
+            d = darr[i]
+            d.N, d.A, d.NO, d.H, d.W, d.ld, d.T, d.anchor_t = N, A, NO, H, W, ld, T, float(cfg.anchor_t)
             for j, v in enumerate([float(x) for pair in cfg.anchors[i] for x in pair]):
                 d.anchors[j] = v
+            descs.append(d)
+            maps.append(r)
+            ncells.append(float(N * A * H * W))
+            if multi:
+                continue
             nbytes = L.load().cvhip_yolov5_loss_workspace_bytes(C.byref(d))
             if nbytes < 0:
                 L.check(int(nbytes), "cvhip_yolov5_loss_workspace_bytes")
@@ -2332,10 +2350,15 @@
                        sums[i].data_ptr(), st)
             else:
                 L.call("cvhip_yolov5_loss_level_fwd", C.byref(d), r.data_ptr(), tg.data_ptr(), ws.data_ptr(), sums[i].data_ptr(), st)
-            descs.append(d)
             wss.append(ws)
-            maps.append(r)
-            ncells.append(float(N * A * H * W))
+        if multi:
+            nbytes = L.load().cvhip_yolov5_loss_workspace_bytes_levels(darr, nl)
+            if nbytes < 0:
+                L.check(int(nbytes), "cvhip_yolov5_loss_workspace_bytes_levels")
+            wss.append(torch.empty((int(nbytes),), dtype=torch.uint8, device=dev))
+            ptrs = (C.c_void_p * nl)(*[r.data_ptr() for r in maps])
+            L.call("cvhip_yolov5_loss_fwd_levels", darr, nl, ptrs, tg.data_ptr(), wss[0].data_ptr(), sums.data_ptr(), st)
+        ctx.multi, ctx.darr = multi, darr
         key = (tuple(ncells), tuple(cfg.balance[:nl]), str(dev))
         consts = cfg._const_cache.get(key)
         if consts is None:
@@ -2363,14 +2386,27 @@
         outs = []
         nc = cfg.num_classes
         clear_colsums()
+        k_box, k_cls = float(cfg.hyp_box) * ctx.bs, (float(cfg.hyp_cls) * ctx.bs / nc) if nc > 1 else 0.0
+        k_obj = [float(cfg.hyp_obj) * float(cfg.balance[i]) * ctx.bs / ctx.ncells[i] for i in range(len(maps))]
+        draws, bps = [], []
         for i, r in enumerate(maps):
             d = ctx.descs[i]
             draw = torch.empty((d.N, d.H, d.W, d.ld), dtype=ACT_DTYPE, device=r.device)
             K = d.A * d.NO
             bp = torch.empty((L.YOLO_BIAS_ROWS + L.REDUCE_SCRATCH_ROWS, 2, K), dtype=torch.float32, device=r.device)
-            L.call("cvhip_yolov5_loss_level_bwd_bias", C.byref(d), r.data_ptr(), tg.data_ptr(), ctx.wss[i].data_ptr(), sums[i].data_ptr(),
-                   g.data_ptr(), float(cfg.hyp_box) * ctx.bs, (float(cfg.hyp_cls) * ctx.bs / nc) if nc > 1 else 0.0,
-                   float(cfg.hyp_obj) * float(cfg.balance[i]) * ctx.bs / ctx.ncells[i], draw.data_ptr(), bp.data_ptr(), st)
+            if not ctx.multi:
+                L.call("cvhip_yolov5_loss_level_bwd_bias", C.byref(d), r.data_ptr(), tg.data_ptr(), ctx.wss[i].data_ptr(), sums[i].data_ptr(),
+                       g.data_ptr(), k_box, k_cls, k_obj[i], draw.data_ptr(), bp.data_ptr(), st)
+            draws.append(draw)
+            bps.append(bp)
+        if ctx.multi:
+            nl = len(maps)
+            vp = C.c_void_p * nl
+            L.call("cvhip_yolov5_loss_bwd_levels", ctx.darr, nl, vp(*[r.data_ptr() for r in maps]), tg.data_ptr(), ctx.wss[0].data_ptr(),
+                   sums.data_ptr(), g.data_ptr(), k_box, k_cls, (C.c_float * nl)(*k_obj), vp(*[t.data_ptr() for t in draws]),
+                   vp(*[t.data_ptr() for t in bps]), st)
+        for i, (draw, bp) in enumerate(zip(draws, bps)):
+            K = ctx.descs[i].A * ctx.descs[i].NO
             offer_colsum(draw, bp, L.YOLO_BIAS_ROWS, K)
             outs.append(draw.permute(0, 3, 1, 2)[:, :K])
         return (None, None, *outs)
diff --git a/include/cvhip.h b/include/cvhip.h
--- a/include/cvhip.h
+++ b/include/cvhip.h
@@ -149,6 +149,10 @@
 int cvhip_maxpool2d_bwd(const void* dy_bf16, int32_t ld_dy, const uint8_t* argmax, void* dx_bf16,
                         int32_t ld_dx, int32_t N, int32_t C, int32_t H, int32_t W, int32_t k,
                         int32_t stride, int32_t pad, int accumulate, void* stream);
+int cvhip_sppf_chain_fwd(void* buf_bf16, int32_t ld, uint8_t* argmax3, int32_t N, int32_t c, int32_t H, int32_t W, int32_t k,
+                         void* stream);
+int cvhip_sppf_chain_bwd(void* buf_bf16, int32_t ld, const uint8_t* argmax3, int32_t N, int32_t c, int32_t H, int32_t W, int32_t k,
+                         void* stream);
 
 int cvhip_upsample2x_cat_fwd(const void* a_bf16, int32_t ld_a, int32_t Ca, const void* b_bf16,
                              int32_t ld_b, int32_t Cb, void* out_bf16, int32_t ld_out, int32_t N,
@@ -278,6 +282,9 @@
 int cvhip_i64_add(int64_t* v, int64_t n, int64_t delta, void* stream);
 int cvhip_ema_update(float* ema, const float* src, int64_t n, float decay, const float* dyn_decay,
                      void* stream);
+int cvhip_train_step_tail(float* ema, const float* src, int64_t n_ema, float decay, const float* dyn_decay, int64_t* counters,
+                          int64_t n_counters, int64_t delta, void* zero_a, int64_t bytes_a, void* zero_b, int64_t bytes_b,
+                          void* stream);
 
 #ifndef CVHIP_REDECLARE_F16
 typedef struct cvhip_yolo_loss_desc {
@@ -299,6 +306,13 @@
 int cvhip_yolov5_loss_level_bwd_bias(const cvhip_yolo_loss_desc* d, const void* raw_bf16, const float* targets, void* ws,
                                      const float* sums4, const float* gout, float k_box, float k_cls, float k_obj,
                                      void* draw_bf16, float* bias_partial, void* stream);
+#define CVHIP_YOLO_MAX_LEVELS 4
+int64_t cvhip_yolov5_loss_workspace_bytes_levels(const cvhip_yolo_loss_desc* d, int32_t levels);
+int cvhip_yolov5_loss_fwd_levels(const cvhip_yolo_loss_desc* d, int32_t levels, const void* const* raws_bf16, const float* targets,
+                                 void* ws, float* sums, void* stream);
+int cvhip_yolov5_loss_bwd_levels(const cvhip_yolo_loss_desc* d, int32_t levels, const void* const* raws_bf16, const float* targets,
+                                 void* ws, const float* sums, const float* gout, float k_box, float k_cls, const float* k_obj,
+                                 void* const* draws_bf16, float* const* bias_partials, void* stream);
 
 #ifndef CVHIP_REDECLARE_F16
 typedef struct cvhip_ota_desc {
diff --git a/include/cvhip_f16.h b/include/cvhip_f16.h
--- a/include/cvhip_f16.h
+++ b/include/cvhip_f16.h
@@ -109,17 +109,23 @@
 #define cvhip_simota_loss_fwd cvhip_simota_loss_fwd_f16
 #define cvhip_simota_read_assignment cvhip_simota_read_assignment_f16
 #define cvhip_simota_workspace_bytes cvhip_simota_workspace_bytes_f16
+#define cvhip_sppf_chain_bwd cvhip_sppf_chain_bwd_f16
+#define cvhip_sppf_chain_fwd cvhip_sppf_chain_fwd_f16
+#define cvhip_train_step_tail cvhip_train_step_tail_f16
 #define cvhip_u8_nhwc_to_bf16_norm cvhip_u8_nhwc_to_bf16_norm_f16
 #define cvhip_upsample2x_bwd cvhip_upsample2x_bwd_f16
 #define cvhip_upsample2x_cat_fwd cvhip_upsample2x_cat_fwd_f16
 #define cvhip_version cvhip_version_f16
 #define cvhip_yolov5_decode cvhip_yolov5_decode_f16
+#define cvhip_yolov5_loss_bwd_levels cvhip_yolov5_loss_bwd_levels_f16
 #define cvhip_yolov5_loss_finalize cvhip_yolov5_loss_finalize_f16
+#define cvhip_yolov5_loss_fwd_levels cvhip_yolov5_loss_fwd_levels_f16
 #define cvhip_yolov5_loss_level_bwd cvhip_yolov5_loss_level_bwd_f16
 #define cvhip_yolov5_loss_level_bwd_bias cvhip_yolov5_loss_level_bwd_bias_f16
 #define cvhip_yolov5_loss_level_fwd cvhip_yolov5_loss_level_fwd_f16
 #define cvhip_yolov5_loss_level_fwd_assigned cvhip_yolov5_loss_level_fwd_assigned_f16
 #define cvhip_yolov5_loss_workspace_bytes cvhip_yolov5_loss_workspace_bytes_f16
+#define cvhip_yolov5_loss_workspace_bytes_levels cvhip_yolov5_loss_workspace_bytes_levels_f16
 #define cvhip_zero_fill cvhip_zero_fill_f16
 #define CVHIP_REDECLARE_F16
 #include "cvhip.h"
@@ -232,16 +238,22 @@
 #undef cvhip_simota_loss_fwd
 #undef cvhip_simota_read_assignment
 #undef cvhip_simota_workspace_bytes
+#undef cvhip_sppf_chain_bwd
+#undef cvhip_sppf_chain_fwd
+#undef cvhip_train_step_tail
 #undef cvhip_u8_nhwc_to_bf16_norm
 #undef cvhip_upsample2x_bwd
 #undef cvhip_upsample2x_cat_fwd
 #undef cvhip_version
 #undef cvhip_yolov5_decode
+#undef cvhip_yolov5_loss_bwd_levels
 #undef cvhip_yolov5_loss_finalize
+#undef cvhip_yolov5_loss_fwd_levels
 #undef cvhip_yolov5_loss_level_bwd
 #undef cvhip_yolov5_loss_level_bwd_bias
 #undef cvhip_yolov5_loss_level_fwd
 #undef cvhip_yolov5_loss_level_fwd_assigned
 #undef cvhip_yolov5_loss_workspace_bytes
+#undef cvhip_yolov5_loss_workspace_bytes_levels
 #undef cvhip_zero_fill
 #endif
```

New measurement: 5042 images/sec (median of 6 runs). +1.3%, better.
